# ShuoYangRobotics/Cerberus

Measured on NVIDIA H100. Metric: sliding-window solves/sec (10-frame x 150-feature windows), higher is better.
Workload: dtype f64

## Files before the change

### cerberus_b200/csrc/cabi.cu

```cuda
#include "../../include/cerberus_b200.h"
#include "solve_kernel.cuh"
#include "preint_kernel.cuh"
#include "feature_kernels.cuh"
#include "marg_kernels.cuh"
#include "pack_kernels.cuh"
#include "resident_kernels.cuh"
#include <string>
#include <vector>
#include <thread>
#include <cstring>
#include <cstdio>
#include <algorithm>
#include <chrono>
#include <cstdlib>
#include <cstdint>
#include <utility>

using namespace cerb;

static thread_local std::string g_err;
static int fail(int code, const std::string &msg) { g_err = msg; return code; }
#define CUDA_TRY(expr)                                                                                         \
    do {                                                                                                       \
        cudaError_t e_ = (expr);                                                                               \
// ... 300 lines not shown
        if (op.height == 1) CUDA_TRY(cudaMemcpyAsync(op.dst, op.src, op.width, cudaMemcpyHostToDevice, s));
        else CUDA_TRY(cudaMemcpy2DAsync(op.dst, op.dpitch, op.src, op.spitch, op.width, op.height, cudaMemcpyHostToDevice, s));
    }
    const size_t staged = [&] { size_t t = 0; for (const auto &j : pl.stage) t += j.bytes; return t; }();
    h->last_dma_ops += (int)pl.dma.size(); h->last_staged_bytes += staged; h->traffic.staged += (int64_t)staged;
    return CERB_OK;
}

static int upload_raw(CerbHandle *h, int w0, int cn, const CerbWindowDesc *descs, const CerbWindowState *states, cudaStream_t s, double *t_stage_ms) {
    for (int w = w0; w < w0 + cn; w++) { int rc = validate_window(h, descs[w], states[w], &h->n0[w]); if (rc) return rc; h->nfeat[w] = descs[w].n_features; }
    h->res_n = 0; h->prior_gathered = h->prior_gather_due = false;
    UploadPlan pl;
    plan_rows(h, pl, w0, cn, h->rdesc, 0, 1, 0, [&](int w) { return (const void *)&descs[w]; }, [&](int) { return sizeof(CerbWindowDesc); });
    plan_rows(h, pl, w0, cn, h->rstate, 0, 1, 0, [&](int w) { return (const void *)&states[w]; }, [&](int) { return sizeof(CerbWindowState); });
    plan_rows(h, pl, w0, cn, h->rfeat, 0, 1, 0,
              [&](int w) { return (const void *)descs[w].features; }, [&](int w) { return (size_t)descs[w].n_features * sizeof(CerbFeature); });
    plan_rows(h, pl, w0, cn, h->robs, 0, 1, 0,
              [&](int w) { return (const void *)descs[w].obs; }, [&](int w) { return (size_t)descs[w].n_obs * sizeof(CerbObservation); });
    plan_rows(h, pl, w0, cn, h->rlam, 0, 1, 0,
              [&](int w) { return (const void *)states[w].para_Feature; }, [&](int w) { return (size_t)descs[w].n_features * 8; });
    const size_t tail_off = (size_t)(RAW_PRE_HEAD + RAW_PRE_JCOL0 * 31) * 8, tail_w = sizeof(CerbIMULegPreint) - tail_off;
    static_assert(sizeof(CerbIMULegPreint) == (33 + 2 * 961) * 8, "CerbIMULegPreint layout");
    static_assert(sizeof(CerbIMUPreint) == 467 * 8 && sizeof(CerbIMUPreint) <= RAW_PRE_STRIDE * 8, "CerbIMUPreint layout");
    plan_rows(h, pl, w0, cn, h->rpre, 0, CERB_WINDOW_SIZE, sizeof(CerbIMULegPreint),
              [&](int w) { return (const void *)descs[w].preint; }, [&](int w) { return descs[w].preint ? (size_t)RAW_PRE_HEAD * 8 : (size_t)0; });
    plan_rows(h, pl, w0, cn, h->rpre, RAW_PRE_HEAD * 8, CERB_WINDOW_SIZE, sizeof(CerbIMULegPreint),
              [&](int w) { return (const void *)((const char *)descs[w].preint + tail_off); }, [&](int w) { return descs[w].preint ? tail_w : (size_t)0; });
    plan_rows(h, pl, w0, cn, h->rpre, 0, CERB_WINDOW_SIZE, sizeof(CerbIMUPreint),
              [&](int w) { return (const void *)descs[w].imu_preint; }, [&](int w) { return descs[w].preint ? (size_t)0 : sizeof(CerbIMUPreint); });
    plan_rows(h, pl, w0, cn, h->prior_J, 0, 1, 0,
              [&](int w) { return (const void *)descs[w].prior.linearized_jacobians; }, [&](int w) { return descs[w].prior.valid ? (size_t)descs[w].prior.n * descs[w].prior.n * 8 : (size_t)0; });
    plan_rows(h, pl, w0, cn, h->prior_r, 0, 1, 0,
              [&](int w) { return (const void *)descs[w].prior.linearized_residuals; }, [&](int w) { return descs[w].prior.valid ? (size_t)descs[w].prior.n * 8 : (size_t)0; });
    return run_plan(h, pl, s, t_stage_ms);
}

static int enqueue_pack(CerbHandle *h, int w0, int cn, cudaStream_t s) {
    PackParams P;
    P.n = cn; P.maxF = h->F; P.maxObs = h->O;
    P.rdesc = h->rdesc.at(w0); P.rfeat = h->rfeat.at(w0); P.robs = h->robs.at(w0); P.rpre = h->rpre.at(w0); P.rstate = h->rstate.at(w0); P.rlam = h->rlam.at(w0);
    P.n_features = h->n_features.at(w0); P.feat_start = h->feat_start.at(w0); P.feat_nobs = h->feat_nobs.at(w0); P.feat_off = h->feat_off.at(w0); P.flags = h->flags.at(w0);
    P.obs_stereo = h->obs_stereo.at(w0); P.prior_meta = h->prior_meta.at(w0); P.perm = h->perm.at(w0);
    P.obs = h->obs.at(w0); P.pre = h->pre.at(w0); P.prior_x0 = h->prior_x0.at(w0); P.state0 = h->state0.at(w0); P.lam0 = h->lam0.at(w0);
    if (h->res_n) { P.pre_slot = h->pre_slot.d; P.window = h->pre_slot.d + (size_t)cn * CERB_WINDOW_SIZE; }
    CERB_LAUNCH(pack_kernel, std::min(cn, 8 * h->sm_count), PACK_THREADS, 0, s, P);
    CUDA_TRY(cudaGetLastError());
    return CERB_OK;
}
static int upload(CerbHandle *h, int n, const CerbWindowDesc *descs, const CerbWindowState *states) {
    h->last_dma_ops = 0; h->last_staged_bytes = 0;
    int rc = upload_raw(h, 0, n, descs, states, h->stream, nullptr); if (rc) return rc;
    rc = enqueue_pack(h, 0, n, h->stream); if (rc) return rc;
    h->n = n; h->solved = false; h->perm_valid = false;
    return CERB_OK;
}
static int ensure_perm(CerbHandle *h) {
    if (h->perm_valid) return CERB_OK;
    h->h_perm.resize((size_t)h->B * h->perm.per);
    CUDA_TRY(cudaMemcpyAsync(h->h_perm.data(), h->perm.d, h->perm.bytes(h->n), cudaMemcpyDeviceToHost, h->stream));
    CUDA_TRY(cudaStreamSynchronize(h->stream));
    h->perm_valid = true;
    return CERB_OK;
}

static const Resident<double> &batch_prior_J(const CerbHandle *h) { return h->prior_gathered ? h->step_J : h->prior_J; }
static const Resident<double> &batch_prior_r(const CerbHandle *h) { return h->prior_gathered ? h->step_r : h->prior_r; }

static SolveParams make_params(CerbHandle *h, int w0, int n, int max_iters, double *dbg, int dbg_window) {
    SolveParams P;
    std::memset(&P, 0, sizeof(P));
    const CerbSolverConfig &c = h->cfg;
    P.n_windows = n; P.maxF = h->F; P.maxObs = h->O; P.max_iters = max_iters; P.optimize_leg_bias = c.optimize_leg_bias;
    for (int k = 0; k < 3; k++) P.G[k] = c.g[k];
    P.sqrt_info = c.visual_sqrt_info; P.huber = c.huber_delta;
    P.radius0 = c.initial_trust_region_radius; P.max_radius = c.max_trust_region_radius; P.min_radius = c.min_trust_region_radius;
    P.min_rel_dec = c.min_relative_decrease; P.ftol = c.function_tolerance; P.gtol = c.gradient_tolerance; P.ptol = c.parameter_tolerance;
    P.n_features = h->n_features.at(w0); P.feat_start = h->feat_start.at(w0); P.feat_nobs = h->feat_nobs.at(w0); P.feat_off = h->feat_off.at(w0); P.flags = h->flags.at(w0);
    P.obs = h->obs.at(w0); P.obs_stereo = h->obs_stereo.at(w0); P.pre = h->pre.at(w0); P.sinfo = h->sinfo.at(w0);
    P.prior_J = batch_prior_J(h).at(w0); P.prior_r = batch_prior_r(h).at(w0); P.prior_x0 = h->prior_x0.at(w0); P.prior_Hp = h->prior_Hp.at(w0); P.prior_meta = h->prior_meta.at(w0);
    P.state = h->state.at(w0); P.lam = h->lam.at(w0); P.rep_i = h->rep_i.at(w0); P.rep_d = h->rep_d.at(w0); P.ws = h->d_ws; P.ws_stride = h->ws_stride;
    P.dbg = dbg; P.dbg_window = dbg_window;
    P.test_fail_factorizations = h->test_fail_factorizations; P.test_initial_mu = h->test_initial_mu;
    P.no_bulk_copy = std::getenv("CERB_NO_TMA") != nullptr;
    return P;
}

static void enqueue_prepare(CerbHandle *h, int w0, int n, cudaStream_t s) {
    const int nfac = n * CERB_WINDOW_SIZE;
    CERB_LAUNCH(imu_leg_prepare_kernel, (nfac + 1) / 2, 64, 0, s, nfac, (const double *)h->pre.at(w0), h->sinfo.at(w0));
    CERB_LAUNCH(prior_prepare_kernel, n, 256, (size_t)PRIOR_TROWS * PRIOR_TLD * sizeof(double), s, (const double *)batch_prior_J(h).at(w0), (const int *)h->prior_meta.at(w0), h->prior_Hp.at(w0));
}

static int gather_priors(CerbHandle *h, cudaStream_t s) {
    if (!h->prior_gather_due) return CERB_OK;
    const int n = h->n;
    CERB_LAUNCH(prior_gather_kernel, std::min(n, 8 * h->sm_count), 256, 0, s, n, (const int *)(h->pre_slot.d + (size_t)n * CERB_WINDOW_SIZE), (const CerbWindowDesc *)h->rdesc.d,
                (const double *)h->prior_J.d, (const double *)h->prior_r.d, h->step_J.d, h->step_r.d);
    CUDA_TRY(cudaGetLastError());
    h->prior_gather_due = false;
    return CERB_OK;
}

static int enqueue_solve(CerbHandle *h, int w0, int n, int max_iters, double *dbg, int dbg_window, bool restore = true, bool probe = false, int lane = 0) {
    cudaStream_t s = h->lane[lane];
    if (restore) {
        CUDA_TRY(cudaMemcpyAsync(h->state.at(w0), h->state0.at(w0), h->state.bytes(n), cudaMemcpyDeviceToDevice, s));
        CUDA_TRY(cudaMemcpyAsync(h->lam.at(w0), h->lam0.at(w0), h->lam.bytes(n), cudaMemcpyDeviceToDevice, s));
    }
    int rc = gather_priors(h, s); if (rc) return rc;
    enqueue_prepare(h, w0, n, s);
    SolveParams P = make_params(h, w0, n, max_iters, dbg, dbg_window);
    P.ws = h->d_ws + (size_t)lane * h->grid * h->ws_stride;
    if (probe) { P.rep_i = h->d_probe_repi; P.rep_d = h->d_probe_repd; }
    if (max_iters > 0) h->solved = true;
    CERB_LAUNCH(vilo_solve_kernel, std::min(n, h->grid), SOLVE_THREADS, h->smem_bytes, s, P);
    CUDA_TRY(cudaGetLastError());
    return CERB_OK;
}
static int launch_solve(CerbHandle *h, int max_iters, double *dbg, int dbg_window, bool timed) {
    const int n = h->n;
    if (n < 1) return fail(CERB_ERR_BAD_ARGUMENT, "no resident batch");
    if (timed) CUDA_TRY(cudaEventRecord(h->ev0, h->stream));
    int rc = enqueue_solve(h, 0, n, max_iters, dbg, dbg_window); if (rc) return rc;
    if (timed) { CUDA_TRY(cudaEventRecord(h->ev1, h->stream)); h->ev_pending = true; h->last_launches = 3; }
    return CERB_OK;
}

static int collect_time(CerbHandle *h) {
    if (h->ev_pending) {
        CUDA_TRY(cudaEventSynchronize(h->ev1));
        float ms = 0; CUDA_TRY(cudaEventElapsedTime(&ms, h->ev0, h->ev1));
        h->last_ms = ms; h->ev_pending = false;
    }
    return CERB_OK;
}

struct States { Resident<double> state, lam; };
static States resident_states(const CerbHandle *h) { return h->solved ? States{h->state, h->lam} : States{h->state0, h->lam0}; }

static int download(CerbHandle *h, CerbWindowState *states, CerbSolveReport *reports) {
    const int n = h->n;
    cudaStream_t s = h->stream;
    const States cur = resident_states(h);
    UnpackParams U;
    U.n = n; U.maxF = h->F; U.n_features = h->n_features.d; U.perm = h->perm.d; U.rep_i = h->rep_i.d; U.rep_d = h->rep_d.d;
    U.lam = cur.lam.d; U.state = cur.state.d;
    U.olam = h->olam.d; U.orep = h->orep.d; U.ostate = h->ostate.d;
    CERB_LAUNCH(unpack_kernel, std::min(n, 8 * h->sm_count), PACK_THREADS, 0, s, U);
    CUDA_TRY(cudaGetLastError());
    COPY_TRY(h, h->ostate.h, h->ostate.d, h->ostate.bytes(n), cudaMemcpyDeviceToHost, s);
    COPY_TRY(h, h->olam.h, h->olam.d, h->olam.bytes(n), cudaMemcpyDeviceToHost, s);
    COPY_TRY(h, h->orep.h, h->orep.d, h->orep.bytes(n), cudaMemcpyDeviceToHost, s);
    CUDA_TRY(cudaStreamSynchronize(s));
    int rc = collect_time(h); if (rc) return rc;
    int status = CERB_OK;
    for (int w = 0; w < n; w++) {
        if (states) {
            std::memcpy(&states[w], h->ostate.h_at(w), ST_SIZE * sizeof(double));
            if (states[w].para_Feature && h->nfeat[w]) std::memcpy(states[w].para_Feature, h->olam.h_at(w), (size_t)h->nfeat[w] * sizeof(double));
        }
        if (reports) reports[w] = h->orep.h[w];
        if (h->orep.h[w].status != 0) status = CERB_ERR_NON_FINITE;
    }
    if (status) return fail(status, "at least one window produced a non-finite cost (see reports[].status)");
    return CERB_OK;
}

extern "C" {

int cerb_register_host_buffer(CerbHandle *h, void *ptr, size_t bytes) {
    if (!h || !ptr || !bytes) return fail(CERB_ERR_BAD_ARGUMENT, "cerb_register_host_buffer: null argument");
    CERB_DEVICE(h);
    CUDA_TRY(cudaHostRegister(ptr, bytes, cudaHostRegisterDefault));
    h->regs.emplace_back((uintptr_t)ptr, bytes);
    return CERB_OK;
}
int cerb_unregister_host_buffer(CerbHandle *h, void *ptr) {
    if (!h || !ptr) return fail(CERB_ERR_BAD_ARGUMENT, "cerb_unregister_host_buffer: null argument");
    CERB_DEVICE(h);
    for (size_t k = 0; k < h->regs.size(); k++) if (h->regs[k].first == (uintptr_t)ptr) {
        CUDA_TRY(cudaStreamSynchronize(h->stream)); CUDA_TRY(cudaStreamSynchronize(h->copy_stream));
        CUDA_TRY(cudaHostUnregister(ptr));
        h->regs.erase(h->regs.begin() + k);
        return CERB_OK;
    }
    return fail(CERB_ERR_BAD_ARGUMENT, "cerb_unregister_host_buffer: not registered with this handle");
}

int cerb_batch_upload(CerbHandle *h, int32_t n, const CerbWindowDesc *descs, const CerbWindowState *states) {
    if (!h || !descs || !states) return fail(CERB_ERR_BAD_ARGUMENT, "null argument");
    CERB_DEVICE(h);
    if (n < 1 || n > h->B) return fail(CERB_ERR_BAD_ARGUMENT, "batch size over capacity");
    CUDA_TRY(cudaStreamSynchronize(h->stream));
    return upload(h, n, descs, states);
}
int cerb_batch_solve_resident(CerbHandle *h) {
    if (!h) return fail(CERB_ERR_BAD_ARGUMENT, "null handle");
    CERB_DEVICE(h);
    int rc = collect_time(h); if (rc) return rc;
    return launch_solve(h, h->cfg.max_num_iterations, nullptr, -1, true);
}
int cerb_batch_download(CerbHandle *h, CerbWindowState *states, CerbSolveReport *reports) {
    if (!h) return fail(CERB_ERR_BAD_ARGUMENT, "null handle");
    CERB_DEVICE(h);
    return download(h, states, reports);
}
int cerb_sync(CerbHandle *h) {
    if (!h) return fail(CERB_ERR_BAD_ARGUMENT, "null handle");
    CERB_DEVICE(h);
    CUDA_TRY(cudaStreamSynchronize(h->stream));
    return collect_time(h);
}
int cerb_last_solve_stats(CerbHandle *h, double *kernel_ms, int32_t *kernel_launches) {
    if (!h) return fail(CERB_ERR_BAD_ARGUMENT, "null handle");
    CERB_DEVICE(h);
    int rc = collect_time(h); if (rc) return rc;
    if (kernel_ms) *kernel_ms = h->last_ms;
    if (kernel_launches) *kernel_launches = h->last_launches;
    return CERB_OK;
}
int cerb_last_upload_stats(CerbHandle *h, int32_t *dma_ops, int64_t *staged_bytes) {
    if (!h) return fail(CERB_ERR_BAD_ARGUMENT, "null handle");
    if (dma_ops) *dma_ops = h->last_dma_ops;
    if (staged_bytes) *staged_bytes = (int64_t)h->last_staged_bytes;
    return CERB_OK;
}
int cerb_solve_batch(CerbHandle *h, int32_t n, const CerbWindowDesc *descs, CerbWindowState *states, CerbSolveReport *reports) {
    if (!h || !descs || !states) return fail(CERB_ERR_BAD_ARGUMENT, "null argument");
    CERB_DEVICE(h);
    if (n < 1 || n > h->B) return fail(CERB_ERR_BAD_ARGUMENT, "batch size over capacity");
    CUDA_TRY(cudaStreamSynchronize(h->stream)); CUDA_TRY(cudaStreamSynchronize(h->copy_stream));
    for (int l = 1; l < CerbHandle::LANES; l++) CUDA_TRY(cudaStreamSynchronize(h->lane[l]));
    int rc = collect_time(h); if (rc) return rc;
    const int MAXC = CerbHandle::MAX_CHUNKS;
    int NL = 3, first = 64;
    if (const char *e = std::getenv("CERB_PIPE_LANES")) NL = std::min((int)CerbHandle::LANES, std::max(1, std::atoi(e)));
    if (const char *e = std::getenv("CERB_PIPE_FIRST")) first = std::max(1, std::atoi(e));
    int bounds[CerbHandle::MAX_CHUNKS + 1], nch = 0; bounds[0] = 0;
    if (const char *e = std::getenv("CERB_TEST_CHUNK")) {
        const int per = std::max(std::max(1, std::atoi(e)), (n + MAXC - 1) / MAXC);
        for (int pos = 0; pos < n; ) { pos = std::min(n, pos + per); bounds[++nch] = pos; }
    } else if (n <= first + first / 2) { bounds[1] = n; nch = 1; }
    else {
        int cap = 4 * first;
        if ((n + cap - 1) / cap > MAXC - 8) cap = (((n + MAXC - 9) / (MAXC - 8)) + first - 1) / first * first;
        int pos = 0, sz = first, k = 0;
        while (pos < n) {
            int take = std::min(sz, n - pos);
            if (n - pos - take < first / 2 || nch == MAXC - 1) take = n - pos;
            pos += take; bounds[++nch] = pos;
            if (++k >= 2) sz = std::min(cap, 2 * sz);
        }
    }
    h->n = n; h->perm_valid = false;
    h->last_dma_ops = 0; h->last_staged_bytes = 0;
    const bool trace = std::getenv("CERB_TRACE") != nullptr;
    auto now = [] { return std::chrono::duration<double, std::milli>(std::chrono::steady_clock::now().time_since_epoch()).count(); };
    const double t_begin = now(); double t_stage = 0.0;
    CUDA_TRY(cudaEventRecord(h->ev0, h->stream));
    for (int l = 1; l < NL; l++) CUDA_TRY(cudaStreamWaitEvent(h->lane[l], h->ev0, 0));
    auto drain = [&](int code) { for (int l = 0; l < NL; l++) cudaStreamSynchronize(h->lane[l]); cudaStreamSynchronize(h->copy_stream); return code; };
    for (int c = 0; c < nch; c++) {
        const int w0 = bounds[c], cn = bounds[c + 1] - bounds[c], l = c % NL;
        rc = upload_raw(h, w0, cn, descs, states, h->copy_stream, &t_stage); if (rc) return drain(rc);
        CUDA_TRY(cudaEventRecord(h->ev_copy[c], h->copy_stream));
        CUDA_TRY(cudaStreamWaitEvent(h->lane[l], h->ev_copy[c], 0));
        rc = enqueue_pack(h, w0, cn, h->lane[l]); if (rc) return drain(rc);
        rc = enqueue_solve(h, w0, cn, h->cfg.max_num_iterations, nullptr, -1, true, false, l); if (rc) return drain(rc);
    }
    for (int l = 1; l < NL; l++) { CUDA_TRY(cudaEventRecord(h->ev_lane[l], h->lane[l])); CUDA_TRY(cudaStreamWaitEvent(h->stream, h->ev_lane[l], 0)); }
    CUDA_TRY(cudaEventRecord(h->ev1, h->stream)); h->ev_pending = true; h->last_launches = 4 * nch + 1;
    const double t_issued = now();
    rc = download(h, states, reports);
    if (trace) std::fprintf(stderr, "[cerb_solve_batch] n=%d chunks=%d dma ops %d, staged %.1f MB in %.2f ms, all issued at %.2f ms, done at %.2f ms\n", n, nch, h->last_dma_ops,
                            h->last_staged_bytes / 1e6, t_stage, t_issued - t_begin, now() - t_begin);
    return rc;
}
int cerb_solve_window(CerbHandle *h, const CerbWindowDesc *desc, CerbWindowState *state, CerbSolveReport *report) {
    return cerb_solve_batch(h, 1, desc, state, report);
}

int cerb_debug_linearize(CerbHandle *h, int32_t w, double *cost, double *gradient, double *jtj_diag, int32_t n_alloc) {
    if (!h || w < 0 || w >= h->n) return fail(CERB_ERR_BAD_ARGUMENT, "bad window index");
    CERB_DEVICE(h);
    const int nf = h->nfeat[w], F = h->F;
    if (n_alloc < NR + nf) return fail(CERB_ERR_BAD_ARGUMENT, "n_alloc too small");
    int rc = ensure_perm(h); if (rc) return rc;
    const size_t cnt = 2 * (size_t)(NR + F) + 8;
    CUDA_TRY(cudaMemsetAsync(h->d_dbg, 0, cnt * sizeof(double), h->stream));
    rc = enqueue_solve(h, w, 1, 0, h->d_dbg, 0, !h->solved, true); if (rc) return rc;
    CUDA_TRY(cudaMemcpyAsync(h->h_dbg, h->d_dbg, cnt * sizeof(double), cudaMemcpyDeviceToHost, h->stream));
    CUDA_TRY(cudaStreamSynchronize(h->stream));
    if (cost) *cost = h->h_dbg[0];
    const int *perm = h->h_perm.data() + (size_t)w * F;
    for (int k = 0; k < NR + nf; k++) {
        const int dst = k < NR ? k : NR + perm[k - NR];
        if (gradient) gradient[dst] = h->h_dbg[1 + k];
        if (jtj_diag) jtj_diag[dst] = h->h_dbg[1 + NR + F + k];
    }
    return CERB_OK;
}

#if defined(CERB_PHASE_TIMING) && !defined(CERB_CUSIM)
extern "C" int cerb_prof_phase_cycles(unsigned long long *out48) {
    unsigned long long z[48] = {0};
    if (cudaMemcpyFromSymbol(out48, g_phase_cycles, sizeof(z)) != cudaSuccess) return CERB_ERR_CUDA;
    if (cudaMemcpyToSymbol(g_phase_cycles, z, sizeof(z)) != cudaSuccess) return CERB_ERR_CUDA;
    return CERB_OK;
}
#endif

struct DevBuf {
    CerbHandle *h;
    explicit DevBuf(CerbHandle *h_) : h(h_) { h->arena_chunk = 0; h->arena_used = 0; }
    void *raw(size_t bytes) {
        bytes = (std::max<size_t>(bytes, 8) + 255) & ~(size_t)255;
        while (h->arena_chunk < h->arena.size() && h->arena_used + bytes > h->arena[h->arena_chunk].second) { h->arena_chunk++; h->arena_used = 0; }
        if (h->arena_chunk == h->arena.size()) {
            const size_t sz = std::max<size_t>(bytes, (size_t)16 << 20);
            char *p = nullptr; if (cudaMalloc((void **)&p, sz) != cudaSuccess) return nullptr;
            h->arena.emplace_back(p, sz); h->arena_used = 0;
        }
        void *r = h->arena[h->arena_chunk].first + h->arena_used; h->arena_used += bytes;
        return r;
    }
    double *up(const double *src, size_t n, cudaStream_t s) {
        double *d = (double *)raw(n * sizeof(double)); if (!d) return nullptr;
        if (src) { h->traffic.count(cudaMemcpyHostToDevice, n * sizeof(double)); cudaMemcpyAsync(d, src, n * sizeof(double), cudaMemcpyHostToDevice, s); }
        return d;
    }
    int *upi(const int *src, size_t n, cudaStream_t s) {
        int *d = (int *)raw(n * sizeof(int)); if (!d) return nullptr;
        if (src) { h->traffic.count(cudaMemcpyHostToDevice, n * sizeof(int)); cudaMemcpyAsync(d, src, n * sizeof(int), cudaMemcpyHostToDevice, s); }
        return d;
    }
};

static void pack_preint(const CerbIMULegPreint &p, double *o) {
    const double *sdb = reinterpret_cast<const double *>(&p);
    std::vector<double> raw(RAW_PRE_STRIDE);
    for (int k = 0; k < RAW_PRE_STRIDE; k++) raw[k] = k < RAW_PRE_HEAD ? sdb[k] : sdb[k + RAW_PRE_JCOL0 * 31];
    for (int k = 0; k < PRE_STRIDE; k++) o[k] = pack_pre_leg(raw.data(), k);
}
static void pack_imu_preint(const CerbIMUPreint &p, double *o) {
    const double *raw = reinterpret_cast<const double *>(&p);
    for (int k = 0; k < PRE_STRIDE; k++) o[k] = pack_pre_imu(raw, k);
}
static const int kImuTo31[15] = {0, 1, 2, 3, 4, 5, 6, 7, 8, 21, 22, 23, 24, 25, 26};
static void encode_prior(const CerbPrior &pr, int *meta, double *x0) {
    std::memset(meta, 0, PRIOR_META_STRIDE * sizeof(int));
    if (!pr.valid) return;
    meta[0] = 1; meta[1] = pr.n; meta[2] = pr.num_blocks;
    for (int b = 0; b < pr.num_blocks; b++) {
        meta[4 + 3 * b] = pr.block_kind[b]; meta[5 + 3 * b] = pr.block_index[b]; meta[6 + 3 * b] = pr.block_col[b];
        for (int k = 0; k < 9; k++) x0[9 * b + k] = pr.block_x0[b][k];
    }
}
static void decode_prior(const int *meta, const double *x0, CerbPrior &pr) {
    pr.valid = 0; pr.n = 0; pr.num_blocks = 0;
    if (!meta[0]) return;
    pr.valid = 1; pr.n = meta[1]; pr.num_blocks = meta[2];
    for (int b = 0; b < pr.num_blocks; b++) {
        pr.block_kind[b] = meta[4 + 3 * b]; pr.block_index[b] = meta[5 + 3 * b]; pr.block_col[b] = meta[6 + 3 * b];
        for (int k = 0; k < 9; k++) pr.block_x0[b][k] = x0[9 * b + k];
    }
}


int cerb_eval_projection(CerbHandle *h, int32_t kind, int32_t n, const double *pose_i, const double *pose_j, const double *ex0, const double *ex1,
                         const double *inv_dep, const double *td, const double *pts_i, const double *pts_j, const double *vel_i, const double *vel_j,
                         const double *td_i, const double *td_j, double *residuals, double *jacobians) {
    if (!h || n < 1 || kind < 0 || kind > 2 || !ex0 || !inv_dep || !td || !pts_i || !pts_j || !vel_i || !vel_j || !td_i || !td_j) return fail(CERB_ERR_BAD_ARGUMENT, "cerb_eval_projection: bad argument");
    CERB_DEVICE(h);
    if (kind != CERB_PROJ_ONE_FRAME_TWO_CAM && (!pose_i || !pose_j)) return fail(CERB_ERR_BAD_ARGUMENT, "poses required");
    if (kind != CERB_PROJ_TWO_FRAME_ONE_CAM && !ex1) return fail(CERB_ERR_BAD_ARGUMENT, "ex1 required");
    cudaStream_t s = h->stream; DevBuf B(h); const size_t N = n;
    const int JS = kind == 0 ? 46 : (kind == 1 ? 60 : 32);
    double *dpi = pose_i ? B.up(pose_i, 7 * N, s) : nullptr, *dpj = pose_j ? B.up(pose_j, 7 * N, s) : nullptr;
    double *de0 = B.up(ex0, 7 * N, s), *de1 = ex1 ? B.up(ex1, 7 * N, s) : nullptr;
    double *dl = B.up(inv_dep, N, s), *dtd = B.up(td, N, s), *dpti = B.up(pts_i, 3 * N, s), *dptj = B.up(pts_j, 3 * N, s);
    double *dvi = B.up(vel_i, 2 * N, s), *dvj = B.up(vel_j, 2 * N, s), *dti = B.up(td_i, N, s), *dtj = B.up(td_j, N, s);
    double *dr = B.up(nullptr, 2 * N, s), *dJ = jacobians ? B.up(nullptr, JS * N, s) : nullptr;
    if (!dr || !dtj) return fail(CERB_ERR_CUDA, "device allocation failed");
    CERB_LAUNCH(projection_eval_kernel, (n + 127) / 128, 128, 0, s, (int)kind, (int)n, (const double *)dpi, (const double *)dpj, (const double *)de0, (const double *)de1,
                (const double *)dl, (const double *)dtd, (const double *)dpti, (const double *)dptj, (const double *)dvi, (const double *)dvj, (const double *)dti,
                (const double *)dtj, h->cfg.visual_sqrt_info, dr, dJ);
    CUDA_TRY(cudaGetLastError());
    if (residuals) CUDA_TRY(cudaMemcpyAsync(residuals, dr, 2 * N * sizeof(double), cudaMemcpyDeviceToHost, s));
    if (jacobians) CUDA_TRY(cudaMemcpyAsync(jacobians, dJ, JS * N * sizeof(double), cudaMemcpyDeviceToHost, s));
    CUDA_TRY(cudaStreamSynchronize(s));
    return CERB_OK;
}

static int eval_imu_leg_packed(CerbHandle *h, int n, const double *packed, const double *params, double *residuals, double *jacobians, double *sqrt_info) {
    cudaStream_t s = h->stream; DevBuf B(h); const size_t N = n;
    double *dpre = B.up(packed, N * PRE_STRIDE, s), *dsi = B.up(nullptr, N * 961, s), *dpar = B.up(params, 40 * N, s);
    double *dr = B.up(nullptr, 31 * N, s), *dJ = jacobians ? B.up(nullptr, 31 * 40 * N, s) : nullptr;
    if (!dpre || !dsi || !dpar || !dr) return fail(CERB_ERR_CUDA, "device allocation failed");
    CERB_LAUNCH(imu_leg_prepare_kernel, (n + 1) / 2, 64, 0, s, (int)n, (const double *)dpre, dsi);
    CERB_LAUNCH(imu_leg_eval_kernel, n, 128, 0, s, (int)n, (const double *)dpre, (const double *)dsi, (const double *)dpar, (const double *)h->d_G, dr, dJ);
    CUDA_TRY(cudaGetLastError());
    if (residuals) CUDA_TRY(cudaMemcpyAsync(residuals, dr, 31 * N * sizeof(double), cudaMemcpyDeviceToHost, s));
    if (jacobians) CUDA_TRY(cudaMemcpyAsync(jacobians, dJ, 31 * 40 * N * sizeof(double), cudaMemcpyDeviceToHost, s));
    if (sqrt_info) CUDA_TRY(cudaMemcpyAsync(sqrt_info, dsi, 961 * N * sizeof(double), cudaMemcpyDeviceToHost, s));
    CUDA_TRY(cudaStreamSynchronize(s));
    return CERB_OK;
}

int cerb_eval_imu_leg(CerbHandle *h, int32_t n, const CerbIMULegPreint *preint, const double *params, double *residuals, double *jacobians, double *sqrt_info) {
    if (!h || n < 1 || !preint || !params) return fail(CERB_ERR_BAD_ARGUMENT, "cerb_eval_imu_leg: bad argument");
    CERB_DEVICE(h);
    std::vector<double> packed((size_t)n * PRE_STRIDE, 0.0);
    for (int k = 0; k < n; k++) pack_preint(preint[k], packed.data() + (size_t)k * PRE_STRIDE);
    return eval_imu_leg_packed(h, n, packed.data(), params, residuals, jacobians, sqrt_info);
}

int cerb_eval_imu(CerbHandle *h, int32_t n, const CerbIMUPreint *preint, const double *params, double *residuals, double *jacobians, double *sqrt_info) {
    if (!h || n < 1 || !preint || !params) return fail(CERB_ERR_BAD_ARGUMENT, "cerb_eval_imu: bad argument");
    CERB_DEVICE(h);
    const size_t N = n;
    std::vector<double> packed(N * PRE_STRIDE), p40(N * 40, 0.0);
    for (int k = 0; k < n; k++) {
        pack_imu_preint(preint[k], packed.data() + (size_t)k * PRE_STRIDE);
        const double *q = params + (size_t)k * 32; double *o = p40.data() + (size_t)k * 40;
        std::memcpy(o, q, 16 * sizeof(double)); std::memcpy(o + 20, q + 16, 16 * sizeof(double));
    }
    std::vector<double> hr(31 * N), hj(jacobians ? 31 * 40 * N : 0), hs(961 * N);
    int rc = eval_imu_leg_packed(h, n, packed.data(), p40.data(), hr.data(), jacobians ? hj.data() : nullptr, hs.data()); if (rc) return rc;
    const int boff31[4] = {0, 7, 20, 27}, bsz[4] = {7, 9, 7, 9}, boff15[4] = {0, 7, 16, 23};
    for (int k = 0; k < n; k++) {
        for (int r = 0; r < 15; r++) {
            const int R = kImuTo31[r];
            if (residuals) residuals[(size_t)k * 15 + r] = hr[(size_t)k * 31 + R];
            if (sqrt_info) for (int c = 0; c < 15; c++) sqrt_info[(size_t)k * 225 + r * 15 + c] = hs[(size_t)k * 961 + R * 31 + kImuTo31[c]];
            if (jacobians) for (int b = 0; b < 4; b++) for (int c = 0; c < bsz[b]; c++)
                jacobians[(size_t)k * 15 * 32 + 15 * boff15[b] + r * bsz[b] + c] = hj[(size_t)k * 31 * 40 + 31 * boff31[b] + R * bsz[b] + c];
        }
    }
    return CERB_OK;
}

int cerb_eval_prior(CerbHandle *h, const CerbPrior *prior, const CerbWindowState *state, double *residuals, double *jacobians) {
    if (!h || !prior || !state || !prior->valid || !residuals) return fail(CERB_ERR_BAD_ARGUMENT, "cerb_eval_prior: bad argument");
    CERB_DEVICE(h);
    std::vector<int> meta(PRIOR_META_STRIDE); std::vector<double> J(PRIOR_LD * PRIOR_LD, 0.0), r(PRIOR_LD, 0.0), x0(16 * 9, 0.0), st(ST_STRIDE, 0.0);
    int rc = validate_prior(*prior); if (rc) return rc;
    encode_prior(*prior, meta.data(), x0.data());
    std::memcpy(J.data(), prior->linearized_jacobians, sizeof(double) * prior->n * prior->n);
    std::memcpy(r.data(), prior->linearized_residuals, sizeof(double) * prior->n);
    std::memcpy(st.data() + ST_POSE, state->para_Pose, sizeof(state->para_Pose)); std::memcpy(st.data() + ST_SB, state->para_SpeedBias, sizeof(state->para_SpeedBias));
    std::memcpy(st.data() + ST_LB, state->para_LegBias, sizeof(state->para_LegBias)); std::memcpy(st.data() + ST_EX, state->para_Ex_Pose, sizeof(state->para_Ex_Pose));
    st[ST_TD] = state->para_Td[0];
    size_t jtot = 0; for (int b = 0; b < prior->num_blocks; b++) jtot += (size_t)prior->n * prior_block_size(prior->block_kind[b]);
    cudaStream_t s = h->stream; DevBuf B(h);
    double *dJ = B.up(J.data(), J.size(), s), *dr0 = B.up(r.data(), r.size(), s), *dx0 = B.up(x0.data(), x0.size(), s), *dst = B.up(st.data(), st.size(), s);
    double *dres = B.up(nullptr, PRIOR_LD, s), *djac = jacobians ? B.up(nullptr, jtot, s) : nullptr;
    int *dmeta = B.upi(meta.data(), PRIOR_META_STRIDE, s);
    if (!dJ || !dr0 || !dx0 || !dst || !dres || !dmeta || (jacobians && !djac)) return fail(CERB_ERR_CUDA, "device allocation failed");
    CERB_LAUNCH(prior_eval_kernel, 1, 128, 0, s, (const double *)dJ, (const double *)dr0, (const int *)dmeta, (const double *)dx0, (const double *)dst, dres, djac);
    CUDA_TRY(cudaGetLastError());
    CUDA_TRY(cudaMemcpyAsync(residuals, dres, prior->n * sizeof(double), cudaMemcpyDeviceToHost, s));
    if (jacobians) CUDA_TRY(cudaMemcpyAsync(jacobians, djac, jtot * sizeof(double), cudaMemcpyDeviceToHost, s));
    CUDA_TRY(cudaStreamSynchronize(s));
    return CERB_OK;
}

int cerb_a1_kinematics(CerbHandle *h, int32_t n, const double *q, const double *rho_opt, const double *rho_fix, double *fk, double *jac, double *dfk_drho,
                       double *dJ_dq, double *dJ_drho) {
    if (!h || n < 1 || !q || !rho_opt || !rho_fix) return fail(CERB_ERR_BAD_ARGUMENT, "cerb_a1_kinematics: bad argument");
    CERB_DEVICE(h);
    cudaStream_t s = h->stream; DevBuf B(h); const size_t N = n;
    double *dq = B.up(q, 3 * N, s), *dro = B.up(rho_opt, N, s), *drf = B.up(rho_fix, 4 * N, s);
    double *dfk = fk ? B.up(nullptr, 3 * N, s) : nullptr, *dj = jac ? B.up(nullptr, 9 * N, s) : nullptr, *ddf = dfk_drho ? B.up(nullptr, 3 * N, s) : nullptr;
    double *djq = dJ_dq ? B.up(nullptr, 27 * N, s) : nullptr, *djr = dJ_drho ? B.up(nullptr, 9 * N, s) : nullptr;
    CERB_LAUNCH(a1_kinematics_kernel, (n + 127) / 128, 128, 0, s, (int)n, (const double *)dq, (const double *)dro, (const double *)drf, dfk, dj, ddf, djq, djr);
    CUDA_TRY(cudaGetLastError());
    if (fk) CUDA_TRY(cudaMemcpyAsync(fk, dfk, 3 * N * sizeof(double), cudaMemcpyDeviceToHost, s));
    if (jac) CUDA_TRY(cudaMemcpyAsync(jac, dj, 9 * N * sizeof(double), cudaMemcpyDeviceToHost, s));
    if (dfk_drho) CUDA_TRY(cudaMemcpyAsync(dfk_drho, ddf, 3 * N * sizeof(double), cudaMemcpyDeviceToHost, s));
    if (dJ_dq) CUDA_TRY(cudaMemcpyAsync(dJ_dq, djq, 27 * N * sizeof(double), cudaMemcpyDeviceToHost, s));
    if (dJ_drho) CUDA_TRY(cudaMemcpyAsync(dJ_drho, djr, 9 * N * sizeof(double), cudaMemcpyDeviceToHost, s));
    CUDA_TRY(cudaStreamSynchronize(s));
    return CERB_OK;
}

}
template <class Launch, class Store> static int feature_pass(CerbHandle *h, int planes, Launch launch, Store store) {
    CERB_DEVICE(h);
    if (h->n < 1) return fail(CERB_ERR_BAD_ARGUMENT, "no resident batch");
    const int n = h->n, F = h->F;
    const size_t N = (size_t)n * F;
    cudaStream_t s = h->stream; DevBuf B(h);
    double *d_out = B.up(nullptr, planes * N, s), *d_perm_out = B.up(nullptr, planes * N, s);
    if (!d_out || !d_perm_out) return fail(CERB_ERR_CUDA, "device allocation failed");
    const int threads = 128, blocks = (int)((N + threads - 1) / threads);
    launch(s, blocks, threads, resident_states(h), d_out);
    CERB_LAUNCH(unpermute_kernel, blocks, threads, 0, s, n, F, planes, (const int *)h->n_features.d, (const int *)h->perm.d, (const double *)d_out, d_perm_out);
    CUDA_TRY(cudaGetLastError());
    std::vector<double> tmp(planes * N);
    COPY_TRY(h, tmp.data(), d_perm_out, tmp.size() * sizeof(double), cudaMemcpyDeviceToHost, s);
    CUDA_TRY(cudaStreamSynchronize(s));
    for (int w = 0; w < n; w++)
        for (int f = 0; f < h->nfeat[w]; f++) store((size_t)w * F + f, tmp.data(), N);
    return CERB_OK;
}
extern "C" {

int cerb_batch_outlier_errors(CerbHandle *h, double focal_length, double *ave_err, int32_t *remove) {
    if (!h || !ave_err) return fail(CERB_ERR_BAD_ARGUMENT, "null argument");
    return feature_pass(h, 1, [&](cudaStream_t s, int blocks, int threads, const States &cur, double *out) {
        CERB_LAUNCH(outlier_error_kernel, blocks, threads, 0, s, h->n, h->F, h->O, (const int *)h->n_features.d, (const int *)h->feat_start.d, (const int *)h->feat_nobs.d,
                    (const int *)h->feat_off.d, (const double *)h->obs.d, (const int *)h->obs_stereo.d, (const double *)cur.state.d, (const double *)cur.lam.d, out);
    }, [&](size_t q, const double *v, size_t) { ave_err[q] = v[q]; if (remove) remove[q] = (v[q] * focal_length > 3.0) ? 1 : 0; });
}
int cerb_batch_triangulate(CerbHandle *h, double init_depth, double *depth) {
    if (!h || !depth) return fail(CERB_ERR_BAD_ARGUMENT, "null argument");
    return feature_pass(h, 1, [&](cudaStream_t s, int blocks, int threads, const States &cur, double *out) {
        CERB_LAUNCH(triangulate_kernel, blocks, threads, 0, s, h->n, h->F, h->O, (const int *)h->n_features.d, (const int *)h->feat_start.d, (const int *)h->feat_nobs.d,
                    (const int *)h->feat_off.d, (const double *)h->obs.d, (const int *)h->obs_stereo.d, (const double *)cur.state.d, (const double *)cur.lam.d, init_depth, out);
    }, [&](size_t q, const double *v, size_t) { depth[q] = v[q]; });
}
int cerb_batch_shift_depth(CerbHandle *h, double init_depth, int32_t *new_start_frame, double *depth, int32_t *keep) {
    if (!h || !new_start_frame || !depth || !keep) return fail(CERB_ERR_BAD_ARGUMENT, "null argument");
    return feature_pass(h, 3, [&](cudaStream_t s, int blocks, int threads, const States &cur, double *out) {
        CERB_LAUNCH(shift_depth_kernel, blocks, threads, 0, s, h->n, h->F, h->O, (const int *)h->n_features.d, (const int *)h->feat_start.d, (const int *)h->feat_nobs.d,
                    (const int *)h->feat_off.d, (const double *)h->obs.d, (const double *)cur.state.d, (const double *)cur.lam.d, init_depth, out);
    }, [&](size_t q, const double *v, size_t N) { new_start_frame[q] = (int32_t)v[q]; depth[q] = v[N + q]; keep[q] = (int32_t)v[2 * N + q]; });
}
static size_t marg_smem_limit() {
    const char *e = std::getenv("CERB_TEST_MARG_SMEM");
    if (!e) return MARG_SMEM_MAX;
    const long v = std::atol(e);
    return (v >= 4096 && (size_t)v <= MARG_SMEM_MAX) ? (size_t)v : MARG_SMEM_MAX;
}
int cerb_marginalize_schur(CerbHandle *h, int32_t n_windows, int32_t m, int32_t n, const double *A, const double *b, double eps,
                           double *linearized_jacobians, double *linearized_residuals, int32_t *sweeps) {
    if (!h || !A || !b || !linearized_jacobians || !linearized_residuals) return fail(CERB_ERR_BAD_ARGUMENT, "null argument");
    CERB_DEVICE(h);
    if (n_windows < 1 || m < 1 || n < 1 || m > 19 + CERB_MAX_FEATURES || n > CERB_MAX_PRIOR_DIM) return fail(CERB_ERR_BAD_ARGUMENT, "cerb_marginalize_schur: bad sizes");
    const size_t pos = (size_t)m + n, N = n_windows;
    const size_t lim = marg_smem_limit();
    int grid = std::min<int>(n_windows, marg_ctas_per_sm(m, n, lim) * h->sm_count);
    grid = (int)std::max<size_t>(1, std::min<size_t>(grid, ((size_t)4 << 30) / (marg_ws_doubles(m, n, lim) * sizeof(double))));
    CUDA_TRY(cudaFuncSetAttribute(marg_schur_kernel, cudaFuncAttributeMaxDynamicSharedMemorySize, (int)marg_smem_bytes(m, n, lim)));
    cudaStream_t s = h->stream; DevBuf B(h);
    double *dA = B.up(A, N * pos * pos, s), *db = B.up(b, N * pos, s), *dws = B.up(nullptr, (size_t)grid * marg_ws_doubles(m, n, lim), s);
    double *dJ = B.up(nullptr, N * n * n, s), *dr = B.up(nullptr, N * n, s), *dsw = B.up(nullptr, N, s);
    if (!dA || !db || !dws || !dJ || !dr || !dsw) return fail(CERB_ERR_CUDA, "device allocation failed");
    CERB_LAUNCH(marg_schur_kernel, grid, marg_threads(m, n, lim), marg_smem_bytes(m, n, lim), s, (int)n_windows, (int)m, (int)n, (const int *)nullptr, (const double *)dA, 0L, (const double *)db, 0L, eps, dws, dJ, 0L, dr, 0L, (int *)dsw, (int)lim);
    CUDA_TRY(cudaGetLastError());
    CUDA_TRY(cudaMemcpyAsync(linearized_jacobians, dJ, N * n * n * sizeof(double), cudaMemcpyDeviceToHost, s));
    CUDA_TRY(cudaMemcpyAsync(linearized_residuals, dr, N * n * sizeof(double), cudaMemcpyDeviceToHost, s));
    if (sweeps) CUDA_TRY(cudaMemcpyAsync(sweeps, dsw, N * 2 * sizeof(int32_t), cudaMemcpyDeviceToHost, s));
    CUDA_TRY(cudaStreamSynchronize(s));
    return CERB_OK;
}

CERB_GLOBAL void permute_lam_kernel(int n, int F, const int *n_features, const int *perm, const double *lam_caller, double *lam_dev) {
    const long idx = (long)blockIdx.x * blockDim.x + threadIdx.x;
    if (idx >= (long)n * F) return;
    const int w = (int)(idx / F), k = (int)(idx % F);
    if (k < n_features[w]) lam_dev[idx] = lam_caller[(size_t)w * F + perm[idx]];
}

static int states_to_device(CerbHandle *h, DevBuf &B, const CerbWindowState *states, const char *who, const States &dst, std::vector<double> &hst) {
    const int n = h->n, F = h->F;
    cudaStream_t s = h->stream;
    hst.assign(n * dst.state.per, 0.0);
    std::vector<double> hl(n * dst.lam.per, 0.0);
    for (int w = 0; w < n; w++) {
        std::memcpy(hst.data() + w * dst.state.per, &states[w], ST_SIZE * sizeof(double));
        if (h->nfeat[w]) {
            if (!states[w].para_Feature) return fail(CERB_ERR_BAD_ARGUMENT, std::string(who) + ": null para_Feature");
            std::memcpy(hl.data() + w * dst.lam.per, states[w].para_Feature, (size_t)h->nfeat[w] * 8);
        }
    }
    double *dlc = B.up(hl.data(), hl.size(), s);
    if (!dlc) return fail(CERB_ERR_CUDA, "device allocation failed");
    COPY_TRY(h, dst.state.d, hst.data(), dst.state.bytes(n), cudaMemcpyHostToDevice, s);
    CERB_LAUNCH(permute_lam_kernel, (int)(((size_t)n * F + 127) / 128), 128, 0, s, n, F, (const int *)h->n_features.d, (const int *)h->perm.d, (const double *)dlc, dst.lam.d);
    CUDA_TRY(cudaGetLastError());
    CUDA_TRY(cudaStreamSynchronize(s));
    return CERB_OK;
}

static int marginalize_impl(CerbHandle *h, const int32_t *flags, const CerbWindowState *states, CerbPrior *priors, int32_t *sweeps, int32_t *valid) {
    const int n = h->n;
    if (n < 1) return fail(CERB_ERR_BAD_ARGUMENT, "no resident batch");
    for (int w = 0; w < n; w++) {
        if (flags[w] != 0 && flags[w] != 1) return fail(CERB_ERR_BAD_ARGUMENT, "cerb_batch_marginalize: flag must be 0 (MARGIN_OLD) or 1 (MARGIN_SECOND_NEW)");
        if (priors && (!priors[w].linearized_jacobians || !priors[w].linearized_residuals)) return fail(CERB_ERR_BAD_ARGUMENT, "cerb_batch_marginalize: priors[w] needs storage for linearized_jacobians / linearized_residuals");
    }
    cudaStream_t s = h->stream; DevBuf B(h);
    int mmax = 19;
    const int nmax = MARG_N_STRUCT;
    for (int w = 0; w < n; w++) if (flags[w] == 0) mmax = std::max(mmax, 19 + h->n0[w]);
    const int posmax = mmax + CERB_MAX_PRIOR_DIM;
    std::vector<double> hst;
    States lin = resident_states(h);
    if (states) {
        lin.state.d = B.up(nullptr, n * lin.state.per, s); lin.lam.d = B.up(nullptr, n * lin.lam.per, s);
        if (!lin.state.d || !lin.lam.d) return fail(CERB_ERR_CUDA, "device allocation failed");
        int rc = states_to_device(h, B, states, "cerb_batch_marginalize", lin, hst); if (rc) return rc;
    } else {
        hst.resize(n * lin.state.per);
        COPY_TRY(h, hst.data(), lin.state.d, lin.state.bytes(n), cudaMemcpyDeviceToHost, s);
    }
    std::vector<int> hflags(flags, flags + n);
    int *dflags = B.upi(hflags.data(), n, s), *ddims = B.upi(nullptr, (size_t)n * 4, s), *dblocks = B.upi(nullptr, (size_t)n * 64, s), *dsw = B.upi(nullptr, (size_t)n * 2, s);
// ... 238 lines not shown
```

### cerberus_b200/csrc/solve_kernel.cuh

```cuda
#pragma once
#include "eval_kernels.cuh"

namespace cerb {

#if defined(CERB_PHASE_TIMING) && !defined(CERB_CUSIM)
__device__ unsigned long long g_phase_cycles[48];
#define PH_DECL() long long ph_t = clock64()
#define PH_MARK_T(id, t) do { if ((threadIdx.x & 31) == 0) { const long long ph_n = clock64(); if (threadIdx.x == (t)) atomicAdd(&g_phase_cycles[id], (unsigned long long)(ph_n - ph_t)); ph_t = ph_n; } __syncwarp(); } while (0)
#define PH_MARK(id) PH_MARK_T(id, 0)
#define PH_ARG , long long &ph_t
#define PH_FWD , ph_t
#else
#define PH_DECL()
#define PH_MARK_T(id, t)
#define PH_MARK(id)
#define PH_ARG
#define PH_FWD
#endif

enum { CERB_WINDOW = 10, NX = 79, NYB = 13, NFR = 11, NY = 143, NR = 222, NRP = 224, HXX_SZ = 79 * 79, HXY_SZ = 79 * 143, X_TD = 78, SOLVE_THREADS = 256, FT = 64, TILE_LD = 33, NOBS_PLANES = 9 };
enum { HBLK = NYB * NYB, AD_SZ = NFR * HBLK, BO_SZ = (NFR - 1) * HBLK };
#ifndef CERB_SOLVE_MIN_BLOCKS
#define CERB_SOLVE_MIN_BLOCKS 1
#endif
enum { PIMG_HXY = HXX_SZ + 1, PIMG_REST = HXY_SZ + AD_SZ + BO_SZ, PIMG_SZ = PIMG_HXY + PIMG_REST, SMEM_HXX_PAD = 3 };
static_assert((PIMG_HXY * 8) % 16 == 0 && (PIMG_REST * 8) % 16 == 0 && ((HXX_SZ + SMEM_HXX_PAD) * 8) % 16 == 0, "bulk-copy alignment of the prior image");

struct SolveParams {
    int n_windows, maxF, maxObs, max_iters, optimize_leg_bias;
    double G[3], sqrt_info, huber;
    double radius0, max_radius, min_radius, min_rel_dec, ftol, gtol, ptol;
    const int *n_features, *feat_start, *feat_nobs, *feat_off, *flags;
    const double *obs; const int *obs_stereo;
    const double *pre;
    const double *sinfo;
    const double *prior_J, *prior_r, *prior_x0, *prior_Hp; const int *prior_meta;
    double *state, *lam;
    int *rep_i; double *rep_d;
    double *ws;
    long ws_stride;
    double *dbg; int dbg_window;
    double test_initial_mu;
    int no_bulk_copy;
    int test_fail_factorizations;
};

CERB_HD long ws_vecs(int F) { return (long)NX * F; }
CERB_HD long ws_prior(int F) { return (long)NX * F + 9L * F; }
CERB_HD long ws_chunks(int F) { return ws_prior(F) + PIMG_SZ; }
CERB_HD long ws_imuplan(int F) { return (ws_chunks(F) + (F + 4) / 2 + 8 + 1) & ~1L; }
CERB_HD long ws_size(int F) { return ws_imuplan(F) + 15 * 2 * 32 * 4 / 2 + 8; }
struct CtaWs {
    double *W, *hh, *gl, *sl, *Dl, *ghl, *gnl, *stl, *lamc, *sinv;
    int *chunks;
    int *imu_plan;
    double *pimg;
    int F;
};
CERB_D CtaWs ws_carve(const SolveParams &P) {
    double *ws = P.ws + (size_t)blockIdx.x * P.ws_stride;
    const int F = P.maxF;
    CtaWs v;
    v.W = ws;
    v.hh = ws + ws_vecs(F); v.gl = v.hh + F; v.sl = v.gl + F; v.Dl = v.sl + F; v.ghl = v.Dl + F; v.gnl = v.ghl + F; v.stl = v.gnl + F; v.lamc = v.stl + F; v.sinv = v.lamc + F;
    v.chunks = reinterpret_cast<int *>(ws + ws_chunks(F)); v.imu_plan = reinterpret_cast<int *>(ws + ws_imuplan(F));
    v.pimg = ws + ws_prior(F); v.F = F;
    return v;
}

struct Smem {
    double *Hxx, *Hxy, *Ad, *Bo;
    double *g, *sc, *D, *gh, *gn, *stp, *yv;
    double *xs, *xc;
    double *Rw, *Rex;
    double *Ju;
    double *lin;
    double *pdx, *pr;
    double *red;
    double *wj;
    double *sca;
    double *chain_col;
    double *idg;
    double *idx;
    int *ti;
    unsigned long long *mbar;
    double *tile;
};
enum { S_RADIUS = 0, S_MU, S_REUSE, S_XCOST, S_CCOST, S_ALPHA, S_GNORM2, S_GNNORM2, S_GDOTGN, S_MODEL, S_STEPNORM, S_XNORM, S_DLNORM,
       S_OK, S_DONE, S_TERM, S_ITER, S_NSUCC, S_INVALID, S_GMAX, S_INIT_COST, S_P, S_Q, S_VHV, S_LCOST, S_LNORM, S_LGMAX, S_COUNT };
static_assert(S_COUNT <= 32, "scalar slots overlap the chain's column line");
enum { TI_PRIOR_MAP = 0, TI_NCHUNKS = 96, TI_CHUNK_CACHE = 97, TI_CACHED_CHUNKS = 15, TI_CHAIN_DONE = 130, TI_IMU_MASK = 131, TI_INTS = 132 };
static_assert(TI_PRIOR_MAP + CERB_MAX_PRIOR_DIM <= TI_NCHUNKS && TI_CHUNK_CACHE + 2 * TI_CACHED_CHUNKS <= TI_CHAIN_DONE && TI_IMU_MASK < TI_INTS && TI_INTS % 2 == 0,
              "s.ti slots overlap");
enum { SMEM_DOUBLES = HXX_SZ + SMEM_HXX_PAD + HXY_SZ + AD_SZ + BO_SZ + 7 * NRP + 2 * ST_STRIDE + 99 + 18 + 3 + 31 * 39 + 960 + 192 + 8 * 256 + 128 * 8 + 32 + 32 + TI_INTS / 2 + 144 + 80 };

CERB_D void smem_carve(double *base, Smem &s) {
    double *p = base;
    s.Hxx = p; p += HXX_SZ; s.mbar = reinterpret_cast<unsigned long long *>(p + 1); p += SMEM_HXX_PAD; s.Hxy = p; p += HXY_SZ; s.Ad = p; p += AD_SZ; s.Bo = p; p += BO_SZ;
    s.g = p; p += NRP; s.sc = p; p += NRP; s.D = p; p += NRP; s.gh = p; p += NRP; s.gn = p; p += NRP; s.stp = p; p += NRP; s.yv = p; p += NRP;
    s.xs = p; p += ST_STRIDE; s.xc = p; p += ST_STRIDE;
    s.Rw = p; p += 99; s.Rex = p; p += 18; p += 3;
    s.Ju = p; p += 31 * 39; s.red = p; p += 8 * 256; s.wj = p; p += 128 * 8;
    s.lin = p; p += 960; s.pdx = p; p += 96; s.pr = p; p += 96; s.sca = p; p += 32; s.chain_col = p; p += 32;
    s.ti = reinterpret_cast<int *>(p); p += TI_INTS / 2;
    s.idg = p; p += 144;
    s.idx = p; p += 80;
    s.tile = s.Hxy;
}

template <int NV>
CERB_D void block_sum(const double *v, double *red, double *out, int tid) {
    for (int k = 0; k < NV; k++) red[k * 256 + tid] = v[k];
    __syncthreads();
    for (int s = 128; s > 0; s >>= 1) {
        if (tid < s) for (int k = 0; k < NV; k++) red[k * 256 + tid] += red[k * 256 + tid + s];
        __syncthreads();
    }
    for (int k = 0; k < NV; k++) out[k] = red[k * 256];
    __syncthreads();
}

CERB_D void copy_g2s(double *dst, const double *src, int n, int tid) {
    for (int k0 = tid; k0 < n; k0 += 8 * SOLVE_THREADS) {
        double b[8];
        _Pragma("unroll")
        for (int u = 0; u < 8; u++) { const int k = k0 + u * SOLVE_THREADS; b[u] = (k < n) ? src[k] : 0.0; }
        _Pragma("unroll")
        for (int u = 0; u < 8; u++) { const int k = k0 + u * SOLVE_THREADS; if (k < n) dst[k] = b[u]; }
    }
}
CERB_D void copy_g2s_async(double *dst, const double *src, int n, int tid) {
    for (int k = tid; k < n; k += SOLVE_THREADS) CERB_CP_ASYNC8(dst + k, src + k);
}
CERB_D void load_geometry(const double *x, Smem &s, int tid) {
    if (tid < 11) { const m33 R = qtoR(ldq(x + ST_POSE + 7 * tid + 3)); for (int k = 0; k < 9; k++) s.Rw[9 * tid + k] = R.m[k]; }
    else if (tid < 13) { const int e = tid - 11; const m33 R = qtoR(ldq(x + ST_EX + 7 * e + 3)); for (int k = 0; k < 9; k++) s.Rex[9 * e + k] = R.m[k]; }
    __syncthreads();
}

struct ObsCtx { int start, nobs, off; double lam, pix, piy, vix, viy, tdi; };

struct ObsVals { double px, py, vx, vy, td; int stereo; };
CERB_D void obs_fetch(const double *obs, const int *stereo, int mo, int o, int cam, ObsVals &v) {
    v.px = obs[(cam ? 4 : 0) * mo + o]; v.py = obs[(cam ? 5 : 1) * mo + o]; v.vx = obs[(cam ? 6 : 2) * mo + o]; v.vy = obs[(cam ? 7 : 3) * mo + o];
    v.td = obs[8 * mo + o]; v.stereo = stereo[o];
}

CERB_NOINLINE double vision_cost(const SolveParams &P, int w, const double *x, const double *lam, int tid) {
    CERB_DYN_SMEM(double, smem_base);
    Smem s; smem_carve(smem_base, s);
    const int nF = P.n_features[w], mo = P.maxObs;
    const double *obs = P.obs + (size_t)w * NOBS_PLANES * P.maxObs;
    const int *stereo = P.obs_stereo + (size_t)w * P.maxObs;
    double cost = 0.0;
    for (int idx = tid; idx < 4 * nF; idx += SOLVE_THREADS) {
        const int f = idx >> 2, cam = idx & 1, part = (idx >> 1) & 1;
        ObsCtx c;
        c.start = P.feat_start[(size_t)w * P.maxF + f]; c.nobs = P.feat_nobs[(size_t)w * P.maxF + f]; c.off = P.feat_off[(size_t)w * P.maxF + f];
        c.lam = lam[f];
        c.pix = obs[0 * mo + c.off]; c.piy = obs[1 * mo + c.off]; c.vix = obs[2 * mo + c.off]; c.viy = obs[3 * mo + c.off];
        c.tdi = obs[8 * mo + c.off];
        const int k0 = part ? 6 : 0, k1 = part ? c.nobs : (c.nobs < 6 ? c.nobs : 6);
        const double inv_l = 1.0 / c.lam;
        const int i = c.start;
        const d3 tic = ld3(x + ST_EX);
        const double tdv = x[ST_TD];
        const d3 pts_i_td = mk3(c.pix, c.piy, 1.0) - (tdv - c.tdi) * mk3(c.vix, c.viy, 0.0);
        const d3 p_bi = mv33(ldm33(s.Rex), inv_l * pts_i_td) + tic;
        const d3 p_w = mv33(ldm33(s.Rw + 9 * i), p_bi) + ld3(x + ST_POSE + 7 * i);
        const double *Rcp = cam ? s.Rex + 9 : s.Rex;
        const d3 tc = cam ? ld3(x + ST_EX + 7) : tic;
        ObsVals cur, nxt;
        cur.px = cur.py = cur.vx = cur.vy = cur.td = 0.0; cur.stereo = 0;
        if (k0 < k1) obs_fetch(obs, stereo, mo, c.off + k0, cam, cur);
        _Pragma("unroll 1")
        for (int k = k0; k < k1; k++) {
            nxt = cur;
            if (k + 1 < k1) obs_fetch(obs, stereo, mo, c.off + k + 1, cam, nxt);
            const bool k3 = (k == 0);
            const bool on = k3 ? (cam == 1 && cur.stereo) : (cam == 0 || cur.stereo);
            if (on) {
                const int j = c.start + k;
                const d3 p_bj = k3 ? p_bi : mTv33(ldm33(s.Rw + 9 * j), p_w - ld3(x + ST_POSE + 7 * j));
                const d3 p_cj = mTv33(ldm33(Rcp), p_bj - tc);
                const double iz = 1.0 / p_cj.z;
                const double r0 = P.sqrt_info * (p_cj.x * iz - (cur.px - (tdv - cur.td) * cur.vx));
                const double r1 = P.sqrt_info * (p_cj.y * iz - (cur.py - (tdv - cur.td) * cur.vy));
                double cf; huber_weight(P.huber, r0 * r0 + r1 * r1, &cf);
                cost += cf;
            }
            cur = nxt;
        }
    }
    return cost;
}

enum { VT_LD = 516, VT_COLS = 26, VT_SZ = VT_COLS * VT_LD, VP_SZ = 6 * 64, VJ_SZ = 4 * 64 };
CERB_D int vis_col_dest(int g, int c, int a, int j) {
    if (g == 0) return c < 6 ? 6 * a + c : (c == 6 ? X_TD : -2);
    if (c >= 6) return -1;
    return g == 1 ? 6 * j + c : (g == 2 ? 66 + c : 72 + c);
}
CERB_D void vis_scatter(Smem &s, int ga, int gb, int ra, int rb, int a, int j, double v) {
    if (ga == gb && ra > rb) return;
    const int da = vis_col_dest(ga, ra, a, j), db = vis_col_dest(gb, rb, a, j);
    if (da == -1 || db == -1) return;
    if (da == -2) { if (db >= 0) s.g[db] += v; return; }
    if (db == -2) { s.g[da] += v; return; }
    if (da <= db) s.Hxx[da * NX + db] += v; else s.Hxx[db * NX + da] += v;
}
CERB_D void vis_jplan(const Smem &s, const double *smem_base, int el, int *base, int *ca, int *cj) {
    const int blk = el >> 6, ra = (el >> 3) & 7, rb = el & 7;
    const int hxx = (int)(s.Hxx - smem_base), g = (int)(s.g - smem_base);
    *base = -1; *ca = 0; *cj = 0;
    if (rb >= 6) return;
    if (blk == 0) {
        if (ra < 6) { *base = hxx + ra * NX + rb; *ca = 6 * NX; *cj = 6; }
        else if (ra == 6) { *base = hxx + rb * NX + X_TD; *cj = 6 * NX; }
        else { *base = g + rb; *cj = 6; }
    } else {
        if (ra >= 6 || (blk == 1 && ra > rb)) return;
        *base = hxx + ra * NX + (blk == 1 ? rb : (blk == 2 ? 66 + rb : 72 + rb)); *cj = 6 * NX + (blk == 1 ? 6 : 0);
    }
}
CERB_NOINLINE double vision_linearize(const SolveParams &P, int w, const double *x, const double *lam, double *W, double *hh, double *gl,
                                      const double *sl, bool prescale, const int *chunks, int tid) {
    CERB_DYN_SMEM(double, smem_base);
    Smem s; smem_carve(smem_base, s);
    const int nF = P.n_features[w], F = P.maxF, mo = P.maxObs;
    const double *obs = P.obs + (size_t)w * NOBS_PLANES * P.maxObs;
    const int *stereo = P.obs_stereo + (size_t)w * P.maxObs;
    double cost = 0.0;
    PH_DECL();
    for (int i = tid; i < NX * nF; i += SOLVE_THREADS) W[(i / nF) * F + (i % nF)] = 0.0;
    __syncthreads();
    const int wid = tid >> 5, lane = tid & 31;
    const int cam = tid >> 7, jj = (tid >> 6) & 1, fl = tid & 63;
    double *T = s.tile;
    double *jp = s.Ju;
    double *pp = (wid < 5) ? s.Ju + 8 * VJ_SZ + VP_SZ * wid : s.tile + VT_SZ + VP_SZ * (wid - 5);
    const int c8 = lane >> 2;
    const double *tq[4];
    bool tv[4];
    for (int g = 0; g < 4; g++) { const int pc = g == 0 ? c8 : 8 + 6 * (g - 1) + c8; tv[g] = (g == 0) || c8 < 6; tq[g] = T + (tv[g] ? pc : 0) * VT_LD + (lane & 3); }
    int jbase, jca, jcj;
    vis_jplan(s, smem_base, tid, &jbase, &jca, &jcj);
    const int nchunks = s.ti[TI_NCHUNKS];
    for (int ch = 0; ch < nchunks; ch++) {
        int c0, nc, a;
        if (ch < TI_CACHED_CHUNKS) { const int *cc = s.ti + TI_CHUNK_CACHE + 2 * ch; c0 = cc[0]; nc = cc[1] >> 8; a = cc[1] & 255; }
        else { c0 = chunks[1 + ch]; nc = chunks[2 + ch] - c0; a = P.feat_start[(size_t)w * F + c0]; }
        const int f = c0 + fl;
        const bool ev = fl < nc;
        int nobs = 0, off = 0;
        double lamf = 1.0, pix = 0.0, piy = 0.0, vix = 0.0, viy = 0.0, tdi = 0.0;
        const double slf = (prescale && ev) ? sl[f] : 1.0;
        if (ev) {
            nobs = P.feat_nobs[(size_t)w * F + f]; off = P.feat_off[(size_t)w * F + f];
            lamf = 1.0 / lam[f];
            pix = obs[0 * mo + off]; piy = obs[1 * mo + off]; vix = obs[2 * mo + off]; viy = obs[3 * mo + off]; tdi = obs[8 * mo + off];
        }
        ObsVals ov; ov.px = ov.py = ov.vx = ov.vy = ov.td = 0.0; ov.stereo = 0;
        { const int j = a + jj; if (ev && j < a + nobs) obs_fetch(obs, stereo, mo, off + (j - a), cam, ov); }
        for (int k = lane; k < VP_SZ; k += 32) pp[k] = 0.0;
        if (tid < 2 * (NFR - 1 - a)) {
            const int jq = a + 1 + (tid >> 1), cq = tid & 1;
            const m33 Rc = ldm33(cq ? s.Rex + 9 : s.Rex);
            const m33 A = mulT33(Rc, tr33(ldm33(s.Rw + 9 * jq)));
            const m33 ARi = mul33(A, ldm33(s.Rw + 9 * a));
            const m33 Tm = mul33(ARi, ldm33(s.Rex));
            double *C = s.lin + 27 * tid;
            for (int k = 0; k < 9; k++) { C[k] = A.m[k]; C[9 + k] = ARi.m[k]; C[18 + k] = Tm.m[k]; }
        } else if (tid == 32) {
            const m33 T3 = mul33(tr33(ldm33(s.Rex + 9)), ldm33(s.Rex));
            for (int k = 0; k < 9; k++) s.lin[540 + k] = T3.m[k];
        }
        __syncthreads();
        double h = 0.0, gq = 0.0, wT = 0.0, wI[6], wE0[6], wE1[6];
        for (int k = 0; k < 6; k++) { wI[k] = 0.0; wE0[k] = 0.0; wE1[k] = 0.0; }
        PH_MARK(20);
        for (int j0 = a; j0 < NFR; j0 += 2) {
            const int j = j0 + jj;
            bool valid = ev && j < a + nobs;
            int kind = PROJ_K1;
            if (valid) {
                if (j == a) { if (cam == 0 || !ov.stereo) valid = false; kind = PROJ_K3; }
                else if (cam == 1) { if (!ov.stereo) valid = false; kind = PROJ_K2; }
            }
            double wjv[6] = {0, 0, 0, 0, 0, 0};
            double *t0 = T + tid, *t1 = T + 256 + tid;
            if (valid) {
                const d3 tic = ld3(x + ST_EX), tc = kind == PROJ_K1 ? tic : ld3(x + ST_EX + 7);
                const double *Rcp = kind == PROJ_K1 ? s.Rex : s.Rex + 9;
                const double tdv = x[ST_TD];
                const d3 pts_i = mk3(pix, piy, 1.0), vel_i = mk3(vix, viy, 0.0);
                const d3 pts_i_td = pts_i - (tdv - tdi) * vel_i;
                const double pjx_td = ov.px - (tdv - ov.td) * ov.vx, pjy_td = ov.py - (tdv - ov.td) * ov.vy;
                const double inv_l = lamf;
                const d3 p_ci = inv_l * pts_i_td;
                const d3 p_bi = mv33(ldm33(s.Rex), p_ci) + tic;
                d3 p_bj = p_bi;
                if (kind != PROJ_K3) p_bj = mTv33(ldm33(s.Rw + 9 * j), (mv33(ldm33(s.Rw + 9 * a), p_bi) + ld3(x + ST_POSE + 7 * a)) - ld3(x + ST_POSE + 7 * j));
                const d3 p_cj = mTv33(ldm33(Rcp), p_bj - tc);
                const double iz = 1.0 / p_cj.z;
                double r0 = P.sqrt_info * (p_cj.x * iz - pjx_td), r1 = P.sqrt_info * (p_cj.y * iz - pjy_td);
                double cf; const double hw = huber_weight(P.huber, r0 * r0 + r1 * r1, &cf);
                cost += cf;
                r0 *= hw; r1 *= hw;
                const double q = hw * P.sqrt_info * iz, c0 = -q * p_cj.x * iz, c1 = -q * p_cj.y * iz;
                const d3 e0 = mk3(q, 0.0, c0), e1 = mk3(0.0, q, c1);
#define VIS_U(M, u0, u1) const d3 u0 = mk3(q * (M)[0] + c0 * (M)[6], q * (M)[1] + c0 * (M)[7], q * (M)[2] + c0 * (M)[8]), u1 = mk3(q * (M)[3] + c1 * (M)[6], q * (M)[4] + c1 * (M)[7], q * (M)[5] + c1 * (M)[8])
#define VIS_PUT(col, a0, a1) do { t0[(col) * VT_LD] = (a0); t1[(col) * VT_LD] = (a1); } while (0)
#define VIS_PUT3(col, v0_, v1_) do { VIS_PUT(col, (v0_).x, (v1_).x); VIS_PUT((col) + 1, (v0_).y, (v1_).y); VIS_PUT((col) + 2, (v0_).z, (v1_).z); } while (0)
                const double *Tm = kind == PROJ_K3 ? s.lin + 540 : s.lin + 27 * (2 * (j - a - 1) + cam) + 18;
                VIS_U(Tm, uT0, uT1);
                const d3 ptl = kind == PROJ_K3 ? pts_i : pts_i_td;
                const double l0 = -inv_l * inv_l * dot3(uT0, ptl), l1 = -inv_l * inv_l * dot3(uT1, ptl);
                const double d0 = -inv_l * dot3(uT0, vel_i) + hw * P.sqrt_info * ov.vx, d1 = -inv_l * dot3(uT1, vel_i) + hw * P.sqrt_info * ov.vy;
                h += l0 * l0 + l1 * l1; gq += l0 * r0 + l1 * r1; wT += d0 * l0 + d1 * l1;
                VIS_PUT(6, d0, d1); VIS_PUT(7, r0, r1);
                const d3 uC0 = mk3(q * Rcp[0] + c0 * Rcp[2], q * Rcp[3] + c0 * Rcp[5], q * Rcp[6] + c0 * Rcp[8]);
                const d3 uC1 = mk3(q * Rcp[1] + c1 * Rcp[2], q * Rcp[4] + c1 * Rcp[5], q * Rcp[7] + c1 * Rcp[8]);
                const d3 er0 = cross3(e0, p_cj), er1 = cross3(e1, p_cj);
                const d3 et0 = cross3(p_ci, uT0), et1 = cross3(p_ci, uT1);
                d3 E0t0, E0t1, E0r0, E0r1, E1t0, E1t1, E1r0, E1r1;
                if (kind == PROJ_K3) {
                    for (int k = 0; k < 6; k++) { VIS_PUT(k, 0.0, 0.0); VIS_PUT(8 + k, 0.0, 0.0); }
                    E0t0 = uC0; E0t1 = uC1; E0r0 = et0; E0r1 = et1; E1t0 = -uC0; E1t1 = -uC1; E1r0 = er0; E1r1 = er1;
                } else {
                    const double *C = s.lin + 27 * (2 * (j - a - 1) + cam);
                    VIS_U(C, uA0, uA1);
                    VIS_U(C + 9, uR0, uR1);
                    const d3 ir0 = cross3(p_bi, uR0), ir1 = cross3(p_bi, uR1);
                    const d3 jr0 = cross3(uC0, p_bj), jr1 = cross3(uC1, p_bj);
                    VIS_PUT3(0, uA0, uA1); VIS_PUT3(3, ir0, ir1);
                    VIS_PUT3(8, -uA0, -uA1); VIS_PUT3(11, jr0, jr1);
                    wI[0] += uA0.x * l0 + uA1.x * l1; wI[1] += uA0.y * l0 + uA1.y * l1; wI[2] += uA0.z * l0 + uA1.z * l1;
                    wI[3] += ir0.x * l0 + ir1.x * l1; wI[4] += ir0.y * l0 + ir1.y * l1; wI[5] += ir0.z * l0 + ir1.z * l1;
                    wjv[0] = -(uA0.x * l0 + uA1.x * l1); wjv[1] = -(uA0.y * l0 + uA1.y * l1); wjv[2] = -(uA0.z * l0 + uA1.z * l1);
                    wjv[3] = jr0.x * l0 + jr1.x * l1; wjv[4] = jr0.y * l0 + jr1.y * l1; wjv[5] = jr0.z * l0 + jr1.z * l1;
                    if (kind == PROJ_K1) {
                        E0t0 = uR0 - uC0; E0t1 = uR1 - uC1; E0r0 = et0 + er0; E0r1 = et1 + er1;
                        E1t0 = mk3(0, 0, 0); E1t1 = E1t0; E1r0 = E1t0; E1r1 = E1t0;
                    } else {
                        E0t0 = uR0; E0t1 = uR1; E0r0 = et0; E0r1 = et1; E1t0 = -uC0; E1t1 = -uC1; E1r0 = er0; E1r1 = er1;
                    }
                }
                VIS_PUT3(14, E0t0, E0t1); VIS_PUT3(17, E0r0, E0r1); VIS_PUT3(20, E1t0, E1t1); VIS_PUT3(23, E1r0, E1r1);
                wE0[0] += E0t0.x * l0 + E0t1.x * l1; wE0[1] += E0t0.y * l0 + E0t1.y * l1; wE0[2] += E0t0.z * l0 + E0t1.z * l1;
                wE0[3] += E0r0.x * l0 + E0r1.x * l1; wE0[4] += E0r0.y * l0 + E0r1.y * l1; wE0[5] += E0r0.z * l0 + E0r1.z * l1;
                wE1[0] += E1t0.x * l0 + E1t1.x * l1; wE1[1] += E1t0.y * l0 + E1t1.y * l1; wE1[2] += E1t0.z * l0 + E1t1.z * l1;
                wE1[3] += E1r0.x * l0 + E1r1.x * l1; wE1[4] += E1r0.y * l0 + E1r1.y * l1; wE1[5] += E1r0.z * l0 + E1r1.z * l1;
#undef VIS_U
#undef VIS_PUT
#undef VIS_PUT3
            } else {
                for (int k = 0; k < VT_COLS; k++) { t0[k * VT_LD] = 0.0; t1[k * VT_LD] = 0.0; }
            }
            const bool wrow = valid && j != a;
            if (wrow && cam == 0) for (int k = 0; k < 6; k++) W[(size_t)(6 * j + k) * F + f] = wjv[k] * (prescale ? s.sc[6 * j + k] * slf : 1.0);
            __syncthreads();
            PH_MARK(21);
            double wprev[6] = {0, 0, 0, 0, 0, 0};
            if (wrow && cam == 1) for (int k = 0; k < 6; k++) wprev[k] = W[(size_t)(6 * j + k) * F + f];
            { const int jn = j + 2; ov.stereo = 0; if (ev && jn < a + nobs) obs_fetch(obs, stereo, mo, off + (jn - a), cam, ov); }
            {
                const int jw = j0 + (wid >> 2), hw = (wid >> 1) & 1, par = wid & 1;
                const bool k3 = (jw == a);
                const int nkt = (nc + 3) >> 2;
                const bool work = jw < NFR && par < nkt;
                double acc[10][2];
                for (int k = 0; k < 10; k++) { acc[k][0] = 0.0; acc[k][1] = 0.0; }
                if (work) {
                    const int rb0 = 256 * hw + 64 * (wid >> 2) + 4 * par;
                    if (!k3) {
                        double v0 = tq[0][rb0], v1 = tv[1] ? tq[1][rb0] : 0.0, v2 = tv[2] ? tq[2][rb0] : 0.0;
                        for (int ks = par; ks < nkt; ks += 2) {
                            const int rn = rb0 + 4 * (ks + 2 - par);
                            const bool more = ks + 2 < nkt;
                            const double n0 = more ? tq[0][rn] : 0.0, n1 = (more && tv[1]) ? tq[1][rn] : 0.0, n2 = (more && tv[2]) ? tq[2][rn] : 0.0;
                            CERB_DMMA(acc[0][0], acc[0][1], v0, v0, acc[0][0], acc[0][1]);
                            CERB_DMMA(acc[1][0], acc[1][1], v0, v1, acc[1][0], acc[1][1]);
                            CERB_DMMA(acc[2][0], acc[2][1], v0, v2, acc[2][0], acc[2][1]);
                            CERB_DMMA(acc[4][0], acc[4][1], v1, v1, acc[4][0], acc[4][1]);
                            CERB_DMMA(acc[5][0], acc[5][1], v1, v2, acc[5][0], acc[5][1]);
                            CERB_DMMA(acc[7][0], acc[7][1], v2, v2, acc[7][0], acc[7][1]);
                            v0 = n0; v1 = n1; v2 = n2;
                        }
                    }
                    {
                        const int rb1 = rb0 + 128;
                        double v0 = tq[0][rb1], v1 = (!k3 && tv[1]) ? tq[1][rb1] : 0.0, v2 = tv[2] ? tq[2][rb1] : 0.0, v3 = tv[3] ? tq[3][rb1] : 0.0;
                        for (int ks = par; ks < nkt; ks += 2) {
                            const int rn = rb1 + 4 * (ks + 2 - par);
                            const bool more = ks + 2 < nkt;
                            const double n0 = more ? tq[0][rn] : 0.0, n1 = (more && !k3 && tv[1]) ? tq[1][rn] : 0.0, n2 = (more && tv[2]) ? tq[2][rn] : 0.0, n3 = (more && tv[3]) ? tq[3][rn] : 0.0;
                            CERB_DMMA(acc[0][0], acc[0][1], v0, v0, acc[0][0], acc[0][1]);
                            CERB_DMMA(acc[2][0], acc[2][1], v0, v2, acc[2][0], acc[2][1]);
                            CERB_DMMA(acc[3][0], acc[3][1], v0, v3, acc[3][0], acc[3][1]);
                            CERB_DMMA(acc[7][0], acc[7][1], v2, v2, acc[7][0], acc[7][1]);
                            CERB_DMMA(acc[8][0], acc[8][1], v2, v3, acc[8][0], acc[8][1]);
                            CERB_DMMA(acc[9][0], acc[9][1], v3, v3, acc[9][0], acc[9][1]);
                            if (!k3) {
                                CERB_DMMA(acc[1][0], acc[1][1], v0, v1, acc[1][0], acc[1][1]);
                                CERB_DMMA(acc[4][0], acc[4][1], v1, v1, acc[4][0], acc[4][1]);
                                CERB_DMMA(acc[5][0], acc[5][1], v1, v2, acc[5][0], acc[5][1]);
                                CERB_DMMA(acc[6][0], acc[6][1], v1, v3, acc[6][0], acc[6][1]);
                            }
                            v0 = n0; v1 = n1; v2 = n2; v3 = n3;
                        }
                    }
                    PH_MARK(28);
                    const int o = (lane >> 2) * 8 + 2 * (lane & 3);
                    pp[0 * 64 + o] += acc[0][0]; pp[0 * 64 + o + 1] += acc[0][1];
                    pp[1 * 64 + o] += acc[2][0]; pp[1 * 64 + o + 1] += acc[2][1];
                    pp[2 * 64 + o] += acc[3][0]; pp[2 * 64 + o + 1] += acc[3][1];
                    pp[3 * 64 + o] += acc[7][0]; pp[3 * 64 + o + 1] += acc[7][1];
                    pp[4 * 64 + o] += acc[8][0]; pp[4 * 64 + o + 1] += acc[8][1];
                    pp[5 * 64 + o] += acc[9][0]; pp[5 * 64 + o + 1] += acc[9][1];
                }
                {
                    const int o = wid * VJ_SZ + (lane >> 2) * 8 + 2 * (lane & 3);
                    jp[o] = acc[1][0]; jp[o + 1] = acc[1][1];
                    jp[64 + o] = acc[4][0]; jp[64 + o + 1] = acc[4][1];
                    jp[128 + o] = acc[5][0]; jp[128 + o + 1] = acc[5][1];
                    jp[192 + o] = acc[6][0]; jp[192 + o + 1] = acc[6][1];
                }
            }
            if (wrow && cam == 1) for (int k = 0; k < 6; k++) W[(size_t)(6 * j + k) * F + f] = wprev[k] + wjv[k] * (prescale ? s.sc[6 * j + k] * slf : 1.0);
            PH_MARK(29);
            __syncthreads();
            PH_MARK(22);
            if (jbase >= 0) {
                _Pragma("unroll")
                for (int fj = 0; fj < 2; fj++) {
                    const int jf = j0 + fj;
                    if (jf >= NFR || jf == a) continue;
                    const double *q = jp + (4 * fj) * VJ_SZ + tid;
                    smem_base[jbase + jca * a + jcj * jf] += ((q[0] + q[VJ_SZ]) + q[2 * VJ_SZ]) + q[3 * VJ_SZ];
                }
            }
            PH_MARK(23);
        }
        __syncthreads();
        {
            double *ex = T;
            ex[0 * 256 + tid] = h; ex[1 * 256 + tid] = gq; ex[2 * 256 + tid] = wT;
            for (int k = 0; k < 6; k++) { ex[(3 + k) * 256 + tid] = wI[k]; ex[(9 + k) * 256 + tid] = wE0[k]; ex[(15 + k) * 256 + tid] = wE1[k]; }
        }
        __syncthreads();
        for (int e = tid; e < VP_SZ; e += SOLVE_THREADS) {
            double v = 0.0;
            for (int wq = 0; wq < 8; wq++) v += ((wq < 5) ? s.Ju + 8 * VJ_SZ + VP_SZ * wq : s.tile + VT_SZ + VP_SZ * (wq - 5))[e];
            const int blk = e >> 6, ra = (e >> 3) & 7, rb = e & 7;
            const int ga = blk < 3 ? 0 : (blk < 5 ? 2 : 3), gb = blk == 0 ? 0 : (blk == 1 || blk == 3 ? 2 : 3);
            vis_scatter(s, ga, gb, ra, rb, a, a, v);
        }
        if (tid < 64 && ev) {
            const double *ex = T;
            double q[21];
            for (int k = 0; k < 21; k++) q[k] = ((ex[k * 256 + tid] + ex[k * 256 + 64 + tid]) + ex[k * 256 + 128 + tid]) + ex[k * 256 + 192 + tid];
            hh[f] = q[0] * slf * slf; gl[f] = q[1] * slf;
            W[(size_t)X_TD * F + f] = q[2] * (prescale ? s.sc[X_TD] * slf : 1.0);
            for (int k = 0; k < 6; k++) {
                W[(size_t)(6 * a + k) * F + f] = q[3 + k] * (prescale ? s.sc[6 * a + k] * slf : 1.0);
                W[(size_t)(66 + k) * F + f] = q[9 + k] * (prescale ? s.sc[66 + k] * slf : 1.0);
                W[(size_t)(72 + k) * F + f] = q[15 + k] * (prescale ? s.sc[72 + k] * slf : 1.0);
            }
        }
        __syncthreads();
        PH_MARK(24);
    }
    return cost;
}

CERB_D void imu_lin_all(const SolveParams &P, Smem &s, int w, const double *x, bool want_jac, int tid) {
    if (tid < CERB_WINDOW) {
        const double *pre = P.pre + ((size_t)w * CERB_WINDOW + tid) * PRE_STRIDE;
        IMULegLin *L = reinterpret_cast<IMULegLin *>(s.lin + 96 * tid);
        imu_leg_linearize(pre, x + ST_POSE + 7 * tid, x + ST_SB + 9 * tid, x + ST_LB + 4 * tid, x + ST_POSE + 7 * (tid + 1),
                          x + ST_SB + 9 * (tid + 1), x + ST_LB + 4 * (tid + 1), P.G, want_jac, L);
    }
    __syncthreads();
}

CERB_D double prior_residual(const SolveParams &P, Smem &s, int w, const double *x, int tid) {
    const int *meta = P.prior_meta + (size_t)w * PRIOR_META_STRIDE;
    if (!meta[0]) return 0.0;
    const int n = meta[1], nb = meta[2];
    const double *J = P.prior_J + (size_t)w * PRIOR_LD * PRIOR_LD, *r0 = P.prior_r + (size_t)w * PRIOR_LD, *x0 = P.prior_x0 + (size_t)w * 16 * 9;
    if (tid < nb) {
        const int kind = meta[4 + 3 * tid], index = meta[5 + 3 * tid], col = meta[6 + 3 * tid];
        prior_block_dx(kind, x + prior_block_state_offset(kind, index), x0 + 9 * tid, s.pdx + col);
    }
    __syncthreads();
    int parts = SOLVE_THREADS / n; if (parts > 4) parts = 4; if (parts < 1) parts = 1;
    const int kc = (n + parts - 1) / parts;
    double *part = s.red;
    for (int e = tid; e < parts * n; e += SOLVE_THREADS) {
        const int p = e / n, i = e % n;
        const int k1 = (p + 1) * kc < n ? (p + 1) * kc : n;
        double t = 0.0;
        for (int k = p * kc; k < k1; k++) t += J[(size_t)k * n + i] * s.pdx[k];
        part[p * PRIOR_LD + i] = t;
    }
    __syncthreads();
    double cost = 0.0;
    for (int i = tid; i < n; i += SOLVE_THREADS) {
        double t = r0[i];
        for (int p = 0; p < parts; p++) t += part[p * PRIOR_LD + i];
        s.pr[i] = t; cost += 0.5 * t * t;
    }
    __syncthreads();
    return cost;
}

CERB_NOINLINE double inertial_cost(const SolveParams &P, int w, const double *x, int tid) {
    CERB_DYN_SMEM(double, smem_base);
    Smem s; smem_carve(smem_base, s);
    imu_lin_all(P, s, w, x, false, tid);
    double cost = 0.0;
    for (int idx = tid; idx < CERB_WINDOW * 31; idx += SOLVE_THREADS) {
        const int i = idx / 31, r = idx % 31;
        const double *pre = P.pre + ((size_t)w * CERB_WINDOW + i) * PRE_STRIDE;
        if (pre[PRE_SUM_DT] > 10.0) continue;
        const double *ru = s.lin + 96 * i, *S = P.sinfo + ((size_t)w * CERB_WINDOW + i) * 961;
        double t = 0.0;
        for (int q = r; q < 31; q++) t += S[r * 31 + q] * ru[q];
        cost += 0.5 * t * t;
    }
    return cost + prior_residual(P, s, w, x, tid);
}

CERB_D int imu_col_dest(int i, int c) {
    if (c < 6) return 6 * i + c;
    if (c < 19) return -(1 + NYB * i + (c - 6));
    if (c < 25) return 6 * (i + 1) + (c - 19);
    return -(1 + NYB * (i + 1) + (c - 25));
}
CERB_D void scatter_addr(const Smem &s, int da, int db, double **a0, double **a1) {
    *a1 = nullptr;
    if (da >= 0 && db >= 0) { *a0 = (da <= db) ? s.Hxx + da * NX + db : s.Hxx + db * NX + da; return; }
    if (da >= 0) { *a0 = s.Hxy + da * NY + (-db - 1); return; }
    if (db >= 0) { *a0 = s.Hxy + db * NY + (-da - 1); return; }
    const int ya = -da - 1, yb = -db - 1;
    const int fa = ya / NYB, fb = yb / NYB, ka = ya % NYB, kb = yb % NYB;
    if (fa == fb) { *a0 = s.Ad + fa * HBLK + ka * NYB + kb; if (ka != kb) *a1 = s.Ad + fa * HBLK + kb * NYB + ka; }
    else if (fb == fa + 1) *a0 = s.Bo + fa * HBLK + ka * NYB + kb;
    else *a0 = s.Bo + fb * HBLK + kb * NYB + ka;
}
CERB_D void scatter_H(Smem &s, int da, int db, double v) {
    if (da >= 0 && db >= 0) { if (da <= db) s.Hxx[da * NX + db] += v; else s.Hxx[db * NX + da] += v; return; }
    if (da >= 0) { s.Hxy[da * NY + (-db - 1)] += v; return; }
    if (db >= 0) { s.Hxy[db * NY + (-da - 1)] += v; return; }
    const int ya = -da - 1, yb = -db - 1;
    const int fa = ya / NYB, fb = yb / NYB, ka = ya % NYB, kb = yb % NYB;
    if (fa == fb) { s.Ad[fa * HBLK + ka * NYB + kb] += v; if (ka != kb) s.Ad[fa * HBLK + kb * NYB + ka] += v; }
    else if (fb == fa + 1) s.Bo[fa * HBLK + ka * NYB + kb] += v;
    else s.Bo[fb * HBLK + kb * NYB + ka] += v;
}

enum { IMU_LDJ = 44, IMU_TILE = 32 * 44, IMU_WARPS = 3, PRIOR_THREADS = SOLVE_THREADS - 32 * IMU_WARPS };
CERB_NOINLINE double inertial_linearize(const SolveParams &P, int w, const double *x, int tid) {
    CERB_DYN_SMEM(double, smem_base);
    Smem s; smem_carve(smem_base, s);
    double cost = 0.0;
    PH_DECL();
    imu_lin_all(P, s, w, x, true, tid);
    PH_MARK(25);
    const int wid = tid >> 5, lane = tid & 31;
    CERB_CP_ASYNC_WAIT();
    double *gp = s.stp;
    double *ppart = s.yv;
    for (int k = tid; k < NRP; k += SOLVE_THREADS) gp[k] = 0.0;
    __syncthreads();
    if (wid < IMU_WARPS) {
        double *Jt = s.Ju + IMU_TILE * wid;
        int plx[30], ply[30];
        {
            const int *plan = ws_carve(P).imu_plan;
            _Pragma("unroll")
            for (int q = 0; q < 30; q++) { plx[q] = __ldg(plan + (2 * q) * 32 + lane); ply[q] = __ldg(plan + (2 * q + 1) * 32 + lane); }
            const int dummy = (int)(s.idg - smem_base) + lane;
            _Pragma("unroll")
            for (int q = 0; q < 30; q++) if (plx[q] == dummy && (ply[q] & 4095) == 0) plx[q] += 32 * wid;
        }
        double sa[20];
        auto load_S = [&](int i) {
            const double *S = P.sinfo + ((size_t)w * CERB_WINDOW + i) * 961;
            int q = 0;
            _Pragma("unroll")
            for (int mi = 0; mi < 4; mi++)
                _Pragma("unroll")
                for (int ks = 2 * mi; ks < 8; ks++) {
                    const int r = 8 * mi + (lane >> 2), c = 4 * ks + (lane & 3);
                    sa[q++] = (r < 31 && c < 31 && c >= r) ? S[r * 31 + c] : 0.0;
                }
        };
        load_S(wid * 4);
        const int imu_mask = s.ti[TI_IMU_MASK];
        double sdt[4];
        _Pragma("unroll")
        for (int rnd = 0; rnd < 4; rnd++) { const int i = rnd + 4 * wid; sdt[rnd] = (i < CERB_WINDOW) ? P.pre[((size_t)w * CERB_WINDOW + i) * PRE_STRIDE + PRE_SUM_DT] : 1e30; }
        _Pragma("unroll")
        for (int rnd = 0; rnd < 4; rnd++) {
            const int i = rnd + 4 * wid;
            const double *pre = P.pre + ((size_t)w * CERB_WINDOW + (i < CERB_WINDOW ? i : 0)) * PRE_STRIDE;
            if (i < CERB_WINDOW && !(sdt[rnd] > 10.0) && (imu_mask == 0 || (imu_mask == 1 && i == 0))) {
                for (int k = lane; k < IMU_TILE; k += 32) Jt[k] = 0.0;
                __syncwarp();
                if (lane < 11) imu_leg_fill_ju_part(*reinterpret_cast<const IMULegLin *>(s.lin + 96 * i), pre, Jt, IMU_LDJ, lane);
                if (lane < 31) Jt[lane * IMU_LDJ + 38] = s.lin[96 * i + lane];
                __syncwarp();
                PH_MARK(32);
                for (int ni = 0; ni < 5; ni++) {
                    double b[8];
                    _Pragma("unroll")
                    for (int ks = 0; ks < 8; ks++) b[ks] = Jt[(4 * ks + (lane & 3)) * IMU_LDJ + 8 * ni + (lane >> 2)];
                    __syncwarp();
                    double c[4][2];
                    int q = 0;
                    _Pragma("unroll")
                    for (int mi = 0; mi < 4; mi++) {
                        c[mi][0] = 0.0; c[mi][1] = 0.0;
                        _Pragma("unroll")
                        for (int ks = 2 * mi; ks < 8; ks++) { CERB_DMMA(c[mi][0], c[mi][1], sa[q], b[ks], c[mi][0], c[mi][1]); q++; }
                    }
                    _Pragma("unroll")
                    for (int mi = 0; mi < 4; mi++) { double *o = Jt + (8 * mi + (lane >> 2)) * IMU_LDJ + 8 * ni + 2 * (lane & 3); o[0] = c[mi][0]; o[1] = c[mi][1]; }
                    __syncwarp();
                }
                PH_MARK(33);
                if (i + 1 < CERB_WINDOW && rnd < 3) load_S(i + 1);
                double acc[15][2];
                _Pragma("unroll")
                for (int k = 0; k < 15; k++) { acc[k][0] = 0.0; acc[k][1] = 0.0; }
                for (int ks = 0; ks < 8; ks++) {
                    double f[5];
                    _Pragma("unroll")
                    for (int n = 0; n < 5; n++) f[n] = Jt[(4 * ks + (lane & 3)) * IMU_LDJ + 8 * n + (lane >> 2)];
                    int q = 0;
                    _Pragma("unroll")
                    for (int mi = 0; mi < 5; mi++)
                        _Pragma("unroll")
                        for (int ni = mi; ni < 5; ni++) { CERB_DMMA(acc[q][0], acc[q][1], f[mi], f[ni], acc[q][0], acc[q][1]); q++; }
                }
                PH_MARK(34);
                if (lane == 27) cost += 0.5 * acc[14][0];
                _Pragma("unroll")
                for (int hq = 0; hq < 30; hq += 15) {
                    double cur[15];
                    _Pragma("unroll")
                    for (int t = 0; t < 15; t++) cur[t] = smem_base[plx[hq + t] + i * (ply[hq + t] & 4095)];
                    _Pragma("unroll")
                    for (int t = 0; t < 15; t++) {
                        const int o = plx[hq + t] + i * (ply[hq + t] & 4095);
                        const double nv = cur[t] + acc[(hq + t) >> 1][(hq + t) & 1];
                        smem_base[o] = nv;
                        smem_base[o + (ply[hq + t] >> 12) - 256] = nv;
                    }
                }
                PH_MARK(35);
            } else if (i + 1 < CERB_WINDOW && rnd < 3) load_S(i + 1);
            CERB_BAR_SYNC(2, 32 * IMU_WARPS);
            PH_MARK(36);
        }
        PH_MARK(30);
    } else {
        const int *meta = P.prior_meta + (size_t)w * PRIOR_META_STRIDE;
        if (meta[0]) {
            const int t5 = tid - 32 * IMU_WARPS, n = meta[1], nb = meta[2];
            const double *J = P.prior_J + (size_t)w * PRIOR_LD * PRIOR_LD, *r0 = P.prior_r + (size_t)w * PRIOR_LD, *x0 = P.prior_x0 + (size_t)w * 16 * 9;
            if (t5 < nb) {
                const int kind = meta[4 + 3 * t5], index = meta[5 + 3 * t5], col = meta[6 + 3 * t5];
                prior_block_dx(kind, x + prior_block_state_offset(kind, index), x0 + 9 * t5, s.pdx + col);
            }
            CERB_BAR_SYNC(3, PRIOR_THREADS);
            const int kc = (n + 1) / 2;
            for (int e = t5; e < 2 * n; e += PRIOR_THREADS) {
                const int p = e / n, i = e % n;
                const int k1 = (p + 1) * kc < n ? (p + 1) * kc : n;
                double t = 0.0;
                for (int k = p * kc; k < k1; k++) t += J[(size_t)k * n + i] * s.pdx[k];
                ppart[p * PRIOR_LD + i] = t;
            }
            CERB_BAR_SYNC(3, PRIOR_THREADS);
            for (int i = t5; i < n; i += PRIOR_THREADS) {
                const double t = (r0[i] + ppart[i]) + ppart[PRIOR_LD + i];
                s.pr[i] = t; cost += 0.5 * t * t;
            }
            CERB_BAR_SYNC(3, PRIOR_THREADS);
            for (int c = wid - IMU_WARPS; c < n; c += PRIOR_THREADS / 32) {
                double t = 0.0;
                for (int k = lane; k < n; k += 32) t += J[(size_t)c * n + k] * s.pr[k];
                for (int o = 16; o > 0; o >>= 1) t += __shfl_sync(0xffffffffu, t, (lane + o) & 31);
                const int d = s.ti[TI_PRIOR_MAP + c];
                if (lane == 0) gp[d >= 0 ? d : NX + (-d - 1)] += t;
            }
        }
        PH_MARK_T(31, 96);
    }
    __syncthreads();
    PH_MARK(26);
    for (int k = tid; k < NR; k += SOLVE_THREADS) s.g[k] += gp[k];
    __syncthreads();
    PH_MARK(27);
    return cost;
}

CERB_D void apply_plus(const Smem &s, const double *delta, const double *lam, const double *dlam, double *lamc, int nF, bool ex_open, bool td_open, int tid) {
    if (tid < 11) pose_plus(s.xs + ST_POSE + 7 * tid, delta + 6 * tid, s.xc + ST_POSE + 7 * tid);
    else if (tid < 13) {
        const int e = tid - 11;
        if (ex_open) pose_plus(s.xs + ST_EX + 7 * e, delta + 66 + 6 * e, s.xc + ST_EX + 7 * e);
        else for (int k = 0; k < 7; k++) s.xc[ST_EX + 7 * e + k] = s.xs[ST_EX + 7 * e + k];
    }
    for (int k = tid; k < 99; k += SOLVE_THREADS) { const int f = k / 9, c = k % 9; s.xc[ST_SB + k] = s.xs[ST_SB + k] + delta[NX + NYB * f + c]; }
    for (int k = tid; k < 44; k += SOLVE_THREADS) { const int f = k / 4, c = k % 4; s.xc[ST_LB + k] = s.xs[ST_LB + k] + delta[NX + NYB * f + 9 + c]; }
    if (tid == 0) s.xc[ST_TD] = td_open ? s.xs[ST_TD] + delta[X_TD] : s.xs[ST_TD];
    for (int f = tid; f < nF; f += SOLVE_THREADS) lamc[f] = lam[f] + dlam[f];
    __syncthreads();
}

CERB_D double ambient_sq(const double *a, const double *b, const double *la, const double *lb, int nF, bool ex_open, bool lb_open, bool td_open, int tid) {
    double t = 0.0;
    for (int k = tid; k < ST_SIZE; k += SOLVE_THREADS) {
        if (k >= ST_LB && k < ST_EX && !lb_open) continue;
        if (k >= ST_EX && k < ST_TD && !ex_open) continue;
        if (k == ST_TD && !td_open) continue;
        const double v = b ? a[k] - b[k] : a[k];
        t += v * v;
    }
    for (int f = tid; f < nF; f += SOLVE_THREADS) { const double v = lb ? la[f] - lb[f] : la[f]; t += v * v; }
    return t;
}

template <bool SUB>
CERB_D double w_column_dot(const double *wf, int F, const double *v, double t) {
    constexpr int BATCH = 16;
    for (int a0 = 0; a0 < NX; a0 += BATCH) {
        double wr[BATCH];
        _Pragma("unroll")
        for (int u = 0; u < BATCH; u++) wr[u] = (a0 + u < NX) ? wf[(size_t)(a0 + u) * F] : 0.0;
        _Pragma("unroll")
        for (int u = 0; u < BATCH; u++) {
            if (a0 + u < NX) { if (SUB) t -= wr[u] * v[a0 + u]; else t += wr[u] * v[a0 + u]; }
        }
    }
    return t;
}

template <int W> struct TTPlan;
#define CERB_TT_PLAN(W, NR_, NB_, ...) template <> struct TTPlan<W> { static constexpr int nr = NR_, nb = NB_; static CERB_HD int tab(int i) { constexpr int t[] = {__VA_ARGS__}; return t[i]; } };
CERB_TT_PLAN(0, 4, 7, 0, 1, 2, 3, 0, 0, 0,   0, 0, 1, 0, 1, 0, 1,   0, 1, 1, 2, 2, 3, 3)
CERB_TT_PLAN(1, 4, 7, 2, 3, 4, 5, 0, 0, 0,   0, 0, 1, 0, 1, 0, 1,   0, 1, 1, 2, 2, 3, 3)
CERB_TT_PLAN(2, 4, 7, 4, 5, 6, 7, 0, 0, 0,   0, 0, 1, 0, 1, 0, 1,   0, 1, 1, 2, 2, 3, 3)
CERB_TT_PLAN(3, 4, 7, 6, 7, 8, 9, 0, 0, 0,   0, 0, 1, 0, 1, 0, 1,   0, 1, 1, 2, 2, 3, 3)
CERB_TT_PLAN(4, 6, 7, 8, 9, 0, 1, 4, 5, 0,   0, 0, 1, 2, 3, 2, 3,   0, 1, 1, 4, 4, 5, 5)
CERB_TT_PLAN(5, 6, 7, 0, 1, 6, 7, 8, 9, 0,   0, 0, 0, 0, 1, 1, 1,   2, 3, 4, 5, 2, 3, 4)
CERB_TT_PLAN(6, 7, 7, 1, 9, 2, 6, 7, 8, 3,   0, 2, 2, 2, 2, 6, 6,   1, 3, 4, 5, 1, 3, 4)
CERB_TT_PLAN(7, 5, 6, 3, 4, 5, 8, 9, 0, 0,   0, 0, 1, 1, 2, 2, 0,   3, 4, 3, 4, 3, 4, 0)
template <int W> CERB_D void ttt_warp(Smem &s, int lane) {
    typedef TTPlan<W> PL;
    const double *pr[7];
    _Pragma("unroll")
    for (int u = 0; u < 7; u++) {
        const int r = 8 * PL::tab(u < PL::nr ? u : 0) + (lane >> 2);
        pr[u] = (r < NX ? s.Hxy + r * NY : s.yv + NX) + (lane & 3);
    }
    double acc[7][2], fv[7];
    _Pragma("unroll")
    for (int k = 0; k < 7; k++) { acc[k][0] = 0.0; acc[k][1] = 0.0; }
    _Pragma("unroll")
    for (int u = 0; u < 7; u++) fv[u] = (u < PL::nr) ? pr[u][0] : 0.0;
    for (int q0 = 0; q0 < NY; q0 += 4) {
        const int qn = q0 + 4;
        const bool take = qn < NY && qn + (lane & 3) < NY;
        double fn[7];
        _Pragma("unroll")
        for (int u = 0; u < 7; u++) fn[u] = (u < PL::nr && take) ? pr[u][qn] : 0.0;
        _Pragma("unroll")
        for (int k = 0; k < 7; k++) if (k < PL::nb) CERB_DMMA(acc[k][0], acc[k][1], fv[PL::tab(7 + k)], fv[PL::tab(14 + k)], acc[k][0], acc[k][1]);
        _Pragma("unroll")
        for (int u = 0; u < 7; u++) fv[u] = fn[u];
    }
    _Pragma("unroll")
    for (int k = 0; k < 7; k++) {
        if (k >= PL::nb) continue;
        const int ba = PL::tab(PL::tab(7 + k)), bb = PL::tab(PL::tab(14 + k));
        const int a = 8 * ba + (lane >> 2);
        for (int e = 0; e < 2; e++) {
            const int b = 8 * bb + 2 * (lane & 3) + e;
            if (a > b || a >= NX || b > NX) continue;
            if (b == NX) s.yv[a] -= acc[k][e];
            else s.Hxx[b * NX + a] -= acc[k][e];
        }
    }
}

template <int W> struct SCPlan;
#define CERB_SC_PLAN(W, NR_, NB_, ...) template <> struct SCPlan<W> { static constexpr int nr = NR_, nb = NB_; static CERB_HD int tab(int i) { constexpr int t[] = {__VA_ARGS__}; return t[i]; } };
CERB_SC_PLAN(0, 8, 8, 0, 1, 2, 3, 4, 5, 6, 7, 0,   0, 0, 0, 0, 0, 0, 0, 0,   0, 1, 2, 3, 4, 5, 6, 7)
CERB_SC_PLAN(1, 9, 8, 0, 8, 9, 1, 2, 3, 4, 5, 6,   0, 0, 3, 3, 3, 3, 3, 3,   1, 2, 3, 4, 5, 6, 7, 8)
CERB_SC_PLAN(2, 9, 8, 1, 7, 8, 9, 2, 3, 4, 5, 6,   0, 0, 0, 4, 4, 4, 4, 4,   1, 2, 3, 4, 5, 6, 7, 8)
CERB_SC_PLAN(3, 8, 8, 2, 7, 8, 9, 3, 4, 5, 6, 0,   0, 0, 0, 4, 4, 4, 4, 4,   1, 2, 3, 4, 5, 6, 7, 1)
CERB_SC_PLAN(4, 7, 8, 3, 8, 9, 4, 5, 6, 7, 0, 0,   0, 0, 3, 3, 3, 3, 3, 3,   1, 2, 3, 4, 5, 6, 1, 2)
CERB_SC_PLAN(5, 5, 8, 5, 6, 7, 8, 9, 0, 0, 0, 0,   0, 0, 0, 0, 0, 1, 1, 1,   0, 1, 2, 3, 4, 1, 2, 3)
CERB_SC_PLAN(6, 4, 7, 6, 7, 8, 9, 0, 0, 0, 0, 0,   0, 1, 1, 1, 2, 2, 3, 0,   3, 1, 2, 3, 2, 3, 3, 0)
enum { SC_LDW = 36 };
template <int W> CERB_D void schur_tile(const double *tw, double (&acc)[8][2], int lane) {
    typedef SCPlan<W> PL;
    const double *pr[9];
    _Pragma("unroll")
    for (int u = 0; u < 9; u++) pr[u] = tw + (8 * PL::tab(u < PL::nr ? u : 0) + (lane >> 2)) * SC_LDW + (lane & 3);
    double fv[9];
    _Pragma("unroll")
    for (int u = 0; u < 9; u++) fv[u] = (u < PL::nr) ? pr[u][0] : 0.0;
    _Pragma("unroll")
    for (int ks = 0; ks < 8; ks++) {
        double fn[9];
        _Pragma("unroll")
        for (int u = 0; u < 9; u++) fn[u] = (u < PL::nr && ks < 7) ? pr[u][4 * (ks + 1)] : 0.0;
        _Pragma("unroll")
        for (int k = 0; k < 8; k++) if (k < PL::nb) CERB_DMMA(acc[k][0], acc[k][1], fv[PL::tab(9 + k)], fv[PL::tab(17 + k)], acc[k][0], acc[k][1]);
        _Pragma("unroll")
        for (int u = 0; u < 9; u++) fv[u] = fn[u];
    }
}
template <int W> CERB_D void schur_scatter(Smem &s, const double (&acc)[8][2], int lane) {
    typedef SCPlan<W> PL;
    _Pragma("unroll")
    for (int k = 0; k < 8; k++) {
        if (k >= PL::nb) continue;
        const int a = 8 * PL::tab(PL::tab(9 + k)) + (lane >> 2);
        for (int e = 0; e < 2; e++) {
            const int b = 8 * PL::tab(PL::tab(17 + k)) + 2 * (lane & 3) + e;
            if (a > b || a >= NX || b > NX) continue;
            if (b == NX) s.yv[a] -= acc[k][e];
            else { s.Hxx[b * NX + a] -= acc[k][e]; if (a != b) s.Hxx[a * NX + b] -= acc[k][e]; }
        }
    }
}

CERB_D bool build_prior_image(const SolveParams &P, Smem &s, int w, double *pimg, int tid) {
    const int *pmeta = P.prior_meta + (size_t)w * PRIOR_META_STRIDE;
    const bool has_prior = pmeta[0] != 0;
    if (has_prior) {
        const int n = pmeta[1], nb = pmeta[2];
        for (int k = tid; k < PIMG_SZ; k += SOLVE_THREADS) pimg[k] = 0.0;
        if (tid < nb) {
            const int kind = pmeta[4 + 3 * tid], index = pmeta[5 + 3 * tid], col = pmeta[6 + 3 * tid];
            const int local = (kind == 0 || kind == 3) ? 6 : prior_block_size(kind);
            for (int k = 0; k < local; k++) {
                int d;
                if (kind == 0) d = 6 * index + k;
                else if (kind == 3) d = 66 + 6 * index + k;
                else if (kind == 1) d = -(1 + NYB * index + k);
                else if (kind == 2) d = -(1 + NYB * index + 9 + k);
                else d = X_TD;
                s.ti[TI_PRIOR_MAP + col + k] = d;
            }
        }
        __syncthreads();
        Smem si = s; si.Hxx = pimg; si.Hxy = pimg + PIMG_HXY; si.Ad = pimg + PIMG_HXY + HXY_SZ; si.Bo = pimg + PIMG_HXY + HXY_SZ + AD_SZ;
        const double *Hp = P.prior_Hp + (size_t)w * PRIOR_LD * PRIOR_LD;
        for (int idx = tid; idx < n * n; idx += SOLVE_THREADS) {
            const int a = idx / n, b = idx % n;
            if (b < a) continue;
            scatter_H(si, s.ti[TI_PRIOR_MAP + a], s.ti[TI_PRIOR_MAP + b], Hp[a * PRIOR_LD + b]);
        }
    }
    return has_prior;
}

CERB_D void build_imu_plan(const Smem &s, const double *smem_base, int *plan, int tid) {
    if (tid >= 32) return;
    int q = 0;
    for (int mi = 0; mi < 5; mi++)
        for (int ni = mi; ni < 5; ni++, q++)
            for (int e = 0; e < 2; e++) {
                const int la = 8 * mi + (tid >> 2), lb = 8 * ni + 2 * (tid & 3) + e;
                int px = (int)(s.idg - smem_base) + tid, py = 256 << 12;
                if (la <= lb && lb <= 38 && la != 38) {
                    double *p0[2], *p1[2];
                    for (int i = 0; i < 2; i++) {
                        const int da = imu_col_dest(i, la);
                        if (lb == 38) { p0[i] = da >= 0 ? s.g + da : s.g + NX + (-da - 1); p1[i] = nullptr; }
                        else scatter_addr(s, da, imu_col_dest(i, lb), &p0[i], &p1[i]);
                    }
                    px = (int)(p0[0] - smem_base);
                    py = (int)(p0[1] - p0[0]) | (((p1[0] ? (int)(p1[0] - p0[0]) : 0) + 256) << 12);
                }
                plan[(2 * (q * 2 + e)) * 32 + tid] = px; plan[(2 * (q * 2 + e) + 1) * 32 + tid] = py;
            }
}
CERB_D void build_chunks(const int *fstart, Smem &s, int *chunks, int n_end) {
    int n = 0, c0 = 0;
    while (c0 < n_end) {
        chunks[1 + n] = c0;
        const int a = fstart[c0];
        int e = c0 + 1;
        while (e < n_end && e < c0 + 64 && fstart[e] == a) e++;
        if (n < TI_CACHED_CHUNKS) { s.ti[TI_CHUNK_CACHE + 2 * n] = c0; s.ti[TI_CHUNK_CACHE + 2 * n + 1] = ((e - c0) << 8) | a; }
        n++; c0 = e;
    }
    chunks[1 + n] = n_end; chunks[0] = n; s.ti[TI_NCHUNKS] = n;
}
struct Win { int w, nF; bool ex_open, lb_open, td_open, has_prior, bulk_ok; double *lam; CtaWs ws; };
struct PriorCopy { unsigned par0, par1; bool hxx_prefetched; };
CERB_D void linearize(const SolveParams &P, Smem &s, const Win &c, PriorCopy &pc, const double *xl, const double *laml, bool first, int tid PH_ARG) {
    const int F = c.ws.F, nF = c.nF;
    double *sca = s.sca, *W = c.ws.W, *hh = c.ws.hh, *gl = c.ws.gl, *sl = c.ws.sl, *pimg = c.ws.pimg;
    if (!c.has_prior) { for (int k = tid; k < HXX_SZ; k += SOLVE_THREADS) s.Hxx[k] = 0.0; }
    else if (c.bulk_ok) {
        if (!pc.hxx_prefetched) { __syncthreads(); if (tid == 0) CERB_BULK_G2S(s.Hxx, pimg, PIMG_HXY * 8, &s.mbar[0]); }
        CERB_MBAR_WAIT(&s.mbar[0], pc.par0); pc.par0 ^= 1;
    } else { if (!pc.hxx_prefetched) copy_g2s_async(s.Hxx, pimg, HXX_SZ, tid); CERB_CP_ASYNC_WAIT(); }
    pc.hxx_prefetched = false;
    for (int k = tid; k < NRP; k += SOLVE_THREADS) s.g[k] = 0.0;
    load_geometry(xl, s, tid);
    double part[2];
    PH_MARK(0);
    part[0] = vision_linearize(P, c.w, xl, laml, W, hh, gl, sl, !first, c.ws.chunks, tid);
    if (c.has_prior && c.bulk_ok) {
        if (tid == 0) CERB_BULK_G2S(s.Hxy, pimg + PIMG_HXY, PIMG_REST * 8, &s.mbar[1]);
        CERB_MBAR_WAIT(&s.mbar[1], pc.par1); pc.par1 ^= 1;
    } else if (c.has_prior) copy_g2s_async(s.Hxy, pimg + PIMG_HXY, PIMG_REST, tid);
    else for (int k = tid; k < PIMG_REST; k += SOLVE_THREADS) s.Hxy[k] = 0.0;
    __syncthreads();
    PH_MARK(1);
    part[0] += inertial_linearize(P, c.w, xl, tid);
    PH_MARK(2);
    part[1] = ambient_sq(xl, nullptr, laml, nullptr, nF, c.ex_open, c.lb_open, c.td_open, tid);
    double tot[2];
    block_sum<2>(part, s.red, tot, tid);
    if (tid == 0) { sca[S_LCOST] = tot[0]; sca[S_LNORM] = sqrt(tot[1]); }
    if (first) {
        for (int k = tid; k < NR; k += SOLVE_THREADS) {
            double d;
            bool active = true;
            if (k < NX) { d = s.Hxx[k * NX + k]; if (k >= 66 && k < X_TD && !c.ex_open) active = false; if (k == X_TD && !c.td_open) active = false; }
            else { const int yk = k - NX, f = yk / NYB, q = yk % NYB; d = s.Ad[f * HBLK + q * NYB + q]; if (q >= 9 && !c.lb_open) active = false; }
            s.sc[k] = active ? 1.0 / (1.0 + sqrt(d)) : 0.0;
        }
        for (int f = tid; f < nF; f += SOLVE_THREADS) sl[f] = 1.0 / (1.0 + sqrt(hh[f]));
    }
    __syncthreads();
    if (P.dbg && c.w == P.dbg_window && first) {
        for (int k = tid; k < NR; k += SOLVE_THREADS) {
            int dst; double d;
            if (k < NX) { dst = k < X_TD ? k : 221; d = s.Hxx[k * NX + k]; }
            else { const int yk = k - NX, f = yk / NYB, q = yk % NYB; dst = q < 9 ? 78 + 9 * f + q : 177 + 4 * f + (q - 9); d = s.Ad[f * HBLK + q * NYB + q]; }
            const bool act = s.sc[k] != 0.0;
            P.dbg[1 + dst] = act ? s.g[k] : 0.0; P.dbg[1 + NR + F + dst] = act ? d : 0.0;
        }
        for (int f = tid; f < nF; f += SOLVE_THREADS) { P.dbg[1 + NR + f] = gl[f]; P.dbg[1 + NR + F + NR + f] = hh[f]; }
        if (tid == 0) P.dbg[0] = sca[S_LCOST];
    }
    double gm = 0.0;
    for (int k = tid; k < NR; k += SOLVE_THREADS) if (s.sc[k] != 0.0) gm = fmax(gm, fabs(s.g[k]));
    for (int f = tid; f < nF; f += SOLVE_THREADS) gm = fmax(gm, fabs(!first ? gl[f] / sl[f] : gl[f]));
    for (int o = 16; o > 0; o >>= 1) gm = fmax(gm, __shfl_sync(0xffffffffu, gm, (tid + o) & 31));
    if ((tid & 31) == 0) s.red[tid >> 5] = gm;
    __syncthreads();
    if (tid == 0) { double m8 = s.red[0]; for (int k = 1; k < SOLVE_THREADS / 32; k++) m8 = fmax(m8, s.red[k]); sca[S_LGMAX] = m8; }
    for (int a = tid >> 5; a < NX; a += SOLVE_THREADS / 32) {
        const double sa = s.sc[a];
        for (int b = a + (tid & 31); b < NX; b += 32) { const double v = s.Hxx[a * NX + b] * (sa * s.sc[b]); s.Hxx[a * NX + b] = v; s.Hxx[b * NX + a] = v; }
        for (int q = tid & 31; q < NY; q += 32) s.Hxy[a * NY + q] *= sa * s.sc[NX + q];
    }
    for (int k = tid; k < AD_SZ; k += SOLVE_THREADS) { const int f = k / HBLK, a = (k % HBLK) / NYB, b = k % NYB; s.Ad[k] *= s.sc[NX + NYB * f + a] * s.sc[NX + NYB * f + b]; }
    for (int k = tid; k < BO_SZ; k += SOLVE_THREADS) { const int f = k / HBLK, a = (k % HBLK) / NYB, b = k % NYB; s.Bo[k] *= s.sc[NX + NYB * f + a] * s.sc[NX + NYB * (f + 1) + b]; }
    for (int k = tid; k < NR; k += SOLVE_THREADS) s.g[k] *= s.sc[k];
    if (first) {
        for (int k = tid; k < NX * nF; k += SOLVE_THREADS) { const int a = k / nF, f = k % nF; W[(size_t)a * F + f] *= s.sc[a] * sl[f]; }
        for (int f = tid; f < nF; f += SOLVE_THREADS) { hh[f] *= sl[f] * sl[f]; gl[f] *= sl[f]; }
    }
    __syncthreads();
}
CERB_D bool finalize_iteration(const SolveParams &P, double *sca, int iteration, int tid) {
    if (tid == 0) {
        if (iteration >= P.max_iters) { sca[S_DONE] = 1; sca[S_TERM] = 1; }
        else if (sca[S_GMAX] <= P.gtol) { sca[S_DONE] = 1; sca[S_TERM] = 0; }
        else if (sca[S_RADIUS] <= P.min_radius) { sca[S_DONE] = 1; sca[S_TERM] = 0; }
        else if (!(sca[S_XCOST] == sca[S_XCOST]) || fabs(sca[S_XCOST]) > 1e300) { sca[S_DONE] = 1; sca[S_TERM] = 2; }
    }
    __syncthreads();
    return sca[S_DONE] != 0.0;
}
CERB_D void dogleg_diagonal(Smem &s, const Win &c, int tid PH_ARG) {
    const int nF = c.nF;
    double *sca = s.sca, *Dl = c.ws.Dl, *ghl = c.ws.ghl, *stl = c.ws.stl;
    for (int k = tid; k < NR; k += SOLVE_THREADS) {
        const double d = (k < NX) ? s.Hxx[k * NX + k] : s.Ad[((k - NX) / NYB) * HBLK + ((k - NX) % NYB) * (NYB + 1)];
        const double D = sqrt(fmin(fmax(d, 1e-6), 1e32));
        s.D[k] = D; s.gh[k] = s.g[k] / D; s.stp[k] = s.gh[k] / D;
    }
    for (int f = tid; f < nF; f += SOLVE_THREADS) { const double D = sqrt(fmin(fmax(c.ws.hh[f], 1e-6), 1e32)); Dl[f] = D; ghl[f] = c.ws.gl[f] / D; stl[f] = ghl[f] / D; }
    __syncthreads();
    double part[2] = {0.0, 0.0};
    for (int k = tid; k < AD_SZ; k += SOLVE_THREADS) { const int f = k / HBLK, a = (k % HBLK) / NYB, b = k % NYB; part[0] += s.stp[NX + NYB * f + a] * s.Ad[k] * s.stp[NX + NYB * f + b]; }
    for (int k = tid; k < BO_SZ; k += SOLVE_THREADS) { const int f = k / HBLK, a = (k % HBLK) / NYB, b = k % NYB; part[0] += 2.0 * s.stp[NX + NYB * f + a] * s.Bo[k] * s.stp[NX + NYB * (f + 1) + b]; }
    for (int f = tid; f < nF; f += SOLVE_THREADS) part[1] += ghl[f] * ghl[f];
    for (int k = tid; k < NR; k += SOLVE_THREADS) part[1] += s.gh[k] * s.gh[k];
    double tot[2];
    block_sum<2>(part, s.red, tot, tid);
    if (tid == 0) { sca[S_GNORM2] = tot[1]; sca[S_VHV] = tot[0]; sca[S_OK] = 1; }
    PH_MARK(4);
}
CERB_D void chain_cholesky(Smem &s, int *chain_done, int lane PH_ARG) {
    const bool act = lane < NYB;
    const int r = act ? lane : 0;
    double m[NYB];
    _Pragma("unroll")
    for (int c = 0; c < NYB; c++) m[c] = 0.0;
    _Pragma("unroll 1")
    for (int f = 0; f < NFR; f++) {
        double *A = s.Ad + f * HBLK;
        double a[NYB], invd[NYB], myinv = 1.0;
        _Pragma("unroll")
        for (int c = 0; c < NYB; c++) a[c] = A[r * NYB + c];
        if (f > 0) {
            const double *Mp = s.Bo + (f - 1) * HBLK;
            _Pragma("unroll")
            for (int c = 0; c < NYB; c++) { double t = 0.0; _Pragma("unroll") for (int q = 0; q < NYB; q++) t += m[q] * Mp[c * NYB + q]; a[c] -= t; }
        }
        _Pragma("unroll")
        for (int j = 0; j < NYB; j++) {
            double d = __shfl_sync(0xffffffffu, a[j], j);
            if (!(d > 0.0)) { if (lane == 0) s.sca[S_OK] = 0; d = 1.0; }
            const double inv = rsqrt(d);
            invd[j] = inv;
            if (lane == j) myinv = inv;
            const double l = (lane == j) ? d * inv : a[j] * inv;
            a[j] = l;
            double *colb = s.chain_col + 16 * (j & 1);
            if (act) colb[lane] = l;
            __syncwarp();
            _Pragma("unroll")
            for (int k = j + 1; k < NYB; k++) a[k] -= l * colb[k];
        }
        if (act) { _Pragma("unroll") for (int c = 0; c < NYB; c++) if (c <= r) A[r * NYB + c] = a[c]; s.idg[NYB * f + r] = myinv; }
        __syncwarp();
        if (f < NFR - 1) {
            double *B = s.Bo + f * HBLK;
            double t[NYB];
            _Pragma("unroll")
            for (int c = 0; c < NYB; c++) t[c] = B[c * NYB + r];
            _Pragma("unroll")
            for (int c = 0; c < NYB; c++) {
                m[c] = t[c] * invd[c];
                _Pragma("unroll")
                for (int c2 = c + 1; c2 < NYB; c2++) t[c2] -= m[c] * A[c2 * NYB + c];
            }
            __syncwarp();
            if (act) { _Pragma("unroll") for (int c = 0; c < NYB; c++) B[r * NYB + c] = m[c]; }
            __syncwarp();
        }
        __threadfence_block(); __syncwarp();
        if (lane == 0) CERB_ST_RELEASE_S32(chain_done, f + 1);
    }
    PH_MARK(6);
}
CERB_D void schur_tile_w(int wq, const double *tw, double (&acc)[8][2], int lane) {
    switch (wq) { case 0: schur_tile<0>(tw, acc, lane); break; case 1: schur_tile<1>(tw, acc, lane); break; case 2: schur_tile<2>(tw, acc, lane); break;
                  case 3: schur_tile<3>(tw, acc, lane); break; case 4: schur_tile<4>(tw, acc, lane); break; case 5: schur_tile<5>(tw, acc, lane); break;
                  default: schur_tile<6>(tw, acc, lane); break; }
}
CERB_D void schur_scatter_w(int wq, Smem &s, const double (&acc)[8][2], int lane) {
    switch (wq) { case 0: schur_scatter<0>(s, acc, lane); break; case 1: schur_scatter<1>(s, acc, lane); break; case 2: schur_scatter<2>(s, acc, lane); break;
                  case 3: schur_scatter<3>(s, acc, lane); break; case 4: schur_scatter<4>(s, acc, lane); break; case 5: schur_scatter<5>(s, acc, lane); break;
                  default: schur_scatter<6>(s, acc, lane); break; }
}
CERB_D void ttt_warp_w(int wq, Smem &s, int lane) {
    switch (wq) { case 0: ttt_warp<0>(s, lane); break; case 1: ttt_warp<1>(s, lane); break; case 2: ttt_warp<2>(s, lane); break; case 3: ttt_warp<3>(s, lane); break;
                  case 4: ttt_warp<4>(s, lane); break; case 5: ttt_warp<5>(s, lane); break; case 6: ttt_warp<6>(s, lane); break; default: ttt_warp<7>(s, lane); break; }
}
CERB_D void lambda_schur(Smem &s, const CtaWs &ws, int nF, double mu, int tid PH_ARG) {
    const int F = ws.F;
    const double *W = ws.W, *hh = ws.hh, *gl = ws.gl, *Dl = ws.Dl, *stl = ws.stl;
    const int t2 = tid - 32, n2 = SOLVE_THREADS - 32;
    const int wq = (tid >> 5) - 1, lane = tid & 31;
    const int LDW = SC_LDW;
    double *tw = s.Ju;
    double *sinv = nF <= 1024 ? s.wj : ws.sinv;
    {
        const double *v = s.stp;
        double pv = 0.0;
        for (int k = t2; k < NX * NX; k += n2) pv += v[k / NX] * s.Hxx[k] * v[k % NX];
        for (int k = t2; k < NX * NY; k += n2) pv += 2.0 * v[k / NY] * s.Hxy[k] * v[NX + k % NY];
        for (int f = t2; f < nF; f += n2) {
            const double wv = w_column_dot<false>(W + f, F, v, 0.0);
            pv += 2.0 * stl[f] * wv + hh[f] * stl[f] * stl[f];
        }
        for (int o = 16; o > 0; o >>= 1) pv += __shfl_sync(0xffffffffu, pv, (lane + o) & 31);
        if (lane == 0) s.lin[wq] = pv;
        CERB_BAR_SYNC(1, n2);
        for (int k = t2; k < NX; k += n2) s.Hxx[k * NX + k] += mu * s.D[k] * s.D[k];
    }
    PH_MARK_T(19, 32);
    for (int f = t2; f < nF; f += n2) sinv[f] = rsqrt(hh[f] + mu * Dl[f] * Dl[f]);
    double acc[8][2];
    _Pragma("unroll")
    for (int k = 0; k < 8; k++) { acc[k][0] = 0.0; acc[k][1] = 0.0; }
    CERB_BAR_SYNC(1, n2);
    double buf[12];
    auto fetch = [&](int f0) {
        const int nf = (nF - f0) < 32 ? (nF - f0) : 32;
        _Pragma("unroll")
        for (int u = 0; u < 12; u++) {
            const int e = t2 + u * n2, a = e >> 5, f = e & 31;
            buf[u] = (e < 80 * 32 && f < nf) ? (a < NX ? W[(size_t)a * F + f0 + f] : (a == NX ? gl[f0 + f] : 0.0)) : 0.0;
        }
    };
    fetch(0);
    PH_MARK_T(37, 32);
    for (int f0 = 0; f0 < nF; f0 += 32) {
        const int nf = (nF - f0) < 32 ? (nF - f0) : 32;
        _Pragma("unroll")
        for (int u = 0; u < 12; u++) {
            const int e = t2 + u * n2, a = e >> 5, f = e & 31;
            if (e < 80 * 32) tw[a * LDW + f] = (f < nf) ? buf[u] * sinv[f0 + f] : 0.0;
        }
        CERB_BAR_SYNC(1, n2);
        PH_MARK_T(38, 32);
        if (f0 + 32 < nF) fetch(f0 + 32);
        schur_tile_w(wq, tw, acc, lane);
        CERB_BAR_SYNC(1, n2);
        PH_MARK_T(39, 32);
    }
    schur_scatter_w(wq, s, acc, lane);
    PH_MARK_T(7, 32);
}
CERB_D void forward_subst(Smem &s, const int *chain_done, int t2) {
    if (t2 <= NX) {
        double *row = (t2 < NX) ? s.Hxy + t2 * NY : s.yv + NX;
        double tp[NYB];
        _Pragma("unroll")
        for (int k = 0; k < NYB; k++) tp[k] = 0.0;
        _Pragma("unroll 1")
        for (int f = 0; f < NFR; f++) {
            while (CERB_LD_ACQUIRE_S32(chain_done) <= f) { CERB_SPIN_PAUSE(); }
            __threadfence_block();
            const double *L = s.Ad + f * HBLK, *idg = s.idg + NYB * f;
            double *t = row + NYB * f;
            double tc[NYB];
            _Pragma("unroll")
            for (int r = 0; r < NYB; r++) tc[r] = t[r];
            if (f > 0) {
                const double *M = s.Bo + (f - 1) * HBLK;
                _Pragma("unroll")
                for (int r = 0; r < NYB; r++) { double acc = 0.0; _Pragma("unroll") for (int q = 0; q < NYB; q++) acc += M[r * NYB + q] * tp[q]; tc[r] -= acc; }
            }
            _Pragma("unroll")
            for (int c = 0; c < NYB; c++) {
                tc[c] *= idg[c];
                _Pragma("unroll")
                for (int r = c + 1; r < NYB; r++) tc[r] -= L[r * NYB + c] * tc[c];
            }
            _Pragma("unroll")
            for (int r = 0; r < NYB; r++) { t[r] = tc[r]; tp[r] = tc[r]; }
        }
    }
}
CERB_D void panel_cholesky(Smem &s, int tid) {
    const int wq = tid >> 5, lane = tid & 31;
    auto factor_diag = [&](int c0, int nb, double *Lkk) {
        const bool act = lane < nb;
        const int r = act ? lane : 0;
        double a[8];
        _Pragma("unroll")
        for (int c = 0; c < 8; c++) a[c] = (c < nb && c <= r) ? s.Hxx[(c0 + r) * NX + c0 + c] : 0.0;
        double myinv = 1.0;
        _Pragma("unroll")
        for (int j = 0; j < 8; j++) {
            double d = __shfl_sync(0xffffffffu, a[j], j);
            if (j < nb && !(d > 0.0)) { if (lane == 0) s.sca[S_OK] = 0; }
            if (!(d > 0.0)) d = 1.0;
            const double inv = rsqrt(d);
            if (lane == j) myinv = inv;
            const double l = (lane == j) ? d * inv : a[j] * inv;
            a[j] = l;
            _Pragma("unroll")
            for (int k = j + 1; k < 8; k++) { const double lk = __shfl_sync(0xffffffffu, l, k); a[k] -= l * lk; }
        }
        if (act) {
            _Pragma("unroll")
            for (int c = 0; c < 8; c++) if (c <= r) { s.Hxx[(c0 + r) * NX + c0 + c] = a[c]; Lkk[r * 8 + c] = a[c]; }
            Lkk[64 + r] = myinv; s.idx[c0 + r] = myinv;
        }
    };
    auto trailing_block = [&](int c0, int b0, int b) {
        int bi = 0, idx = b;
        while (idx > bi) { idx -= bi + 1; bi++; }
        const int ri = 8 * (b0 + bi) + (lane >> 2), rj = 8 * (b0 + idx) + (lane >> 2);
        double a0 = 0.0, a1 = 0.0;
        for (int ks = 0; ks < 2; ks++) {
            const int cc = c0 + 4 * ks + (lane & 3);
            const double av = (ri < NX) ? s.Hxx[ri * NX + cc] : (ri == NX ? s.yv[cc] : 0.0);
            const double bv = (rj < NX) ? s.Hxx[rj * NX + cc] : 0.0;
            CERB_DMMA(a0, a1, av, bv, a0, a1);
        }
        const int cj = 8 * (b0 + idx) + 2 * (lane & 3);
        if (ri < NX) {
            if (cj <= ri && cj < NX) s.Hxx[ri * NX + cj] -= a0;
            if (cj + 1 <= ri && cj + 1 < NX) s.Hxx[ri * NX + cj + 1] -= a1;
        } else if (ri == NX) {
            if (cj < NX) s.yv[cj] -= a0;
            if (cj + 1 < NX) s.yv[cj + 1] -= a1;
        }
    };
    if (wq == 0) factor_diag(0, 8, s.red);
    __syncthreads();
    int pk = 0;
    for (int c0 = 0; c0 < NX; c0 += 8, pk ^= 1) {
        const int nb = (NX - c0) < 8 ? (NX - c0) : 8, c1 = c0 + nb;
        const double *Lkk = s.red + 80 * pk;
        if (tid <= NX - c1) {
            const int i = c1 + tid;
            double *row = (i < NX) ? s.Hxx + i * NX + c0 : s.yv + c0;
            double t[8];
            _Pragma("unroll")
            for (int c = 0; c < 8; c++) t[c] = (c < nb) ? row[c] : 0.0;
            _Pragma("unroll")
            for (int c = 0; c < 8; c++) {
                if (c < nb) {
                    t[c] *= Lkk[64 + c];
                    _Pragma("unroll")
                    for (int c2 = c + 1; c2 < 8; c2++) if (c2 < nb) t[c2] -= t[c] * Lkk[c2 * 8 + c];
                }
            }
            _Pragma("unroll")
            for (int c = 0; c < 8; c++) if (c < nb) row[c] = t[c];
        }
        __syncthreads();
        if (c1 >= NX) break;
        {
            const int b0 = c1 >> 3, nbt = 10 - b0;
            const int nblk = nbt * (nbt + 1) / 2;
            if (wq == 0) {
                trailing_block(c0, b0, 0);
                __syncwarp();
                factor_diag(c1, (NX - c1) < 8 ? (NX - c1) : 8, s.red + 80 * (pk ^ 1));
            } else {
                for (int b = wq; b < nblk; b += 7) trailing_block(c0, b0, b);
            }
        }
        __syncthreads();
    }
}
CERB_NOINLINE void gn_eliminate(const SolveParams &P, int w, double mu, int tid PH_ARG) {
    CERB_DYN_SMEM(double, smem_base);
    Smem s; smem_carve(smem_base, s);
    int *chain_done = s.ti + TI_CHAIN_DONE;
    if (tid < 32) chain_cholesky(s, chain_done, tid PH_FWD);
    else { lambda_schur(s, ws_carve(P), P.n_features[w], mu, tid PH_FWD); forward_subst(s, chain_done, tid - 32); }
}
CERB_NOINLINE void gn_reduce_factor(int tid PH_ARG) {
    CERB_DYN_SMEM(double, smem_base);
    Smem s; smem_carve(smem_base, s);
    ttt_warp_w(tid >> 5, s, tid & 31);
    __syncthreads();
    PH_MARK(9);
    panel_cholesky(s, tid);
    PH_MARK(10);
}
CERB_NOINLINE void back_substitution(const SolveParams &P, int w, bool has_prior, bool bulk_ok, double mu, bool fail, int tid PH_ARG) {
    CERB_DYN_SMEM(double, smem_base);
    Smem s; smem_carve(smem_base, s);
    const CtaWs ws = ws_carve(P);
    if (tid < 32) {
        double y0 = s.yv[tid], y1 = s.yv[32 + tid], y2 = (64 + tid < NX) ? s.yv[64 + tid] : 0.0;
        _Pragma("unroll 1")
        for (int k = NX - 1; k >= 0; k--) {
            const double *Lk = s.Hxx + k * NX;
            const double ik = s.idx[k];
            const double l0 = (tid < k) ? Lk[tid] : 0.0, l1 = (32 + tid < k) ? Lk[32 + tid] : 0.0, l2 = (64 + tid < k) ? Lk[64 + tid] : 0.0;
            const double src = (k >= 64) ? y2 : (k >= 32 ? y1 : y0);
            const double yk = __shfl_sync(0xffffffffu, src, k & 31) * ik;
            y0 = (tid == k) ? yk : y0 - l0 * yk;
            y1 = (32 + tid == k) ? yk : y1 - l1 * yk;
            y2 = (64 + tid == k) ? yk : y2 - l2 * yk;
        }
        s.yv[tid] = y0; s.yv[32 + tid] = y1; if (64 + tid < NX) s.yv[64 + tid] = y2;
    }
    __syncthreads();
    if (has_prior) {
        if (bulk_ok) { if (tid == 0) CERB_BULK_G2S(s.Hxx, ws.pimg, PIMG_HXY * 8, &s.mbar[0]); }
        else copy_g2s_async(s.Hxx, ws.pimg, HXX_SZ, tid);
    }
    PH_MARK(11);
    for (int q = tid; q < NY; q += SOLVE_THREADS) { double t = 0.0; for (int a = 0; a < NX; a++) t += s.Hxy[a * NY + q] * s.yv[a]; s.yv[NX + q] -= t; }
    __syncthreads();
    if (tid < 32) {
        const int r = tid < NYB ? tid : 0;
        double yn[NYB];
        _Pragma("unroll")
        for (int k = 0; k < NYB; k++) yn[k] = 0.0;
        _Pragma("unroll 1")
        for (int f = NFR - 1; f >= 0; f--) {
            const double *L = s.Ad + f * HBLK;
            double u = s.yv[NX + NYB * f + r];
            if (f < NFR - 1) {
                const double *M = s.Bo + f * HBLK;
                double t = 0.0;
                _Pragma("unroll")
                for (int k = 0; k < NYB; k++) t += M[k * NYB + r] * yn[k];
                u -= t;
            }
            double lc[NYB], ig[NYB];
            _Pragma("unroll")
            for (int k = 0; k < NYB; k++) { lc[k] = (tid < k) ? L[k * NYB + r] : 0.0; ig[k] = s.idg[NYB * f + k]; }
            _Pragma("unroll")
            for (int k = NYB - 1; k >= 0; k--) {
                const double yk = __shfl_sync(0xffffffffu, u, k) * ig[k];
                yn[k] = yk;
                u = (tid == k) ? yk : u - lc[k] * yk;
            }
            if (tid < NYB) s.yv[NX + NYB * f + tid] = u;
        }
    }
    __syncthreads();
    PH_MARK(12);
    double bad = 0.0;
    const int nF = P.n_features[w];
    for (int f = tid; f < nF; f += SOLVE_THREADS) {
        const double t = w_column_dot<true>(ws.W + f, ws.F, s.yv, ws.gl[f]);
        const double y = t / (ws.hh[f] + mu * ws.Dl[f] * ws.Dl[f]);
        ws.gnl[f] = y;
        if (!(fabs(y) < 1e300)) bad = 1.0;
    }
    for (int k = tid; k < NR; k += SOLVE_THREADS) if (!(fabs(s.yv[k]) < 1e300)) bad = 1.0;
    if (bad != 0.0) s.sca[S_OK] = 0;
    if (fail) s.sca[S_OK] = 0;
    __syncthreads();
    PH_MARK(13);
}
CERB_D void gauss_newton_step(const SolveParams &P, Smem &s, const Win &c, PriorCopy &pc, int &gn_attempts, int tid PH_ARG) {
    const int nF = c.nF;
    const double mu = s.sca[S_MU];
    for (int k = tid; k < NR; k += SOLVE_THREADS) {
        s.yv[k] = s.g[k];
        if (k >= NX) s.Ad[((k - NX) / NYB) * HBLK + ((k - NX) % NYB) * (NYB + 1)] += mu * s.D[k] * s.D[k];
    }
    if (tid == 0) s.ti[TI_CHAIN_DONE] = 0;
    __syncthreads();
    gn_eliminate(P, c.w, mu, tid PH_FWD);
    __syncthreads();
    if (tid == 0) {
        double vhv = s.sca[S_VHV];
        for (int k = 0; k < 7; k++) vhv += s.lin[k];
        s.sca[S_ALPHA] = s.sca[S_GNORM2] / vhv;
    }
    PH_MARK(5);
    __syncthreads();
    PH_MARK(8);
    gn_reduce_factor(tid PH_FWD);
    back_substitution(P, c.w, c.has_prior, c.bulk_ok, mu, gn_attempts < P.test_fail_factorizations, tid PH_FWD);
    if (c.has_prior) pc.hxx_prefetched = true;
    gn_attempts++;
    if (s.sca[S_OK] != 0.0) {
        double part3[2] = {0.0, 0.0};
        for (int k = tid; k < NR; k += SOLVE_THREADS) { const double v = -s.D[k] * s.yv[k]; s.gn[k] = v; part3[0] += v * v; part3[1] += s.gh[k] * v; }
        for (int f = tid; f < nF; f += SOLVE_THREADS) { const double v = -c.ws.Dl[f] * c.ws.gnl[f]; c.ws.gnl[f] = v; part3[0] += v * v; part3[1] += c.ws.ghl[f] * v; }
        double tot3[2];
        block_sum<2>(part3, s.red, tot3, tid);
        if (tid == 0) { s.sca[S_GNNORM2] = tot3[0]; s.sca[S_GDOTGN] = tot3[1]; }
        __syncthreads();
    }
}
CERB_D void dogleg_step(double *sca, int tid) {
    if (tid == 0) {
        const double radius = sca[S_RADIUS], alpha = sca[S_ALPHA];
        const double gradient_norm = sqrt(sca[S_GNORM2]), gauss_newton_norm = sqrt(sca[S_GNNORM2]);
        double p, q, nrm;
        if (gauss_newton_norm <= radius) { p = 0.0; q = 1.0; nrm = gauss_newton_norm; }
        else if (gradient_norm * alpha >= radius) { p = -(radius / gradient_norm); q = 0.0; nrm = radius; }
        else {
            const double b_dot_a = -alpha * sca[S_GDOTGN];
            const double a_squared_norm = (alpha * gradient_norm) * (alpha * gradient_norm);
            const double b_minus_a_squared_norm = a_squared_norm - 2 * b_dot_a + gauss_newton_norm * gauss_newton_norm;
            const double c = b_dot_a - a_squared_norm;
            const double d = sqrt(c * c + b_minus_a_squared_norm * (radius * radius - a_squared_norm));
            const double beta = (c <= 0) ? (d - c) / b_minus_a_squared_norm : (radius * radius - a_squared_norm) / (d + c);
            p = -alpha * (1.0 - beta); q = beta;
            nrm = sqrt(p * p * sca[S_GNORM2] + 2 * p * q * sca[S_GDOTGN] + q * q * sca[S_GNNORM2]);
        }
        sca[S_P] = p; sca[S_Q] = q; sca[S_DLNORM] = nrm;
        const double mu = sca[S_MU], g2 = sca[S_GNORM2], gg = sca[S_GDOTGN], n2 = sca[S_GNNORM2];
        const double sTg = p * g2 + q * gg;
        const double sHs = p * p * (g2 / alpha) - 2.0 * p * q * (g2 + mu * gg) + q * q * (-gg - mu * n2);
        sca[S_MODEL] = -(sTg + 0.5 * sHs);
    }
    __syncthreads();
}
CERB_D bool handle_invalid_step(double *sca, int tid) {
    if (tid == 0) {
        sca[S_INVALID] += 1;
        if (sca[S_INVALID] >= 5) { sca[S_DONE] = 1; sca[S_TERM] = 2; }
        sca[S_MU] *= 10.0; sca[S_REUSE] = 0;
    }
    __syncthreads();
    return sca[S_DONE] != 0.0;
}
CERB_D void evaluate_candidate(const SolveParams &P, Smem &s, const Win &c, PriorCopy &pc, bool speculate, int tid PH_ARG) {
    const int nF = c.nF;
    double *sca = s.sca, *stl = c.ws.stl, *lamc = c.ws.lamc;
    {
        const double p = sca[S_P], q = sca[S_Q];
        for (int k = tid; k < NR; k += SOLVE_THREADS) s.stp[k] = (p * s.gh[k] + q * s.gn[k]) / s.D[k] * s.sc[k];
        for (int f = tid; f < nF; f += SOLVE_THREADS) stl[f] = (p * c.ws.ghl[f] + q * c.ws.gnl[f]) / c.ws.Dl[f] * c.ws.sl[f];
    }
    __syncthreads();
    PH_MARK(14);
    apply_plus(s, s.stp, c.lam, stl, lamc, nF, c.ex_open, c.td_open, tid);
    double part[2];
    PH_MARK(15);
    if (speculate) { linearize(P, s, c, pc, s.xc, lamc, false, tid PH_FWD); part[0] = 0.0; }
    else {
        load_geometry(s.xc, s, tid);
        part[0] = vision_cost(P, c.w, s.xc, lamc, tid);
        PH_MARK(16);
        part[0] += inertial_cost(P, c.w, s.xc, tid);
    }
    PH_MARK(17);
    part[1] = ambient_sq(s.xs, s.xc, c.lam, lamc, nF, c.ex_open, c.lb_open, c.td_open, tid);
    double tot[2];
    block_sum<2>(part, s.red, tot, tid);
    if (tid == 0) {
        double cc = speculate ? sca[S_LCOST] : tot[0];
        if (!(cc == cc) || fabs(cc) > 1e300) cc = 1.7976931348623157e308;
        sca[S_CCOST] = cc; sca[S_STEPNORM] = sqrt(tot[1]);
    }
    __syncthreads();
}
CERB_D bool accept_or_reject(const SolveParams &P, double *sca, int tid) {
    if (tid == 0) {
        const double x_cost = sca[S_XCOST], cand = sca[S_CCOST];
        if (sca[S_STEPNORM] <= P.ptol * (sca[S_XNORM] + P.ptol)) { sca[S_DONE] = 1; sca[S_TERM] = 0; }
        else if (fabs(x_cost - cand) <= P.ftol * x_cost) { sca[S_DONE] = 1; sca[S_TERM] = 0; }
        else {
            const double rel = (x_cost - cand) / sca[S_MODEL];
            if (rel > P.min_rel_dec) {
                if (rel < 0.25) sca[S_RADIUS] *= 0.5;
                if (rel > 0.75) sca[S_RADIUS] = fmax(sca[S_RADIUS], 3.0 * sca[S_DLNORM]);
                sca[S_MU] = fmax(1e-8, 2.0 * sca[S_MU] / 10.0);
                sca[S_REUSE] = 0; sca[S_NSUCC] += 1; sca[S_OK] = 2;
                sca[S_XCOST] = cand;
            } else {
                sca[S_RADIUS] *= 0.5; sca[S_REUSE] = 1; sca[S_OK] = 1;
            }
        }
    }
    __syncthreads();
    return sca[S_DONE] != 0.0;
}

CERB_GLOBAL void __launch_bounds__(SOLVE_THREADS, CERB_SOLVE_MIN_BLOCKS) vilo_solve_kernel(CERB_GRID_CONSTANT SolveParams P) {
    CERB_DYN_SMEM(double, smem_base);
    Smem s; smem_carve(smem_base, s);
    const int tid = threadIdx.x;
    const CtaWs ws = ws_carve(P);
    double *sca = s.sca;
    PH_DECL();
    PriorCopy pc = {0, 0, false};
    if (tid == 0) { CERB_MBAR_INIT(&s.mbar[0]); CERB_MBAR_INIT(&s.mbar[1]); }
    build_imu_plan(s, smem_base, ws.imu_plan, tid);
    __syncthreads();
    for (int w = blockIdx.x; w < P.n_windows; w += gridDim.x) {
        Win c; c.w = w; c.nF = P.n_features[w]; c.ws = ws; c.lam = P.lam + (size_t)w * ws.F;
        c.ex_open = (P.flags[w] & 1) != 0; c.lb_open = P.optimize_leg_bias && (P.flags[w] & 4) == 0; c.td_open = (P.flags[w] & 2) != 0;
        if (tid == 0) build_chunks(P.feat_start + (size_t)w * ws.F, s, ws.chunks, c.nF);
        c.has_prior = build_prior_image(P, s, w, ws.pimg, tid);
        if (tid == 0) s.ti[TI_IMU_MASK] = 0;
        for (int k = tid; k < ST_STRIDE; k += SOLVE_THREADS) s.xs[k] = (k < ST_SIZE) ? P.state[(size_t)w * ST_STRIDE + k] : 0.0;
        if (tid == 0) {
            sca[S_RADIUS] = P.radius0; sca[S_MU] = P.test_initial_mu > 0.0 ? P.test_initial_mu : 1e-8; sca[S_REUSE] = 0; sca[S_DONE] = 0; sca[S_TERM] = 1; sca[S_ITER] = 0; sca[S_NSUCC] = 0;
            sca[S_INVALID] = 0; sca[S_DLNORM] = 0;
        }
        __syncthreads();
        c.bulk_ok = (reinterpret_cast<uintptr_t>(ws.pimg) & 15) == 0 && !P.no_bulk_copy;
        pc.hxx_prefetched = false;
        bool need_linearize = true, last_accepted = true;
        int iteration = 0, gn_attempts = 0;
        while (true) {
            if (need_linearize && (iteration < P.max_iters || iteration == 0)) {
                linearize(P, s, c, pc, s.xs, c.lam, iteration == 0, tid PH_FWD);
                if (tid == 0) { sca[S_XCOST] = sca[S_LCOST]; sca[S_XNORM] = sca[S_LNORM]; sca[S_GMAX] = sca[S_LGMAX]; if (iteration == 0) sca[S_INIT_COST] = sca[S_LCOST]; }
                __syncthreads();
                need_linearize = false;
                PH_MARK(3);
            }
            if (finalize_iteration(P, sca, iteration, tid)) break;
            iteration++;
            if (sca[S_REUSE] == 0.0) {
                for (;;) {
                    if (!(sca[S_MU] < 1.0)) {
                        __syncthreads();
                        if (tid == 0) { sca[S_OK] = 0; sca[S_REUSE] = 1; }
                        __syncthreads();
                        break;
                    }
                    dogleg_diagonal(s, c, tid PH_FWD);
                    gauss_newton_step(P, s, c, pc, gn_attempts, tid PH_FWD);
                    if (tid == 0) sca[S_REUSE] = 1;
                    __syncthreads();
                    if (sca[S_OK] != 0.0) break;
                    __syncthreads();
                    if (tid == 0) sca[S_MU] *= 10.0;
                    __syncthreads();
                    if (!(sca[S_MU] < 1.0)) break;
                    linearize(P, s, c, pc, s.xs, c.lam, false, tid PH_FWD);
                }
            }
            if (sca[S_OK] == 0.0) { if (handle_invalid_step(sca, tid)) break; need_linearize = true; continue; }
            dogleg_step(sca, tid);
            if (!(sca[S_MODEL] > 0.0)) { if (handle_invalid_step(sca, tid)) break; need_linearize = true; continue; }
            if (tid == 0) sca[S_INVALID] = 0;
            const bool speculate = last_accepted && iteration < P.max_iters;
            evaluate_candidate(P, s, c, pc, speculate, tid PH_FWD);
            if (accept_or_reject(P, sca, tid)) break;
            const bool accepted = (sca[S_OK] == 2.0);
            __syncthreads();
            if (accepted) {
                for (int k = tid; k < ST_STRIDE; k += SOLVE_THREADS) s.xs[k] = s.xc[k];
                for (int f = tid; f < c.nF; f += SOLVE_THREADS) c.lam[f] = ws.lamc[f];
                if (tid == 0) { sca[S_OK] = 1; if (speculate) { sca[S_XNORM] = sca[S_LNORM]; sca[S_GMAX] = sca[S_LGMAX]; } }
                __syncthreads();
                need_linearize = !speculate;
            }
            last_accepted = accepted;
            PH_MARK(18);
        }
        if (c.bulk_ok && pc.hxx_prefetched) { CERB_MBAR_WAIT(&s.mbar[0], pc.par0); pc.par0 ^= 1; }
        CERB_CP_ASYNC_WAIT();
        for (int k = tid; k < ST_SIZE; k += SOLVE_THREADS) P.state[(size_t)w * ST_STRIDE + k] = s.xs[k];
        if (tid == 0) {
            P.rep_i[4 * w + 0] = iteration; P.rep_i[4 * w + 1] = (int)sca[S_NSUCC]; P.rep_i[4 * w + 2] = (int)sca[S_TERM];
            P.rep_i[4 * w + 3] = (sca[S_XCOST] == sca[S_XCOST] && fabs(sca[S_XCOST]) < 1e300) ? 0 : 4;
            P.rep_d[2 * w + 0] = sca[S_INIT_COST]; P.rep_d[2 * w + 1] = sca[S_XCOST];
        }
        __syncthreads();
    }
}

struct MargParams {
    const int *flags;
    const double *state, *lam;
    double *A, *b;
    int posmax;
    int *dims;
    int *blocks;
};
enum { MARG_OLD = 0, MARG_SECOND_NEW = 1 };

CERB_GLOBAL void __launch_bounds__(SOLVE_THREADS, 1) marg_assemble_kernel(CERB_GRID_CONSTANT SolveParams P, CERB_GRID_CONSTANT MargParams M) {
    CERB_DYN_SMEM(double, smem_base);
    Smem s; smem_carve(smem_base, s);
    const int tid = threadIdx.x, F = P.maxF;
    const CtaWs ws = ws_carve(P);
    int *colx = reinterpret_cast<int *>(s.idx);
    int *coly = colx + 80;
    int *misc = coly + 32;
    build_imu_plan(s, smem_base, ws.imu_plan, tid);
    __syncthreads();
    for (int w = blockIdx.x; w < P.n_windows; w += gridDim.x) {
        const int nF = P.n_features[w], flag = M.flags[w];
        const double *lam = M.lam + (size_t)w * F;
        const int *pmeta = P.prior_meta + (size_t)w * PRIOR_META_STRIDE;
        const int *fstart = P.feat_start + (size_t)w * F, *fnobs = P.feat_nobs + (size_t)w * F, *foff = P.feat_off + (size_t)w * F;
        const int *stereo = P.obs_stereo + (size_t)w * P.maxObs;
        if (tid == 0) {
            int n0 = 0;
            if (flag == MARG_OLD) while (n0 < nF && fstart[n0] == 0) n0++;
            build_chunks(fstart, s, ws.chunks, n0);
            s.ti[TI_IMU_MASK] = flag == MARG_OLD ? 1 : 2;
            misc[0] = n0; misc[4] = 0; misc[5] = 0;
        }
        const bool has_prior = build_prior_image(P, s, w, ws.pimg, tid);
        for (int k = tid; k < ST_STRIDE; k += SOLVE_THREADS) s.xs[k] = (k < ST_SIZE) ? M.state[(size_t)w * ST_STRIDE + k] : 0.0;
        __syncthreads();
        const int n0 = misc[0];
        {
            int st = 0, len = 0;
            for (int f = tid; f < n0; f += SOLVE_THREADS) { const int nb = fnobs[f]; len = nb > len ? nb : len; for (int k = 0; k < nb; k++) st |= (stereo[foff[f] + k] != 0); }
            s.red[tid] = (double)(len | (st << 8));
            __syncthreads();
            if (tid == 0) { int l = 0, q = 0; for (int k = 0; k < SOLVE_THREADS; k++) { const int v = (int)s.red[k]; l = (v & 255) > l ? (v & 255) : l; q |= v >> 8; } misc[4] = q; misc[5] = l; }
            __syncthreads();
        }
        if (!has_prior) { for (int k = tid; k < HXX_SZ; k += SOLVE_THREADS) s.Hxx[k] = 0.0; }
        else copy_g2s(s.Hxx, ws.pimg, HXX_SZ, tid);
        for (int k = tid; k < NRP; k += SOLVE_THREADS) s.g[k] = 0.0;
        load_geometry(s.xs, s, tid);
        if (n0 > 0) vision_linearize(P, w, s.xs, lam, ws.W, ws.hh, ws.gl, ws.sl, false, ws.chunks, tid);
        __syncthreads();
        if (has_prior) copy_g2s(s.Hxy, ws.pimg + PIMG_HXY, PIMG_REST, tid);
        else for (int k = tid; k < PIMG_REST; k += SOLVE_THREADS) s.Hxy[k] = 0.0;
        __syncthreads();
        inertial_linearize(P, w, s.xs, tid);
        if (tid == 0) {
            bool pose[NFR] = {false}, sb[2] = {false, false}, lb[2] = {false, false}, ex[2] = {false, false}, td = false;
            if (has_prior) for (int b = 0; b < pmeta[2]; b++) {
                const int kind = pmeta[4 + 3 * b], index = pmeta[5 + 3 * b];
                if (kind == 0) pose[index] = true; else if (kind == 1) sb[index ? 1 : 0] = true; else if (kind == 2) lb[index ? 1 : 0] = true;
                else if (kind == 3) ex[index] = true; else td = true;
            }
            const bool noleg = (P.flags[w] & 4) != 0;
            if (flag == MARG_OLD) {
                if (!(P.pre[(size_t)w * CERB_WINDOW * PRE_STRIDE + PRE_SUM_DT] > 10.0)) { pose[0] = pose[1] = true; sb[0] = sb[1] = true; if (!noleg) lb[0] = lb[1] = true; }
                if (n0 > 0) { pose[0] = true; ex[0] = true; td = true; if (misc[4]) ex[1] = true; for (int j = 1; j < misc[5] && j < NFR; j++) pose[j] = true; }
            }
            for (int k = 0; k < 80 + 32; k++) colx[k] = -1;
            int m = 0, n = 0, status = 1, nblk = 0;
            int *blk = M.blocks + (size_t)w * 64;
#define MARG_BLK(kind_, shifted_, src_) do { blk[4 * nblk] = (kind_); blk[4 * nblk + 1] = (shifted_); blk[4 * nblk + 2] = n; blk[4 * nblk + 3] = (src_); nblk++; } while (0)
            if (flag == MARG_OLD) {
                if (pose[0]) { for (int k = 0; k < 6; k++) colx[k] = m + k; m += 6; }
                if (sb[0]) { for (int k = 0; k < 9; k++) coly[k] = m + k; m += 9; }
                if (lb[0]) { for (int k = 0; k < 4; k++) coly[9 + k] = m + k; m += 4; }
                m += n0;
                if (m == 0) status = 0;
                for (int j = 1; j < NFR; j++) if (pose[j]) { for (int k = 0; k < 6; k++) colx[6 * j + k] = m + n + k; MARG_BLK(0, j - 1, j); n += 6; }
                if (sb[1]) { for (int k = 0; k < 9; k++) coly[13 + k] = m + n + k; MARG_BLK(1, 0, 1); n += 9; }
                if (lb[1]) { for (int k = 0; k < 4; k++) coly[13 + 9 + k] = m + n + k; MARG_BLK(2, 0, 1); n += 4; }
            } else {
                if (!has_prior || !pose[CERB_WINDOW - 1]) status = 2;
                else {
                    for (int k = 0; k < 6; k++) colx[6 * (CERB_WINDOW - 1) + k] = k;
                    m = 6;
                    for (int j = 0; j < NFR; j++) if (pose[j] && j != CERB_WINDOW - 1) {
                        for (int k = 0; k < 6; k++) colx[6 * j + k] = m + n + k;
                        MARG_BLK(0, (j == CERB_WINDOW) ? j - 1 : j, j); n += 6;
                    }
                    if (sb[0]) { for (int k = 0; k < 9; k++) coly[k] = m + n + k; MARG_BLK(1, 0, 0); n += 9; }
                    if (lb[0]) { for (int k = 0; k < 4; k++) coly[9 + k] = m + n + k; MARG_BLK(2, 0, 0); n += 4; }
                }
            }
            if (status == 1) {
                for (int e = 0; e < 2; e++) if (ex[e]) { for (int k = 0; k < 6; k++) colx[66 + 6 * e + k] = m + n + k; MARG_BLK(3, e, e); n += 6; }
                if (td) { colx[X_TD] = m + n; MARG_BLK(4, 0, 0); n += 1; }
            }
#undef MARG_BLK
            misc[1] = m; misc[2] = n; misc[3] = status;
            int *dm = M.dims + 4 * w; dm[0] = m; dm[1] = n; dm[2] = status; dm[3] = nblk;
        }
        __syncthreads();
        if (misc[3] == 1) {
            const int m = misc[1], n = misc[2], pos = m + n, l0 = m - n0;
            double *A = M.A + (size_t)w * M.posmax * M.posmax, *b = M.b + (size_t)w * M.posmax;
            for (int e = tid; e < pos * pos; e += SOLVE_THREADS) A[e] = 0.0;
            __syncthreads();
            for (int e = tid; e < NX * NX; e += SOLVE_THREADS) {
                const int a = e / NX, c = e % NX; if (c < a) continue;
                const int ca = colx[a], cc = colx[c]; if (ca < 0 || cc < 0) continue;
                const double v = s.Hxx[a * NX + c];
                A[(size_t)ca * pos + cc] = v; A[(size_t)cc * pos + ca] = v;
            }
            for (int e = tid; e < NX * 26; e += SOLVE_THREADS) {
                const int a = e / 26, q = e % 26, ca = colx[a], cq = coly[q]; if (ca < 0 || cq < 0) continue;
                const double v = s.Hxy[a * NY + q];
                A[(size_t)ca * pos + cq] = v; A[(size_t)cq * pos + ca] = v;
            }
            for (int e = tid; e < 26 * 26; e += SOLVE_THREADS) {
                const int q = e / 26, r = e % 26, cq = coly[q], cr = coly[r]; if (cq < 0 || cr < 0) continue;
                const int fq = q / NYB, fr = r / NYB, kq = q % NYB, kr = r % NYB;
                A[(size_t)cq * pos + cr] = fq == fr ? s.Ad[fq * HBLK + kq * NYB + kr] : (fq < fr ? s.Bo[kq * NYB + kr] : s.Bo[kr * NYB + kq]);
            }
            for (int e = tid; e < NX * n0; e += SOLVE_THREADS) {
                const int a = e / n0, k = e % n0, ca = colx[a]; if (ca < 0) continue;
                const double v = ws.W[(size_t)a * F + k];
                A[(size_t)ca * pos + l0 + k] = v; A[(size_t)(l0 + k) * pos + ca] = v;
            }
            for (int k = tid; k < n0; k += SOLVE_THREADS) { A[(size_t)(l0 + k) * pos + l0 + k] = ws.hh[k]; b[l0 + k] = ws.gl[k]; }
            for (int a = tid; a < NX; a += SOLVE_THREADS) if (colx[a] >= 0) b[colx[a]] = s.g[a];
            for (int q = tid; q < 26; q += SOLVE_THREADS) if (coly[q] >= 0) b[coly[q]] = s.g[NX + q];
        }
        __syncthreads();
    }
}

}
```

Baseline: 33660.

## Pack vision chunks adaptively with per-chunk frames-per-pass and observed frame end

Rewrites the vision linearization so each feature chunk is processed by a templated routine that handles 1, 2 or 4 target frames per pass with 128, 64 or 32 features. Chunk building now also reads each feature's observation count, records the last observed frame, and picks a split that minimizes the number of passes. The aim is to stop iterating over frames no feature in the chunk observes and to fill idle lanes when chunks are small. The cost is three template instantiations, a more complex chunk encoding, and more serial work for thread 0 when building chunks.

```diff
diff --git a/cerberus_b200/csrc/cabi.cu b/cerberus_b200/csrc/cabi.cu
--- a/cerberus_b200/csrc/cabi.cu
+++ b/cerberus_b200/csrc/cabi.cu
@@ -626,9 +626,9 @@
 }
 
 #if defined(CERB_PHASE_TIMING) && !defined(CERB_CUSIM)
-extern "C" int cerb_prof_phase_cycles(unsigned long long *out48) {
-    unsigned long long z[48] = {0};
-    if (cudaMemcpyFromSymbol(out48, g_phase_cycles, sizeof(z)) != cudaSuccess) return CERB_ERR_CUDA;
+extern "C" int cerb_prof_phase_cycles(unsigned long long *out64) {
+    unsigned long long z[CERB_PHASE_SLOTS] = {0};
+    if (cudaMemcpyFromSymbol(out64, g_phase_cycles, sizeof(z)) != cudaSuccess) return CERB_ERR_CUDA;
     if (cudaMemcpyToSymbol(g_phase_cycles, z, sizeof(z)) != cudaSuccess) return CERB_ERR_CUDA;
     return CERB_OK;
 }
diff --git a/cerberus_b200/csrc/solve_kernel.cuh b/cerberus_b200/csrc/solve_kernel.cuh
--- a/cerberus_b200/csrc/solve_kernel.cuh
+++ b/cerberus_b200/csrc/solve_kernel.cuh
@@ -4,16 +4,19 @@
 namespace cerb {
 
 #if defined(CERB_PHASE_TIMING) && !defined(CERB_CUSIM)
-__device__ unsigned long long g_phase_cycles[48];
+#define CERB_PHASE_SLOTS 64
+__device__ unsigned long long g_phase_cycles[CERB_PHASE_SLOTS];
 #define PH_DECL() long long ph_t = clock64()
 #define PH_MARK_T(id, t) do { if ((threadIdx.x & 31) == 0) { const long long ph_n = clock64(); if (threadIdx.x == (t)) atomicAdd(&g_phase_cycles[id], (unsigned long long)(ph_n - ph_t)); ph_t = ph_n; } __syncwarp(); } while (0)
 #define PH_MARK(id) PH_MARK_T(id, 0)
+#define PH_COUNT(id) do { if (threadIdx.x == 0) atomicAdd(&g_phase_cycles[id], 1ull); } while (0)
 #define PH_ARG , long long &ph_t
 #define PH_FWD , ph_t
 #else
 #define PH_DECL()
 #define PH_MARK_T(id, t)
 #define PH_MARK(id)
+#define PH_COUNT(id)
 #define PH_ARG
 #define PH_FWD
 #endif
@@ -90,8 +93,11 @@
        S_OK, S_DONE, S_TERM, S_ITER, S_NSUCC, S_INVALID, S_GMAX, S_INIT_COST, S_P, S_Q, S_VHV, S_LCOST, S_LNORM, S_LGMAX, S_COUNT };
 static_assert(S_COUNT <= 32, "scalar slots overlap the chain's column line");
 enum { TI_PRIOR_MAP = 0, TI_NCHUNKS = 96, TI_CHUNK_CACHE = 97, TI_CACHED_CHUNKS = 15, TI_CHAIN_DONE = 130, TI_IMU_MASK = 131, TI_INTS = 132 };
-static_assert(TI_PRIOR_MAP + CERB_MAX_PRIOR_DIM <= TI_NCHUNKS && TI_CHUNK_CACHE + 2 * TI_CACHED_CHUNKS <= TI_CHAIN_DONE && TI_IMU_MASK < TI_INTS && TI_INTS % 2 == 0,
+static_assert(TI_PRIOR_MAP + CERB_MAX_PRIOR_DIM <= TI_NCHUNKS && TI_CHUNK_CACHE + TI_CACHED_CHUNKS + 1 <= TI_CHAIN_DONE && TI_IMU_MASK < TI_INTS && TI_INTS % 2 == 0,
               "s.ti slots overlap");
+enum { CHUNK_FPP = 4, CHUNK_JEND = 6, CHUNK_START = 10 };
+static_assert(NFR <= 16 && (CERB_MAX_FEATURES << CHUNK_START) > 0, "chunk word fields");
+CERB_HD int chunk_start(int word) { return word >> CHUNK_START; }
 enum { SMEM_DOUBLES = HXX_SZ + SMEM_HXX_PAD + HXY_SZ + AD_SZ + BO_SZ + 7 * NRP + 2 * ST_STRIDE + 99 + 18 + 3 + 31 * 39 + 960 + 192 + 8 * 256 + 128 * 8 + 32 + 32 + TI_INTS / 2 + 144 + 80 };
 
 CERB_D void smem_carve(double *base, Smem &s) {
@@ -223,19 +229,18 @@
         *base = hxx + ra * NX + (blk == 1 ? rb : (blk == 2 ? 66 + rb : 72 + rb)); *cj = 6 * NX + (blk == 1 ? 6 : 0);
     }
 }
-CERB_NOINLINE double vision_linearize(const SolveParams &P, int w, const double *x, const double *lam, double *W, double *hh, double *gl,
-                                      const double *sl, bool prescale, const int *chunks, int tid) {
+template <int FPP>
+CERB_D double vision_chunk(const SolveParams &P, int w, const double *x, const double *lam, double *W, double *hh, double *gl,
+                           const double *sl, bool prescale, int c0, int nc, int a, int jend, int jbase, int jca, int jcj, double cost,
+                           int tid PH_ARG) {
+    enum { CAP = 128 / FPP, NPH = 4 / FPP };
     CERB_DYN_SMEM(double, smem_base);
     Smem s; smem_carve(smem_base, s);
-    const int nF = P.n_features[w], F = P.maxF, mo = P.maxObs;
+    const int F = P.maxF, mo = P.maxObs;
     const double *obs = P.obs + (size_t)w * NOBS_PLANES * P.maxObs;
     const int *stereo = P.obs_stereo + (size_t)w * P.maxObs;
-    double cost = 0.0;
-    PH_DECL();
-    for (int i = tid; i < NX * nF; i += SOLVE_THREADS) W[(i / nF) * F + (i % nF)] = 0.0;
-    __syncthreads();
     const int wid = tid >> 5, lane = tid & 31;
-    const int cam = tid >> 7, jj = (tid >> 6) & 1, fl = tid & 63;
+    const int cam = tid >> 7, jj = (tid & 127) / CAP, fl = tid & (CAP - 1);
     double *T = s.tile;
     double *jp = s.Ju;
     double *pp = (wid < 5) ? s.Ju + 8 * VJ_SZ + VP_SZ * wid : s.tile + VT_SZ + VP_SZ * (wid - 5);
@@ -243,233 +248,262 @@
     const double *tq[4];
     bool tv[4];
     for (int g = 0; g < 4; g++) { const int pc = g == 0 ? c8 : 8 + 6 * (g - 1) + c8; tv[g] = (g == 0) || c8 < 6; tq[g] = T + (tv[g] ? pc : 0) * VT_LD + (lane & 3); }
+    PH_COUNT(48);
+    const int f = c0 + fl;
+    const bool ev = fl < nc;
+    int nobs = 0, off = 0;
+    double lamf = 1.0, pix = 0.0, piy = 0.0, vix = 0.0, viy = 0.0, tdi = 0.0;
+    const double slf = (prescale && ev) ? sl[f] : 1.0;
+    if (ev) {
+        nobs = P.feat_nobs[(size_t)w * F + f]; off = P.feat_off[(size_t)w * F + f];
+        lamf = 1.0 / lam[f];
+        pix = obs[0 * mo + off]; piy = obs[1 * mo + off]; vix = obs[2 * mo + off]; viy = obs[3 * mo + off]; tdi = obs[8 * mo + off];
+    }
+    ObsVals ov; ov.px = ov.py = ov.vx = ov.vy = ov.td = 0.0; ov.stereo = 0;
+    { const int j = a + jj; if (ev && j < a + nobs) obs_fetch(obs, stereo, mo, off + (j - a), cam, ov); }
+    for (int k = lane; k < VP_SZ; k += 32) pp[k] = 0.0;
+    if (tid < 2 * (NFR - 1 - a)) {
+        const int jq = a + 1 + (tid >> 1), cq = tid & 1;
+        const m33 Rc = ldm33(cq ? s.Rex + 9 : s.Rex);
+        const m33 A = mulT33(Rc, tr33(ldm33(s.Rw + 9 * jq)));
+        const m33 ARi = mul33(A, ldm33(s.Rw + 9 * a));
+        const m33 Tm = mul33(ARi, ldm33(s.Rex));
+        double *C = s.lin + 27 * tid;
+        for (int k = 0; k < 9; k++) { C[k] = A.m[k]; C[9 + k] = ARi.m[k]; C[18 + k] = Tm.m[k]; }
+    } else if (tid == 32) {
+        const m33 T3 = mul33(tr33(ldm33(s.Rex + 9)), ldm33(s.Rex));
+        for (int k = 0; k < 9; k++) s.lin[540 + k] = T3.m[k];
+    }
+    __syncthreads();
+    double h = 0.0, gq = 0.0, wT = 0.0, wI[6], wE0[6], wE1[6];
+    for (int k = 0; k < 6; k++) { wI[k] = 0.0; wE0[k] = 0.0; wE1[k] = 0.0; }
+    PH_MARK(20);
+    for (int j0 = a; j0 <= jend; j0 += FPP) {
+        PH_COUNT(49);
+        const int j = j0 + jj;
+        bool valid = ev && j < a + nobs;
+        int kind = PROJ_K1;
+        if (valid) {
+            if (j == a) { if (cam == 0 || !ov.stereo) valid = false; kind = PROJ_K3; }
+            else if (cam == 1) { if (!ov.stereo) valid = false; kind = PROJ_K2; }
+        }
+        double wjv[6] = {0, 0, 0, 0, 0, 0};
+        double *t0 = T + tid, *t1 = T + 256 + tid;
+        if (valid) {
+            const d3 tic = ld3(x + ST_EX), tc = kind == PROJ_K1 ? tic : ld3(x + ST_EX + 7);
+            const double *Rcp = kind == PROJ_K1 ? s.Rex : s.Rex + 9;
+            const double tdv = x[ST_TD];
+            const d3 pts_i = mk3(pix, piy, 1.0), vel_i = mk3(vix, viy, 0.0);
+            const d3 pts_i_td = pts_i - (tdv - tdi) * vel_i;
+            const double pjx_td = ov.px - (tdv - ov.td) * ov.vx, pjy_td = ov.py - (tdv - ov.td) * ov.vy;
+            const double inv_l = lamf;
+            const d3 p_ci = inv_l * pts_i_td;
+            const d3 p_bi = mv33(ldm33(s.Rex), p_ci) + tic;
+            d3 p_bj = p_bi;
+            if (kind != PROJ_K3) p_bj = mTv33(ldm33(s.Rw + 9 * j), (mv33(ldm33(s.Rw + 9 * a), p_bi) + ld3(x + ST_POSE + 7 * a)) - ld3(x + ST_POSE + 7 * j));
+            const d3 p_cj = mTv33(ldm33(Rcp), p_bj - tc);
+            const double iz = 1.0 / p_cj.z;
+            double r0 = P.sqrt_info * (p_cj.x * iz - pjx_td), r1 = P.sqrt_info * (p_cj.y * iz - pjy_td);
+            double cf; const double hw = huber_weight(P.huber, r0 * r0 + r1 * r1, &cf);
+            cost += cf;
+            r0 *= hw; r1 *= hw;
+            const double q = hw * P.sqrt_info * iz, c0 = -q * p_cj.x * iz, c1 = -q * p_cj.y * iz;
+            const d3 e0 = mk3(q, 0.0, c0), e1 = mk3(0.0, q, c1);
+#define VIS_U(M, u0, u1) const d3 u0 = mk3(q * (M)[0] + c0 * (M)[6], q * (M)[1] + c0 * (M)[7], q * (M)[2] + c0 * (M)[8]), u1 = mk3(q * (M)[3] + c1 * (M)[6], q * (M)[4] + c1 * (M)[7], q * (M)[5] + c1 * (M)[8])
+#define VIS_PUT(col, a0, a1) do { t0[(col) * VT_LD] = (a0); t1[(col) * VT_LD] = (a1); } while (0)
+#define VIS_PUT3(col, v0_, v1_) do { VIS_PUT(col, (v0_).x, (v1_).x); VIS_PUT((col) + 1, (v0_).y, (v1_).y); VIS_PUT((col) + 2, (v0_).z, (v1_).z); } while (0)
+            const double *Tm = kind == PROJ_K3 ? s.lin + 540 : s.lin + 27 * (2 * (j - a - 1) + cam) + 18;
+            VIS_U(Tm, uT0, uT1);
+            const d3 ptl = kind == PROJ_K3 ? pts_i : pts_i_td;
+            const double l0 = -inv_l * inv_l * dot3(uT0, ptl), l1 = -inv_l * inv_l * dot3(uT1, ptl);
+            const double d0 = -inv_l * dot3(uT0, vel_i) + hw * P.sqrt_info * ov.vx, d1 = -inv_l * dot3(uT1, vel_i) + hw * P.sqrt_info * ov.vy;
+            h += l0 * l0 + l1 * l1; gq += l0 * r0 + l1 * r1; wT += d0 * l0 + d1 * l1;
+            VIS_PUT(6, d0, d1); VIS_PUT(7, r0, r1);
+            const d3 uC0 = mk3(q * Rcp[0] + c0 * Rcp[2], q * Rcp[3] + c0 * Rcp[5], q * Rcp[6] + c0 * Rcp[8]);
+            const d3 uC1 = mk3(q * Rcp[1] + c1 * Rcp[2], q * Rcp[4] + c1 * Rcp[5], q * Rcp[7] + c1 * Rcp[8]);
+            const d3 er0 = cross3(e0, p_cj), er1 = cross3(e1, p_cj);
+            const d3 et0 = cross3(p_ci, uT0), et1 = cross3(p_ci, uT1);
+            d3 E0t0, E0t1, E0r0, E0r1, E1t0, E1t1, E1r0, E1r1;
+            if (kind == PROJ_K3) {
+                for (int k = 0; k < 6; k++) { VIS_PUT(k, 0.0, 0.0); VIS_PUT(8 + k, 0.0, 0.0); }
+                E0t0 = uC0; E0t1 = uC1; E0r0 = et0; E0r1 = et1; E1t0 = -uC0; E1t1 = -uC1; E1r0 = er0; E1r1 = er1;
+            } else {
+                const double *C = s.lin + 27 * (2 * (j - a - 1) + cam);
+                VIS_U(C, uA0, uA1);
+                VIS_U(C + 9, uR0, uR1);
+                const d3 ir0 = cross3(p_bi, uR0), ir1 = cross3(p_bi, uR1);
+                const d3 jr0 = cross3(uC0, p_bj), jr1 = cross3(uC1, p_bj);
+                VIS_PUT3(0, uA0, uA1); VIS_PUT3(3, ir0, ir1);
+                VIS_PUT3(8, -uA0, -uA1); VIS_PUT3(11, jr0, jr1);
+                wI[0] += uA0.x * l0 + uA1.x * l1; wI[1] += uA0.y * l0 + uA1.y * l1; wI[2] += uA0.z * l0 + uA1.z * l1;
+                wI[3] += ir0.x * l0 + ir1.x * l1; wI[4] += ir0.y * l0 + ir1.y * l1; wI[5] += ir0.z * l0 + ir1.z * l1;
+                wjv[0] = -(uA0.x * l0 + uA1.x * l1); wjv[1] = -(uA0.y * l0 + uA1.y * l1); wjv[2] = -(uA0.z * l0 + uA1.z * l1);
+                wjv[3] = jr0.x * l0 + jr1.x * l1; wjv[4] = jr0.y * l0 + jr1.y * l1; wjv[5] = jr0.z * l0 + jr1.z * l1;
+                if (kind == PROJ_K1) {
+                    E0t0 = uR0 - uC0; E0t1 = uR1 - uC1; E0r0 = et0 + er0; E0r1 = et1 + er1;
+                    E1t0 = mk3(0, 0, 0); E1t1 = E1t0; E1r0 = E1t0; E1r1 = E1t0;
+                } else {
+                    E0t0 = uR0; E0t1 = uR1; E0r0 = et0; E0r1 = et1; E1t0 = -uC0; E1t1 = -uC1; E1r0 = er0; E1r1 = er1;
+                }
+            }
+            VIS_PUT3(14, E0t0, E0t1); VIS_PUT3(17, E0r0, E0r1); VIS_PUT3(20, E1t0, E1t1); VIS_PUT3(23, E1r0, E1r1);
+            wE0[0] += E0t0.x * l0 + E0t1.x * l1; wE0[1] += E0t0.y * l0 + E0t1.y * l1; wE0[2] += E0t0.z * l0 + E0t1.z * l1;
+            wE0[3] += E0r0.x * l0 + E0r1.x * l1; wE0[4] += E0r0.y * l0 + E0r1.y * l1; wE0[5] += E0r0.z * l0 + E0r1.z * l1;
+            wE1[0] += E1t0.x * l0 + E1t1.x * l1; wE1[1] += E1t0.y * l0 + E1t1.y * l1; wE1[2] += E1t0.z * l0 + E1t1.z * l1;
+            wE1[3] += E1r0.x * l0 + E1r1.x * l1; wE1[4] += E1r0.y * l0 + E1r1.y * l1; wE1[5] += E1r0.z * l0 + E1r1.z * l1;
+#undef VIS_U
+#undef VIS_PUT
+#undef VIS_PUT3
+        } else {
+            for (int k = 0; k < VT_COLS; k++) { t0[k * VT_LD] = 0.0; t1[k * VT_LD] = 0.0; }
+        }
+        const bool wrow = valid && j != a;
+        if (wrow && cam == 0) for (int k = 0; k < 6; k++) W[(size_t)(6 * j + k) * F + f] = wjv[k] * (prescale ? s.sc[6 * j + k] * slf : 1.0);
+        __syncthreads();
+        PH_MARK(21);
+        double wprev[6] = {0, 0, 0, 0, 0, 0};
+        if (wrow && cam == 1) for (int k = 0; k < 6; k++) wprev[k] = W[(size_t)(6 * j + k) * F + f];
+        { const int jn = j + FPP; ov.stereo = 0; if (ev && jn < a + nobs) obs_fetch(obs, stereo, mo, off + (jn - a), cam, ov); }
+        {
+            const int jw = j0 + wid / (2 * NPH), hw = (wid / NPH) & 1, par = wid % NPH;
+            const bool k3 = (jw == a);
+            const int nkt = (nc + 3) >> 2;
+            const bool work = jw <= jend && par < nkt;
+            double acc[10][2];
+            for (int k = 0; k < 10; k++) { acc[k][0] = 0.0; acc[k][1] = 0.0; }
+            if (work) {
+                const int rb0 = 256 * hw + CAP * (jw - j0) + 4 * par;
+                if (!k3) {
+                    double v0 = tq[0][rb0], v1 = tv[1] ? tq[1][rb0] : 0.0, v2 = tv[2] ? tq[2][rb0] : 0.0;
+                    for (int ks = par; ks < nkt; ks += NPH) {
+                        const int rn = rb0 + 4 * (ks + NPH - par);
+                        const bool more = ks + NPH < nkt;
+                        const double n0 = more ? tq[0][rn] : 0.0, n1 = (more && tv[1]) ? tq[1][rn] : 0.0, n2 = (more && tv[2]) ? tq[2][rn] : 0.0;
+                        CERB_DMMA(acc[0][0], acc[0][1], v0, v0, acc[0][0], acc[0][1]);
+                        CERB_DMMA(acc[1][0], acc[1][1], v0, v1, acc[1][0], acc[1][1]);
+                        CERB_DMMA(acc[2][0], acc[2][1], v0, v2, acc[2][0], acc[2][1]);
+                        CERB_DMMA(acc[4][0], acc[4][1], v1, v1, acc[4][0], acc[4][1]);
+                        CERB_DMMA(acc[5][0], acc[5][1], v1, v2, acc[5][0], acc[5][1]);
+                        CERB_DMMA(acc[7][0], acc[7][1], v2, v2, acc[7][0], acc[7][1]);
+                        v0 = n0; v1 = n1; v2 = n2;
+                    }
+                }
+                {
+                    const int rb1 = rb0 + 128;
+                    double v0 = tq[0][rb1], v1 = (!k3 && tv[1]) ? tq[1][rb1] : 0.0, v2 = tv[2] ? tq[2][rb1] : 0.0, v3 = tv[3] ? tq[3][rb1] : 0.0;
+                    for (int ks = par; ks < nkt; ks += NPH) {
+                        const int rn = rb1 + 4 * (ks + NPH - par);
+                        const bool more = ks + NPH < nkt;
+                        const double n0 = more ? tq[0][rn] : 0.0, n1 = (more && !k3 && tv[1]) ? tq[1][rn] : 0.0, n2 = (more && tv[2]) ? tq[2][rn] : 0.0, n3 = (more && tv[3]) ? tq[3][rn] : 0.0;
+                        CERB_DMMA(acc[0][0], acc[0][1], v0, v0, acc[0][0], acc[0][1]);
+                        CERB_DMMA(acc[2][0], acc[2][1], v0, v2, acc[2][0], acc[2][1]);
+                        CERB_DMMA(acc[3][0], acc[3][1], v0, v3, acc[3][0], acc[3][1]);
+                        CERB_DMMA(acc[7][0], acc[7][1], v2, v2, acc[7][0], acc[7][1]);
+                        CERB_DMMA(acc[8][0], acc[8][1], v2, v3, acc[8][0], acc[8][1]);
+                        CERB_DMMA(acc[9][0], acc[9][1], v3, v3, acc[9][0], acc[9][1]);
+                        if (!k3) {
+                            CERB_DMMA(acc[1][0], acc[1][1], v0, v1, acc[1][0], acc[1][1]);
+                            CERB_DMMA(acc[4][0], acc[4][1], v1, v1, acc[4][0], acc[4][1]);
+                            CERB_DMMA(acc[5][0], acc[5][1], v1, v2, acc[5][0], acc[5][1]);
+                            CERB_DMMA(acc[6][0], acc[6][1], v1, v3, acc[6][0], acc[6][1]);
+                        }
+                        v0 = n0; v1 = n1; v2 = n2; v3 = n3;
+                    }
+                }
+                PH_MARK(28);
+                const int o = (lane >> 2) * 8 + 2 * (lane & 3);
+                pp[0 * 64 + o] += acc[0][0]; pp[0 * 64 + o + 1] += acc[0][1];
+                pp[1 * 64 + o] += acc[2][0]; pp[1 * 64 + o + 1] += acc[2][1];
+                pp[2 * 64 + o] += acc[3][0]; pp[2 * 64 + o + 1] += acc[3][1];
+                pp[3 * 64 + o] += acc[7][0]; pp[3 * 64 + o + 1] += acc[7][1];
+                pp[4 * 64 + o] += acc[8][0]; pp[4 * 64 + o + 1] += acc[8][1];
+                pp[5 * 64 + o] += acc[9][0]; pp[5 * 64 + o + 1] += acc[9][1];
+            }
+            {
+                const int o = wid * VJ_SZ + (lane >> 2) * 8 + 2 * (lane & 3);
+                jp[o] = acc[1][0]; jp[o + 1] = acc[1][1];
+                jp[64 + o] = acc[4][0]; jp[64 + o + 1] = acc[4][1];
+                jp[128 + o] = acc[5][0]; jp[128 + o + 1] = acc[5][1];
+                jp[192 + o] = acc[6][0]; jp[192 + o + 1] = acc[6][1];
+            }
+        }
+        if (wrow && cam == 1) for (int k = 0; k < 6; k++) W[(size_t)(6 * j + k) * F + f] = wprev[k] + wjv[k] * (prescale ? s.sc[6 * j + k] * slf : 1.0);
+        PH_MARK(29);
+        __syncthreads();
+        PH_MARK(22);
+        if (jbase >= 0) {
+            _Pragma("unroll")
+            for (int fj = 0; fj < FPP; fj++) {
+                const int jf = j0 + fj;
+                if (jf > jend || jf == a) continue;
+                const double *q = jp + (2 * NPH * fj) * VJ_SZ + tid;
+                double v = q[0];
+                _Pragma("unroll")
+                for (int u = 1; u < 2 * NPH; u++) v += q[u * VJ_SZ];
+                smem_base[jbase + jca * a + jcj * jf] += v;
+            }
+        }
+        PH_MARK(23);
+    }
+    __syncthreads();
+    {
+        double *ex = T;
+        ex[0 * 256 + tid] = h; ex[1 * 256 + tid] = gq; ex[2 * 256 + tid] = wT;
+        for (int k = 0; k < 6; k++) { ex[(3 + k) * 256 + tid] = wI[k]; ex[(9 + k) * 256 + tid] = wE0[k]; ex[(15 + k) * 256 + tid] = wE1[k]; }
+    }
+    __syncthreads();
+    for (int e = tid; e < VP_SZ; e += SOLVE_THREADS) {
+        double v = 0.0;
+        for (int wq = 0; wq < 8; wq++) v += ((wq < 5) ? s.Ju + 8 * VJ_SZ + VP_SZ * wq : s.tile + VT_SZ + VP_SZ * (wq - 5))[e];
+        const int blk = e >> 6, ra = (e >> 3) & 7, rb = e & 7;
+        const int ga = blk < 3 ? 0 : (blk < 5 ? 2 : 3), gb = blk == 0 ? 0 : (blk == 1 || blk == 3 ? 2 : 3);
+        vis_scatter(s, ga, gb, ra, rb, a, a, v);
+    }
+    if (tid < CAP && ev) {
+        const double *ex = T;
+        double q[21];
+        for (int k = 0; k < 21; k++) {
+            double v[2 * FPP];
+            _Pragma("unroll")
+            for (int u = 0; u < 2 * FPP; u++) v[u] = ex[k * 256 + u * CAP + tid];
+            _Pragma("unroll")
+            for (int h = 1; h < 2 * FPP; h *= 2)
+                _Pragma("unroll")
+                for (int u = 0; u < 2 * FPP; u += 2 * h) v[u] += v[u + h];
+            q[k] = v[0];
+        }
+        hh[f] = q[0] * slf * slf; gl[f] = q[1] * slf;
+        W[(size_t)X_TD * F + f] = q[2] * (prescale ? s.sc[X_TD] * slf : 1.0);
+        for (int k = 0; k < 6; k++) {
+            W[(size_t)(6 * a + k) * F + f] = q[3 + k] * (prescale ? s.sc[6 * a + k] * slf : 1.0);
+            W[(size_t)(66 + k) * F + f] = q[9 + k] * (prescale ? s.sc[66 + k] * slf : 1.0);
+            W[(size_t)(72 + k) * F + f] = q[15 + k] * (prescale ? s.sc[72 + k] * slf : 1.0);
+        }
+        for (int j = 0; j < NFR; j++)
+            if (j < a || j >= a + nobs) for (int k = 0; k < 6; k++) W[(size_t)(6 * j + k) * F + f] = 0.0;
+    }
+    __syncthreads();
+    PH_MARK(24);
+    return cost;
+}
+CERB_NOINLINE double vision_linearize(const SolveParams &P, int w, const double *x, const double *lam, double *W, double *hh, double *gl,
+                                      const double *sl, bool prescale, const int *chunks, int tid) {
+    CERB_DYN_SMEM(double, smem_base);
+    Smem s; smem_carve(smem_base, s);
+    double cost = 0.0;
+    PH_DECL();
+    PH_COUNT(50);
     int jbase, jca, jcj;
     vis_jplan(s, smem_base, tid, &jbase, &jca, &jcj);
     const int nchunks = s.ti[TI_NCHUNKS];
     for (int ch = 0; ch < nchunks; ch++) {
-        int c0, nc, a;
-        if (ch < TI_CACHED_CHUNKS) { const int *cc = s.ti + TI_CHUNK_CACHE + 2 * ch; c0 = cc[0]; nc = cc[1] >> 8; a = cc[1] & 255; }
-        else { c0 = chunks[1 + ch]; nc = chunks[2 + ch] - c0; a = P.feat_start[(size_t)w * F + c0]; }
-        const int f = c0 + fl;
-        const bool ev = fl < nc;
-        int nobs = 0, off = 0;
-        double lamf = 1.0, pix = 0.0, piy = 0.0, vix = 0.0, viy = 0.0, tdi = 0.0;
-        const double slf = (prescale && ev) ? sl[f] : 1.0;
-        if (ev) {
-            nobs = P.feat_nobs[(size_t)w * F + f]; off = P.feat_off[(size_t)w * F + f];
-            lamf = 1.0 / lam[f];
-            pix = obs[0 * mo + off]; piy = obs[1 * mo + off]; vix = obs[2 * mo + off]; viy = obs[3 * mo + off]; tdi = obs[8 * mo + off];
-        }
-        ObsVals ov; ov.px = ov.py = ov.vx = ov.vy = ov.td = 0.0; ov.stereo = 0;
-        { const int j = a + jj; if (ev && j < a + nobs) obs_fetch(obs, stereo, mo, off + (j - a), cam, ov); }
-        for (int k = lane; k < VP_SZ; k += 32) pp[k] = 0.0;
-        if (tid < 2 * (NFR - 1 - a)) {
-            const int jq = a + 1 + (tid >> 1), cq = tid & 1;
-            const m33 Rc = ldm33(cq ? s.Rex + 9 : s.Rex);
-            const m33 A = mulT33(Rc, tr33(ldm33(s.Rw + 9 * jq)));
-            const m33 ARi = mul33(A, ldm33(s.Rw + 9 * a));
-            const m33 Tm = mul33(ARi, ldm33(s.Rex));
-            double *C = s.lin + 27 * tid;
-            for (int k = 0; k < 9; k++) { C[k] = A.m[k]; C[9 + k] = ARi.m[k]; C[18 + k] = Tm.m[k]; }
-        } else if (tid == 32) {
-            const m33 T3 = mul33(tr33(ldm33(s.Rex + 9)), ldm33(s.Rex));
-            for (int k = 0; k < 9; k++) s.lin[540 + k] = T3.m[k];
-        }
-        __syncthreads();
-        double h = 0.0, gq = 0.0, wT = 0.0, wI[6], wE0[6], wE1[6];
-        for (int k = 0; k < 6; k++) { wI[k] = 0.0; wE0[k] = 0.0; wE1[k] = 0.0; }
-        PH_MARK(20);
-        for (int j0 = a; j0 < NFR; j0 += 2) {
-            const int j = j0 + jj;
-            bool valid = ev && j < a + nobs;
-            int kind = PROJ_K1;
-            if (valid) {
-                if (j == a) { if (cam == 0 || !ov.stereo) valid = false; kind = PROJ_K3; }
-                else if (cam == 1) { if (!ov.stereo) valid = false; kind = PROJ_K2; }
-            }
-            double wjv[6] = {0, 0, 0, 0, 0, 0};
-            double *t0 = T + tid, *t1 = T + 256 + tid;
-            if (valid) {
-                const d3 tic = ld3(x + ST_EX), tc = kind == PROJ_K1 ? tic : ld3(x + ST_EX + 7);
-                const double *Rcp = kind == PROJ_K1 ? s.Rex : s.Rex + 9;
-                const double tdv = x[ST_TD];
-                const d3 pts_i = mk3(pix, piy, 1.0), vel_i = mk3(vix, viy, 0.0);
-                const d3 pts_i_td = pts_i - (tdv - tdi) * vel_i;
-                const double pjx_td = ov.px - (tdv - ov.td) * ov.vx, pjy_td = ov.py - (tdv - ov.td) * ov.vy;
-                const double inv_l = lamf;
-                const d3 p_ci = inv_l * pts_i_td;
-                const d3 p_bi = mv33(ldm33(s.Rex), p_ci) + tic;
-                d3 p_bj = p_bi;
-                if (kind != PROJ_K3) p_bj = mTv33(ldm33(s.Rw + 9 * j), (mv33(ldm33(s.Rw + 9 * a), p_bi) + ld3(x + ST_POSE + 7 * a)) - ld3(x + ST_POSE + 7 * j));
-                const d3 p_cj = mTv33(ldm33(Rcp), p_bj - tc);
-                const double iz = 1.0 / p_cj.z;
-                double r0 = P.sqrt_info * (p_cj.x * iz - pjx_td), r1 = P.sqrt_info * (p_cj.y * iz - pjy_td);
-                double cf; const double hw = huber_weight(P.huber, r0 * r0 + r1 * r1, &cf);
-                cost += cf;
-                r0 *= hw; r1 *= hw;
-                const double q = hw * P.sqrt_info * iz, c0 = -q * p_cj.x * iz, c1 = -q * p_cj.y * iz;
-                const d3 e0 = mk3(q, 0.0, c0), e1 = mk3(0.0, q, c1);
-#define VIS_U(M, u0, u1) const d3 u0 = mk3(q * (M)[0] + c0 * (M)[6], q * (M)[1] + c0 * (M)[7], q * (M)[2] + c0 * (M)[8]), u1 = mk3(q * (M)[3] + c1 * (M)[6], q * (M)[4] + c1 * (M)[7], q * (M)[5] + c1 * (M)[8])
-#define VIS_PUT(col, a0, a1) do { t0[(col) * VT_LD] = (a0); t1[(col) * VT_LD] = (a1); } while (0)
-#define VIS_PUT3(col, v0_, v1_) do { VIS_PUT(col, (v0_).x, (v1_).x); VIS_PUT((col) + 1, (v0_).y, (v1_).y); VIS_PUT((col) + 2, (v0_).z, (v1_).z); } while (0)
-                const double *Tm = kind == PROJ_K3 ? s.lin + 540 : s.lin + 27 * (2 * (j - a - 1) + cam) + 18;
-                VIS_U(Tm, uT0, uT1);
-                const d3 ptl = kind == PROJ_K3 ? pts_i : pts_i_td;
-                const double l0 = -inv_l * inv_l * dot3(uT0, ptl), l1 = -inv_l * inv_l * dot3(uT1, ptl);
-                const double d0 = -inv_l * dot3(uT0, vel_i) + hw * P.sqrt_info * ov.vx, d1 = -inv_l * dot3(uT1, vel_i) + hw * P.sqrt_info * ov.vy;
-                h += l0 * l0 + l1 * l1; gq += l0 * r0 + l1 * r1; wT += d0 * l0 + d1 * l1;
-                VIS_PUT(6, d0, d1); VIS_PUT(7, r0, r1);
-                const d3 uC0 = mk3(q * Rcp[0] + c0 * Rcp[2], q * Rcp[3] + c0 * Rcp[5], q * Rcp[6] + c0 * Rcp[8]);
-                const d3 uC1 = mk3(q * Rcp[1] + c1 * Rcp[2], q * Rcp[4] + c1 * Rcp[5], q * Rcp[7] + c1 * Rcp[8]);
-                const d3 er0 = cross3(e0, p_cj), er1 = cross3(e1, p_cj);
-                const d3 et0 = cross3(p_ci, uT0), et1 = cross3(p_ci, uT1);
-                d3 E0t0, E0t1, E0r0, E0r1, E1t0, E1t1, E1r0, E1r1;
-                if (kind == PROJ_K3) {
-                    for (int k = 0; k < 6; k++) { VIS_PUT(k, 0.0, 0.0); VIS_PUT(8 + k, 0.0, 0.0); }
-                    E0t0 = uC0; E0t1 = uC1; E0r0 = et0; E0r1 = et1; E1t0 = -uC0; E1t1 = -uC1; E1r0 = er0; E1r1 = er1;
-                } else {
-                    const double *C = s.lin + 27 * (2 * (j - a - 1) + cam);
-                    VIS_U(C, uA0, uA1);
-                    VIS_U(C + 9, uR0, uR1);
-                    const d3 ir0 = cross3(p_bi, uR0), ir1 = cross3(p_bi, uR1);
-                    const d3 jr0 = cross3(uC0, p_bj), jr1 = cross3(uC1, p_bj);
-                    VIS_PUT3(0, uA0, uA1); VIS_PUT3(3, ir0, ir1);
-                    VIS_PUT3(8, -uA0, -uA1); VIS_PUT3(11, jr0, jr1);
-                    wI[0] += uA0.x * l0 + uA1.x * l1; wI[1] += uA0.y * l0 + uA1.y * l1; wI[2] += uA0.z * l0 + uA1.z * l1;
-                    wI[3] += ir0.x * l0 + ir1.x * l1; wI[4] += ir0.y * l0 + ir1.y * l1; wI[5] += ir0.z * l0 + ir1.z * l1;
-                    wjv[0] = -(uA0.x * l0 + uA1.x * l1); wjv[1] = -(uA0.y * l0 + uA1.y * l1); wjv[2] = -(uA0.z * l0 + uA1.z * l1);
-                    wjv[3] = jr0.x * l0 + jr1.x * l1; wjv[4] = jr0.y * l0 + jr1.y * l1; wjv[5] = jr0.z * l0 + jr1.z * l1;
-                    if (kind == PROJ_K1) {
-                        E0t0 = uR0 - uC0; E0t1 = uR1 - uC1; E0r0 = et0 + er0; E0r1 = et1 + er1;
-                        E1t0 = mk3(0, 0, 0); E1t1 = E1t0; E1r0 = E1t0; E1r1 = E1t0;
-                    } else {
-                        E0t0 = uR0; E0t1 = uR1; E0r0 = et0; E0r1 = et1; E1t0 = -uC0; E1t1 = -uC1; E1r0 = er0; E1r1 = er1;
-                    }
-                }
-                VIS_PUT3(14, E0t0, E0t1); VIS_PUT3(17, E0r0, E0r1); VIS_PUT3(20, E1t0, E1t1); VIS_PUT3(23, E1r0, E1r1);
-                wE0[0] += E0t0.x * l0 + E0t1.x * l1; wE0[1] += E0t0.y * l0 + E0t1.y * l1; wE0[2] += E0t0.z * l0 + E0t1.z * l1;
-                wE0[3] += E0r0.x * l0 + E0r1.x * l1; wE0[4] += E0r0.y * l0 + E0r1.y * l1; wE0[5] += E0r0.z * l0 + E0r1.z * l1;
-                wE1[0] += E1t0.x * l0 + E1t1.x * l1; wE1[1] += E1t0.y * l0 + E1t1.y * l1; wE1[2] += E1t0.z * l0 + E1t1.z * l1;
-                wE1[3] += E1r0.x * l0 + E1r1.x * l1; wE1[4] += E1r0.y * l0 + E1r1.y * l1; wE1[5] += E1r0.z * l0 + E1r1.z * l1;
-#undef VIS_U
-#undef VIS_PUT
-#undef VIS_PUT3
-            } else {
-                for (int k = 0; k < VT_COLS; k++) { t0[k * VT_LD] = 0.0; t1[k * VT_LD] = 0.0; }
-            }
-            const bool wrow = valid && j != a;
-            if (wrow && cam == 0) for (int k = 0; k < 6; k++) W[(size_t)(6 * j + k) * F + f] = wjv[k] * (prescale ? s.sc[6 * j + k] * slf : 1.0);
-            __syncthreads();
-            PH_MARK(21);
-            double wprev[6] = {0, 0, 0, 0, 0, 0};
-            if (wrow && cam == 1) for (int k = 0; k < 6; k++) wprev[k] = W[(size_t)(6 * j + k) * F + f];
-            { const int jn = j + 2; ov.stereo = 0; if (ev && jn < a + nobs) obs_fetch(obs, stereo, mo, off + (jn - a), cam, ov); }
-            {
-                const int jw = j0 + (wid >> 2), hw = (wid >> 1) & 1, par = wid & 1;
-                const bool k3 = (jw == a);
-                const int nkt = (nc + 3) >> 2;
-                const bool work = jw < NFR && par < nkt;
-                double acc[10][2];
-                for (int k = 0; k < 10; k++) { acc[k][0] = 0.0; acc[k][1] = 0.0; }
-                if (work) {
-                    const int rb0 = 256 * hw + 64 * (wid >> 2) + 4 * par;
-                    if (!k3) {
-                        double v0 = tq[0][rb0], v1 = tv[1] ? tq[1][rb0] : 0.0, v2 = tv[2] ? tq[2][rb0] : 0.0;
-                        for (int ks = par; ks < nkt; ks += 2) {
-                            const int rn = rb0 + 4 * (ks + 2 - par);
-                            const bool more = ks + 2 < nkt;
-                            const double n0 = more ? tq[0][rn] : 0.0, n1 = (more && tv[1]) ? tq[1][rn] : 0.0, n2 = (more && tv[2]) ? tq[2][rn] : 0.0;
-                            CERB_DMMA(acc[0][0], acc[0][1], v0, v0, acc[0][0], acc[0][1]);
-                            CERB_DMMA(acc[1][0], acc[1][1], v0, v1, acc[1][0], acc[1][1]);
-                            CERB_DMMA(acc[2][0], acc[2][1], v0, v2, acc[2][0], acc[2][1]);
-                            CERB_DMMA(acc[4][0], acc[4][1], v1, v1, acc[4][0], acc[4][1]);
-                            CERB_DMMA(acc[5][0], acc[5][1], v1, v2, acc[5][0], acc[5][1]);
-                            CERB_DMMA(acc[7][0], acc[7][1], v2, v2, acc[7][0], acc[7][1]);
-                            v0 = n0; v1 = n1; v2 = n2;
-                        }
-                    }
-                    {
-                        const int rb1 = rb0 + 128;
-                        double v0 = tq[0][rb1], v1 = (!k3 && tv[1]) ? tq[1][rb1] : 0.0, v2 = tv[2] ? tq[2][rb1] : 0.0, v3 = tv[3] ? tq[3][rb1] : 0.0;
-                        for (int ks = par; ks < nkt; ks += 2) {
-                            const int rn = rb1 + 4 * (ks + 2 - par);
-                            const bool more = ks + 2 < nkt;
-                            const double n0 = more ? tq[0][rn] : 0.0, n1 = (more && !k3 && tv[1]) ? tq[1][rn] : 0.0, n2 = (more && tv[2]) ? tq[2][rn] : 0.0, n3 = (more && tv[3]) ? tq[3][rn] : 0.0;
-                            CERB_DMMA(acc[0][0], acc[0][1], v0, v0, acc[0][0], acc[0][1]);
-                            CERB_DMMA(acc[2][0], acc[2][1], v0, v2, acc[2][0], acc[2][1]);
-                            CERB_DMMA(acc[3][0], acc[3][1], v0, v3, acc[3][0], acc[3][1]);
-                            CERB_DMMA(acc[7][0], acc[7][1], v2, v2, acc[7][0], acc[7][1]);
-                            CERB_DMMA(acc[8][0], acc[8][1], v2, v3, acc[8][0], acc[8][1]);
-                            CERB_DMMA(acc[9][0], acc[9][1], v3, v3, acc[9][0], acc[9][1]);
-                            if (!k3) {
-                                CERB_DMMA(acc[1][0], acc[1][1], v0, v1, acc[1][0], acc[1][1]);
-                                CERB_DMMA(acc[4][0], acc[4][1], v1, v1, acc[4][0], acc[4][1]);
-                                CERB_DMMA(acc[5][0], acc[5][1], v1, v2, acc[5][0], acc[5][1]);
-                                CERB_DMMA(acc[6][0], acc[6][1], v1, v3, acc[6][0], acc[6][1]);
-                            }
-                            v0 = n0; v1 = n1; v2 = n2; v3 = n3;
-                        }
-                    }
-                    PH_MARK(28);
-                    const int o = (lane >> 2) * 8 + 2 * (lane & 3);
-                    pp[0 * 64 + o] += acc[0][0]; pp[0 * 64 + o + 1] += acc[0][1];
-                    pp[1 * 64 + o] += acc[2][0]; pp[1 * 64 + o + 1] += acc[2][1];
-                    pp[2 * 64 + o] += acc[3][0]; pp[2 * 64 + o + 1] += acc[3][1];
-                    pp[3 * 64 + o] += acc[7][0]; pp[3 * 64 + o + 1] += acc[7][1];
-                    pp[4 * 64 + o] += acc[8][0]; pp[4 * 64 + o + 1] += acc[8][1];
-                    pp[5 * 64 + o] += acc[9][0]; pp[5 * 64 + o + 1] += acc[9][1];
-                }
-                {
-                    const int o = wid * VJ_SZ + (lane >> 2) * 8 + 2 * (lane & 3);
-                    jp[o] = acc[1][0]; jp[o + 1] = acc[1][1];
-                    jp[64 + o] = acc[4][0]; jp[64 + o + 1] = acc[4][1];
-                    jp[128 + o] = acc[5][0]; jp[128 + o + 1] = acc[5][1];
-                    jp[192 + o] = acc[6][0]; jp[192 + o + 1] = acc[6][1];
-                }
-            }
-            if (wrow && cam == 1) for (int k = 0; k < 6; k++) W[(size_t)(6 * j + k) * F + f] = wprev[k] + wjv[k] * (prescale ? s.sc[6 * j + k] * slf : 1.0);
-            PH_MARK(29);
-            __syncthreads();
-            PH_MARK(22);
-            if (jbase >= 0) {
-                _Pragma("unroll")
-                for (int fj = 0; fj < 2; fj++) {
-                    const int jf = j0 + fj;
-                    if (jf >= NFR || jf == a) continue;
-                    const double *q = jp + (4 * fj) * VJ_SZ + tid;
-                    smem_base[jbase + jca * a + jcj * jf] += ((q[0] + q[VJ_SZ]) + q[2 * VJ_SZ]) + q[3 * VJ_SZ];
-                }
-            }
-            PH_MARK(23);
-        }
-        __syncthreads();
-        {
-            double *ex = T;
-            ex[0 * 256 + tid] = h; ex[1 * 256 + tid] = gq; ex[2 * 256 + tid] = wT;
-            for (int k = 0; k < 6; k++) { ex[(3 + k) * 256 + tid] = wI[k]; ex[(9 + k) * 256 + tid] = wE0[k]; ex[(15 + k) * 256 + tid] = wE1[k]; }
-        }
-        __syncthreads();
-        for (int e = tid; e < VP_SZ; e += SOLVE_THREADS) {
-            double v = 0.0;
-            for (int wq = 0; wq < 8; wq++) v += ((wq < 5) ? s.Ju + 8 * VJ_SZ + VP_SZ * wq : s.tile + VT_SZ + VP_SZ * (wq - 5))[e];
-            const int blk = e >> 6, ra = (e >> 3) & 7, rb = e & 7;
-            const int ga = blk < 3 ? 0 : (blk < 5 ? 2 : 3), gb = blk == 0 ? 0 : (blk == 1 || blk == 3 ? 2 : 3);
-            vis_scatter(s, ga, gb, ra, rb, a, a, v);
-        }
-        if (tid < 64 && ev) {
-            const double *ex = T;
-            double q[21];
-            for (int k = 0; k < 21; k++) q[k] = ((ex[k * 256 + tid] + ex[k * 256 + 64 + tid]) + ex[k * 256 + 128 + tid]) + ex[k * 256 + 192 + tid];
-            hh[f] = q[0] * slf * slf; gl[f] = q[1] * slf;
-            W[(size_t)X_TD * F + f] = q[2] * (prescale ? s.sc[X_TD] * slf : 1.0);
-            for (int k = 0; k < 6; k++) {
-                W[(size_t)(6 * a + k) * F + f] = q[3 + k] * (prescale ? s.sc[6 * a + k] * slf : 1.0);
-                W[(size_t)(66 + k) * F + f] = q[9 + k] * (prescale ? s.sc[66 + k] * slf : 1.0);
-                W[(size_t)(72 + k) * F + f] = q[15 + k] * (prescale ? s.sc[72 + k] * slf : 1.0);
-            }
-        }
-        __syncthreads();
-        PH_MARK(24);
+        const int *cw = ch < TI_CACHED_CHUNKS ? s.ti + TI_CHUNK_CACHE + ch : chunks + 1 + ch;
+        const int w0 = cw[0], c0 = chunk_start(w0), nc = chunk_start(cw[1]) - c0, a = w0 & 15, jend = (w0 >> CHUNK_JEND) & 15;
+        switch ((w0 >> CHUNK_FPP) & 3) {
+            case 0: cost = vision_chunk<1>(P, w, x, lam, W, hh, gl, sl, prescale, c0, nc, a, jend, jbase, jca, jcj, cost, tid PH_FWD); break;
+            case 1: cost = vision_chunk<2>(P, w, x, lam, W, hh, gl, sl, prescale, c0, nc, a, jend, jbase, jca, jcj, cost, tid PH_FWD); break;
+            default: cost = vision_chunk<4>(P, w, x, lam, W, hh, gl, sl, prescale, c0, nc, a, jend, jbase, jca, jcj, cost, tid PH_FWD); break;
+        }
     }
     return cost;
 }
@@ -894,17 +928,44 @@
                 plan[(2 * (q * 2 + e)) * 32 + tid] = px; plan[(2 * (q * 2 + e) + 1) * 32 + tid] = py;
             }
 }
-CERB_D void build_chunks(const int *fstart, Smem &s, int *chunks, int n_end) {
-    int n = 0, c0 = 0;
+CERB_D void build_chunks(const int *fstart, const int *fnobs, Smem &s, int *chunks, int n_end) {
+    int n = 0;
+    auto put = [&](int word) { chunks[1 + n] = word; if (n <= TI_CACHED_CHUNKS) s.ti[TI_CHUNK_CACHE + n] = word; };
+    int c0 = 0;
     while (c0 < n_end) {
-        chunks[1 + n] = c0;
         const int a = fstart[c0];
-        int e = c0 + 1;
-        while (e < n_end && e < c0 + 64 && fstart[e] == a) e++;
-        if (n < TI_CACHED_CHUNKS) { s.ti[TI_CHUNK_CACHE + 2 * n] = c0; s.ti[TI_CHUNK_CACHE + 2 * n + 1] = ((e - c0) << 8) | a; }
-        n++; c0 = e;
-    }
-    chunks[1 + n] = n_end; chunks[0] = n; s.ti[TI_NCHUNKS] = n;
+        int e = c0, jrun = a;
+        for (bool open = true; open;) {
+            int st[8], nb[8];
+            _Pragma("unroll")
+            for (int u = 0; u < 8; u++) { const int t = e + u; st[u] = t < n_end ? fstart[t] : -1; nb[u] = t < n_end ? fnobs[t] : 0; }
+            _Pragma("unroll")
+            for (int u = 0; u < 8; u++) { open = open && st[u] == a; if (open) { jrun = jrun > a + nb[u] - 1 ? jrun : a + nb[u] - 1; e++; } }
+        }
+        const int r = e - c0, L = (jrun < NFR - 1 ? jrun : NFR - 1) - a + 1;
+        int b1 = 0, b2 = 0, b4 = 0, bp = 1 << 30, bc = 0;
+        for (int n1 = (r + 31) / 128; n1 <= (r + 127) / 128; n1++)
+            for (int q = 0; q < 4; q++) {
+                const int n2 = q & 1, n4 = q >> 1, cap = 128 * n1 + 64 * n2 + 32 * n4, last = n4 ? 32 : (n2 ? 64 : 128);
+                if (cap < r || cap - last >= r) continue;
+                const int np = n1 * L + n2 * ((L + 1) / 2) + n4 * ((L + 3) / 4), nch = n1 + n2 + n4;
+                if (np < bp || (np == bp && nch < bc)) { bp = np; bc = nch; b1 = n1; b2 = n2; b4 = n4; }
+            }
+        for (int k = 0; k < b1 + b2 + b4; k++) {
+            const int lf = k < b1 ? 0 : (k < b1 + b2 ? 1 : 2), nc = (128 >> lf) < e - c0 ? (128 >> lf) : e - c0;
+            int jend = a;
+            for (int t = c0; t < c0 + nc; t += 8) {
+                int nb[8];
+                _Pragma("unroll")
+                for (int u = 0; u < 8; u++) nb[u] = t + u < c0 + nc ? fnobs[t + u] : 0;
+                _Pragma("unroll")
+                for (int u = 0; u < 8; u++) jend = jend > a + nb[u] - 1 ? jend : a + nb[u] - 1;
+            }
+            put(c0 << CHUNK_START | (jend < NFR - 1 ? jend : NFR - 1) << CHUNK_JEND | lf << CHUNK_FPP | a);
+            n++; c0 += nc;
+        }
+    }
+    put(n_end << CHUNK_START); chunks[0] = n; s.ti[TI_NCHUNKS] = n;
 }
 struct Win { int w, nF; bool ex_open, lb_open, td_open, has_prior, bulk_ok; double *lam; CtaWs ws; };
 struct PriorCopy { unsigned par0, par1; bool hxx_prefetched; };
@@ -1470,7 +1531,7 @@
     for (int w = blockIdx.x; w < P.n_windows; w += gridDim.x) {
         Win c; c.w = w; c.nF = P.n_features[w]; c.ws = ws; c.lam = P.lam + (size_t)w * ws.F;
         c.ex_open = (P.flags[w] & 1) != 0; c.lb_open = P.optimize_leg_bias && (P.flags[w] & 4) == 0; c.td_open = (P.flags[w] & 2) != 0;
-        if (tid == 0) build_chunks(P.feat_start + (size_t)w * ws.F, s, ws.chunks, c.nF);
+        if (tid == 0) build_chunks(P.feat_start + (size_t)w * ws.F, P.feat_nobs + (size_t)w * ws.F, s, ws.chunks, c.nF);
         c.has_prior = build_prior_image(P, s, w, ws.pimg, tid);
         if (tid == 0) s.ti[TI_IMU_MASK] = 0;
         for (int k = tid; k < ST_STRIDE; k += SOLVE_THREADS) s.xs[k] = (k < ST_SIZE) ? P.state[(size_t)w * ST_STRIDE + k] : 0.0;
@@ -1573,7 +1634,7 @@
         if (tid == 0) {
             int n0 = 0;
             if (flag == MARG_OLD) while (n0 < nF && fstart[n0] == 0) n0++;
-            build_chunks(fstart, s, ws.chunks, n0);
+            build_chunks(fstart, fnobs, s, ws.chunks, n0);
             s.ti[TI_IMU_MASK] = flag == MARG_OLD ? 1 : 2;
             misc[0] = n0; misc[4] = 0; misc[5] = 0;
         }
```

Result: faster. 34010 (median of 6 runs) (+1.0%).
